# krm01/Snappy.jl

Hardware: AMD Instinct MI355X
Metric: GB/s compressed+decompressed (batched blocks) at 1/2/4/8 GPUs; % HBM peak (higher is better)
Workload: dtype u8; 1 GPU; configs 2+3: 10000 x 64 KiB text blocks per GPU, fast-mode compress + uncompress round trip per step; blocks_per_gpu=10000, block_bytes=65536, parallelism=dp1 (blocks sharded per rank, RCCL size all-gather)

## Files before the change

### include/snappy_mi355x.h

```cpp
#ifndef SNAPPY_MI355X_H_
#define SNAPPY_MI355X_H_

#include <stddef.h>
#include <stdint.h>

#ifdef __cplusplus
extern "C" {
#endif

typedef int32_t sm_status;
enum {
  SM_OK = 0,
  SM_INVALID_INPUT = 1,
  SM_BUFFER_TOO_SMALL = 2,
  SM_ERR_INPUT_TOO_LARGE = 16,
  SM_ERR_INVALID = 17,
  SM_ERR_VARINT = 18,
  SM_ERR_COPY_OFFSET = 19,
  SM_ERR_COPY_LENGTH = 20,
  SM_ERR_LITERAL = 21,
  SM_ERR_DEVICE = 32,
  SM_ERR_ARGUMENT = 33
};

enum { SM_MODE_REFERENCE = 0, SM_MODE_FAST = 1, SM_MODE_FAST_DENSE = 2 };

#define SM_BLOCK_SIZE 65536u
#define SM_OUT_LEN_ERROR 0xfff00000u

typedef struct sm_ctx sm_ctx;

const char* sm_status_message(sm_status st);

size_t sm_max_compressed_length(size_t source_length);
sm_status sm_uncompressed_length(const char* compressed, size_t compressed_length, size_t* result);
sm_status sm_parse32(const uint8_t* buf, size_t len, size_t off, uint32_t* value, size_t* next);
size_t sm_encode32(uint8_t* buf, uint32_t value);
sm_status sm_find_match_length(const uint8_t* buf, size_t len, size_t i1, size_t i2, size_t limit,
                               size_t* matched);

sm_ctx* sm_ctx_create(int device);
void sm_ctx_destroy(sm_ctx* ctx);
void* sm_ctx_stream(sm_ctx* ctx);
int sm_ctx_last_path(sm_ctx* ctx);
sm_status sm_ctx_set_small_decode(sm_ctx* ctx, int enable);
sm_status sm_ctx_set_split_compress(sm_ctx* ctx, int enable);
int sm_ctx_last_compress_split(sm_ctx* ctx);

sm_status sm_compress(sm_ctx* ctx, const char* input, size_t input_length, char* compressed,
                      size_t* compressed_length, int mode);
sm_status sm_uncompress(sm_ctx* ctx, const char* compressed, size_t compressed_length, char* uncompressed,
                        size_t* uncompressed_length);

sm_status sm_compress_batch_device(sm_ctx* ctx, const uint8_t* d_in, const uint64_t* d_in_off,
                                   const uint32_t* d_in_len, uint32_t nblk, uint8_t* d_out,
                                   const uint64_t* d_out_off, uint32_t* d_out_len, int mode, void* stream);
sm_status sm_compress_fragments_device(sm_ctx* ctx, const uint8_t* d_in, const uint64_t* d_in_off,
                                       const uint32_t* d_in_len, uint32_t nblk, uint8_t* d_out,
                                       const uint64_t* d_out_off, uint32_t* d_out_len, uint64_t total_len,
                                       int mode, void* stream);
sm_status sm_place_fragments_device(sm_ctx* ctx, const uint8_t* d_src, const uint64_t* d_src_off,
                                    const uint32_t* d_len, uint32_t nfrag, const uint64_t* d_dst_off,
                                    uint64_t total_len, int write_header, uint8_t* d_dst, uint64_t dst_capacity,
                                    uint64_t* d_local_off, int32_t* d_status, void* stream);
sm_status sm_uncompress_fragments_device(sm_ctx* ctx, const uint8_t* d_in, const uint64_t* d_in_off,
                                         const uint32_t* d_in_len, uint32_t nblk, uint8_t* d_out,
                                         const uint64_t* d_out_off, const uint32_t* d_frag_len, uint32_t* d_out_len,
                                         int32_t* d_status, void* stream);

sm_status sm_uncompress_batch_device(sm_ctx* ctx, const uint8_t* d_in, const uint64_t* d_in_off,
                                     const uint32_t* d_in_len, uint32_t nblk, uint8_t* d_out,
                                     const uint64_t* d_out_off, const uint32_t* d_out_cap,
                                     uint32_t* d_out_len, int32_t* d_status, void* stream);

sm_status sm_validate_batch_device(sm_ctx* ctx, const uint8_t* d_in, const uint64_t* d_in_off,
                                   const uint32_t* d_in_len, uint32_t nblk, int32_t* d_status, void* stream);
sm_status sm_uncompressed_length_batch_device(sm_ctx* ctx, const uint8_t* d_in, const uint64_t* d_in_off,
                                              const uint32_t* d_in_len, uint32_t nblk, uint32_t* d_len,
                                              int32_t* d_status, void* stream);

sm_status sm_compress_batch(sm_ctx* ctx, const uint8_t* in, const uint64_t* in_off, const uint32_t* in_len,
                            uint32_t nblk, uint8_t* out, const uint64_t* out_off, uint32_t* out_len, int mode);
sm_status sm_uncompress_batch(sm_ctx* ctx, const uint8_t* in, const uint64_t* in_off, const uint32_t* in_len,
                              uint32_t nblk, uint8_t* out, const uint64_t* out_off, const uint32_t* out_cap,
                              uint32_t* out_len, int32_t* status);

sm_status sm_compress_batch_sharded(sm_ctx* const* ctxs, int nctx, const uint8_t* in, const uint64_t* in_off,
                                    const uint32_t* in_len, uint32_t nblk, uint8_t* out, const uint64_t* out_off,
                                    uint32_t* out_len, int mode);
sm_status sm_uncompress_batch_sharded(sm_ctx* const* ctxs, int nctx, const uint8_t* in, const uint64_t* in_off,
                                      const uint32_t* in_len, uint32_t nblk, uint8_t* out, const uint64_t* out_off,
                                      const uint32_t* out_cap, uint32_t* out_len, int32_t* status);

sm_status sm_validate_compressed_buffer(sm_ctx* ctx, const char* compressed, size_t compressed_length);

sm_status sm_snappy_compress(const char* input, size_t input_length, char* compressed, size_t* compressed_length);
sm_status sm_snappy_uncompress(const char* compressed, size_t compressed_length, char* uncompressed,
                               size_t* uncompressed_length);
size_t sm_snappy_max_compressed_length(size_t source_length);
sm_status sm_snappy_uncompressed_length(const char* compressed, size_t compressed_length, size_t* result);
sm_status sm_snappy_validate_compressed_buffer(const char* compressed, size_t compressed_length);
sm_status sm_snappy_set_mode(int mode);

const char* sm_version(void);

#ifdef __cplusplus
}
#endif
#endif
```

### snappy.jl_amd/__init__.py

```python
import ctypes
import os
import threading

import numpy as np

HERE = os.path.dirname(os.path.abspath(__file__))
LIB_PATH = os.environ.get("SNAPPY_MI355X_LIB") or os.path.join(HERE, "libsnappy_mi355x.so")
BLOCK_SIZE = 65536

SM_OK = 0
SM_BUFFER_TOO_SMALL = 2
SM_ERR_DEVICE = 32
SM_OUT_LEN_ERROR = 0xFFF00000
MODES = {"reference": 0, "fast": 1, "dense": 2}

ABI_SYMBOLS = (
    "sm_status_message", "sm_max_compressed_length", "sm_uncompressed_length", "sm_parse32",
    "sm_encode32", "sm_ctx_create", "sm_ctx_destroy", "sm_ctx_stream", "sm_compress", "sm_uncompress",
    "sm_compress_batch_device", "sm_uncompress_batch_device", "sm_compress_batch",
    "sm_uncompress_batch", "sm_version", "sm_compress_fragments_device", "sm_ctx_last_path", "sm_ctx_set_small_decode",
    "sm_ctx_set_split_compress", "sm_ctx_last_compress_split",
    "sm_find_match_length", "sm_validate_batch_device", "sm_uncompressed_length_batch_device",
    "sm_validate_compressed_buffer", "sm_compress_batch_sharded", "sm_uncompress_batch_sharded",
    "sm_uncompress_fragments_device", "sm_place_fragments_device", "sm_snappy_compress", "sm_snappy_uncompress",
    "sm_snappy_max_compressed_length", "sm_snappy_uncompressed_length", "sm_snappy_validate_compressed_buffer",
    "sm_snappy_set_mode",
)


class SnappyError(Exception):

    def __init__(self, code, message=None):
        self.code = int(code)
        super().__init__(message if message is not None else status_message(code))


_lib = None
_ctx = {}
_ctx_lock = threading.Lock()


def library_path():
    return LIB_PATH


def lib():
    global _lib
    if _lib is None:
        if not os.path.exists(LIB_PATH):
            raise OSError("libsnappy_mi355x.so not built (run __graft_entry__.build())")
        _lib = load_library(LIB_PATH)
    return _lib


def load_library(path):
    L = ctypes.CDLL(path)
    vp, sz, i32, u32 = ctypes.c_void_p, ctypes.c_size_t, ctypes.c_int32, ctypes.c_uint32
    L.sm_status_message.restype = ctypes.c_char_p
    L.sm_status_message.argtypes = [i32]
    L.sm_max_compressed_length.restype = sz
    L.sm_max_compressed_length.argtypes = [sz]
    L.sm_uncompressed_length.restype = i32
    L.sm_uncompressed_length.argtypes = [vp, sz, ctypes.POINTER(sz)]
    L.sm_parse32.restype = i32
    L.sm_parse32.argtypes = [vp, sz, sz, ctypes.POINTER(u32), ctypes.POINTER(sz)]
    L.sm_encode32.restype = sz
    L.sm_encode32.argtypes = [vp, u32]
    L.sm_ctx_create.restype = vp
    L.sm_ctx_create.argtypes = [ctypes.c_int]
    L.sm_ctx_destroy.restype = None
    L.sm_ctx_destroy.argtypes = [vp]
    L.sm_ctx_stream.restype = vp
    L.sm_ctx_stream.argtypes = [vp]
    L.sm_compress.restype = i32
    L.sm_compress.argtypes = [vp, vp, sz, vp, ctypes.POINTER(sz), ctypes.c_int]
    L.sm_uncompress.restype = i32
    L.sm_uncompress.argtypes = [vp, vp, sz, vp, ctypes.POINTER(sz)]
    L.sm_compress_batch_device.restype = i32
    L.sm_compress_batch_device.argtypes = [vp, vp, vp, vp, u32, vp, vp, vp, ctypes.c_int, vp]
    L.sm_uncompress_batch_device.restype = i32
    L.sm_uncompress_batch_device.argtypes = [vp, vp, vp, vp, u32, vp, vp, vp, vp, vp, vp]
    L.sm_compress_batch.restype = i32
    L.sm_compress_batch.argtypes = [vp, vp, vp, vp, u32, vp, vp, vp, ctypes.c_int]
    L.sm_uncompress_batch.restype = i32
    L.sm_uncompress_batch.argtypes = [vp, vp, vp, vp, u32, vp, vp, vp, vp, vp]
    L.sm_compress_batch_sharded.restype = i32
    L.sm_compress_batch_sharded.argtypes = [vp, ctypes.c_int, vp, vp, vp, u32, vp, vp, vp, ctypes.c_int]
    L.sm_uncompress_batch_sharded.restype = i32
    L.sm_uncompress_batch_sharded.argtypes = [vp, ctypes.c_int, vp, vp, vp, u32, vp, vp, vp, vp, vp]
    L.sm_find_match_length.restype = i32
    L.sm_find_match_length.argtypes = [vp, sz, sz, sz, sz, ctypes.POINTER(sz)]
    L.sm_ctx_last_path.restype = ctypes.c_int
    L.sm_ctx_last_path.argtypes = [vp]
    L.sm_ctx_set_small_decode.restype = ctypes.c_int
    L.sm_ctx_set_small_decode.argtypes = [vp, ctypes.c_int]
    L.sm_ctx_set_split_compress.restype = ctypes.c_int
    L.sm_ctx_set_split_compress.argtypes = [vp, ctypes.c_int]
    L.sm_ctx_last_compress_split.restype = ctypes.c_int
    L.sm_ctx_last_compress_split.argtypes = [vp]
    L.sm_version.restype = ctypes.c_char_p
    L.sm_version.argtypes = []
    L.sm_compress_fragments_device.restype = i32
    L.sm_compress_fragments_device.argtypes = [vp, vp, vp, vp, u32, vp, vp, vp, ctypes.c_uint64, ctypes.c_int, vp]
    L.sm_validate_batch_device.restype = i32
    L.sm_validate_batch_device.argtypes = [vp, vp, vp, vp, u32, vp, vp]
    L.sm_uncompressed_length_batch_device.restype = i32
    L.sm_uncompressed_length_batch_device.argtypes = [vp, vp, vp, vp, u32, vp, vp, vp]
    L.sm_validate_compressed_buffer.restype = i32
    L.sm_validate_compressed_buffer.argtypes = [vp, vp, sz]
    L.sm_place_fragments_device.restype = i32
    L.sm_place_fragments_device.argtypes = [vp, vp, vp, vp, u32, vp, ctypes.c_uint64, ctypes.c_int, vp,
                                            ctypes.c_uint64, vp, vp, vp]
    L.sm_uncompress_fragments_device.restype = i32
    L.sm_uncompress_fragments_device.argtypes = [vp, vp, vp, vp, u32, vp, vp, vp, vp, vp, vp]
    L.sm_snappy_compress.restype = i32
    L.sm_snappy_compress.argtypes = [vp, sz, vp, ctypes.POINTER(sz)]
    L.sm_snappy_uncompress.restype = i32
    L.sm_snappy_uncompress.argtypes = [vp, sz, vp, ctypes.POINTER(sz)]
    L.sm_snappy_max_compressed_length.restype = sz
    L.sm_snappy_max_compressed_length.argtypes = [sz]
    L.sm_snappy_uncompressed_length.restype = i32
    L.sm_snappy_uncompressed_length.argtypes = [vp, sz, ctypes.POINTER(sz)]
    L.sm_snappy_validate_compressed_buffer.restype = i32
    L.sm_snappy_validate_compressed_buffer.argtypes = [vp, sz]
    L.sm_snappy_set_mode.restype = i32
    L.sm_snappy_set_mode.argtypes = [ctypes.c_int]
    return L


def status_message(code):
    return lib().sm_status_message(int(code)).decode()


def _bytes(x):
    if isinstance(x, str):
        x = x.encode("utf-8")
    if isinstance(x, np.ndarray):
        return np.ascontiguousarray(x, dtype=np.uint8)
    return np.frombuffer(bytes(x), dtype=np.uint8)


def context(device=0):
    with _ctx_lock:
        c = _ctx.get(device)
        if c is None:
            c = lib().sm_ctx_create(device)
            if not c:
                raise SnappyError(32, "no usable HIP device %d for snappy_mi355x" % device)
            _ctx[device] = c
    return c


def contexts(devices):
    seen, out = {}, []
    for d in devices:
        k = seen.get(d, 0)
        seen[d] = k + 1
        key = ("shard", d, k)
        c = _ctx.get(key)
        if c is None:
            c = lib().sm_ctx_create(d)
            if not c:
                raise SnappyError(32, "no usable HIP device %d for snappy_mi355x" % d)
            _ctx[key] = c
        out.append(c)
    return (ctypes.c_void_p * len(out))(*out)


def _mode(mode):
    if mode not in MODES:
        raise ValueError("mode must be 'reference', 'fast' or 'dense'")
    return MODES[mode]


def maxlength_compressed(n):
    return lib().sm_max_compressed_length(int(n))


def parse32(buf, offset=0):
    a = _bytes(buf)
    v = ctypes.c_uint32(0)
    nx = ctypes.c_size_t(0)
    st = lib().sm_parse32(a.ctypes.data if a.size else None, a.size, int(offset), ctypes.byref(v), ctypes.byref(nx))
    if st:
        raise SnappyError(st)
    return v.value, nx.value


def encode32(value):
    out = np.zeros(8, dtype=np.uint8)
    n = lib().sm_encode32(out.ctypes.data, int(value))
    return out[:n].tobytes()


def length_uncompressed(data):
    return parse32(data, 0)


_tls = threading.local()
_SCRATCH_MAX = 64 << 20


def _out_buffer(n):
    if n > _SCRATCH_MAX:
        a = np.empty(max(n, 1), dtype=np.uint8)
        return a.__array_interface__["data"][0], a
    buf = getattr(_tls, "buf", None)
    if buf is None or buf.size < n:
        buf = np.empty(max(n, 1 << 20), dtype=np.uint8)
        _tls.buf, _tls.ptr = buf, buf.__array_interface__["data"][0]
    return _tls.ptr, buf


def _in_arg(data):
    if isinstance(data, bytes):
        return (data if data else None), len(data), data
    a = _bytes(data)
    return (a.__array_interface__["data"][0] if a.size else None), a.size, a


def compress(data, mode="fast", device=0):
    src, n, keep = _in_arg(data)
    if n > 0xFFFFFFFF:
        raise SnappyError(16)
    cap = 32 + n + n // 6
    ptr, buf = _out_buffer(cap)
    ol = ctypes.c_size_t(cap)
    st = lib().sm_compress(context(device), src, n, ptr, ctypes.byref(ol), _mode(mode))
    if st:
        raise SnappyError(st)
    return ctypes.string_at(ptr, ol.value)


def find_match_length(buf, i1, i2, limit):
    src = _bytes(buf)
    res = ctypes.c_size_t(0)
    st = lib().sm_find_match_length(src.ctypes.data if src.size else None, src.size, i1, i2, limit,
                                    ctypes.byref(res))
    if st:
        raise SnappyError(st)
    return res.value


def last_uncompress_path(device=0):
    return int(lib().sm_ctx_last_path(context(device)))


def set_small_decode(enable, device=0):
    st = lib().sm_ctx_set_small_decode(context(device), 1 if enable else 0)
    if st:
        raise SnappyError(st)


def set_split_compress(enable, device=0):
    st = lib().sm_ctx_set_split_compress(context(device), 1 if enable else 0)
    if st:
        raise SnappyError(st)


def last_compress_split(device=0):
    return int(lib().sm_ctx_last_compress_split(context(device))) == 1


def _declared_length(b):
    v = 0
    for i in range(min(5, len(b))):
        c = b[i]
        v |= (c & 0x7F) << (7 * i)
        if c < 0x80:
            return v if v <= 0xFFFFFFFF else 0
    return 0


def uncompress(data, device=0):
    src, n, keep = _in_arg(data)
    size = _declared_length(keep if isinstance(keep, bytes) else memoryview(keep))
    ptr, buf = _out_buffer(size)
    ol = ctypes.c_size_t(size)
    st = lib().sm_uncompress(context(device), src, n, ptr, ctypes.byref(ol))
    if st:
        raise SnappyError(st)
    return ctypes.string_at(ptr, ol.value)



def pack_blocks(blocks):
    lens = np.array([len(b) for b in blocks], dtype=np.uint32)
    offs = np.zeros(len(blocks), dtype=np.uint64)
    if len(blocks) > 1:
        offs[1:] = np.cumsum(lens[:-1], dtype=np.uint64)
    buf = np.frombuffer(b"".join(bytes(b) for b in blocks), dtype=np.uint8) if blocks else np.zeros(0, np.uint8)
    return np.ascontiguousarray(buf), offs, lens


def slot_offsets(in_len):
    caps = (32 + in_len.astype(np.uint64) + in_len.astype(np.uint64) // 6 + 15) // 16 * 16
    offs = np.zeros(in_len.size, dtype=np.uint64)
    if in_len.size > 1:
        offs[1:] = np.cumsum(caps[:-1], dtype=np.uint64)
    return offs, caps


def compress_batch(blocks, mode="fast", device=0, devices=None):
    buf, in_off, in_len = pack_blocks(blocks)
    if np.any(in_len > BLOCK_SIZE):
        raise ValueError("batch blocks must be <= 65536 bytes")
    out_off, caps = slot_offsets(in_len)
    out = np.empty(int(out_off[-1] + caps[-1]) if len(blocks) else 1, dtype=np.uint8)
    out_len = np.zeros(len(blocks), dtype=np.uint32)
    if not blocks:
        return []
    args = (buf.ctypes.data, in_off.ctypes.data, in_len.ctypes.data, len(blocks), out.ctypes.data,
            out_off.ctypes.data, out_len.ctypes.data, _mode(mode))
    if devices is None:
        st = lib().sm_compress_batch(context(device), *args)
    else:
        st = lib().sm_compress_batch_sharded(contexts(devices), len(devices), *args)
    if st:
        raise SnappyError(st)
    return [out[int(o): int(o) + int(l)].tobytes() for o, l in zip(out_off, out_len)]


def uncompress_batch(streams, capacities=None, device=0, devices=None):
    if not streams:
        return [], np.zeros(0, np.int32)
    buf, in_off, in_len = pack_blocks(streams)
    if capacities is None:
        caps = []
        for s in streams:
            try:
                caps.append(parse32(s)[0])
            except SnappyError:
                caps.append(0)
        capacities = caps
    cap = np.array(capacities, dtype=np.uint32)
    out_off = np.zeros(len(streams), dtype=np.uint64)
    if len(streams) > 1:
        out_off[1:] = np.cumsum(cap[:-1].astype(np.uint64), dtype=np.uint64)
    out = np.empty(max(int(cap.astype(np.uint64).sum()), 1), dtype=np.uint8)
    out_len = np.zeros(len(streams), dtype=np.uint32)
    status = np.zeros(len(streams), dtype=np.int32)
    args = (buf.ctypes.data, in_off.ctypes.data, in_len.ctypes.data, len(streams), out.ctypes.data,
            out_off.ctypes.data, cap.ctypes.data, out_len.ctypes.data, status.ctypes.data)
    if devices is None:
        st = lib().sm_uncompress_batch(context(device), *args)
    else:
        st = lib().sm_uncompress_batch_sharded(contexts(devices), len(devices), *args)
    if st:
        raise SnappyError(st)
    res = [out[int(o): int(o) + int(l)].tobytes() if s == 0 else None for o, l, s in zip(out_off, out_len, status)]
    return res, status



def _ptr(t):
    return ctypes.c_void_p(t.data_ptr())


def _stream(stream, dev):
    import torch
    if stream is None:
        return torch.cuda.current_stream(dev).cuda_stream
    return stream.cuda_stream if hasattr(stream, "cuda_stream") else stream


def compress_batch_device(d_in, d_in_off, d_in_len, d_out, d_out_off, d_out_len, mode="fast", stream=None,
                          device=None):
    import torch
    dev = d_in.device.index if device is None else device
    if stream is None:
        stream = torch.cuda.current_stream(dev).cuda_stream
    elif hasattr(stream, "cuda_stream"):
        stream = stream.cuda_stream
    st = lib().sm_compress_batch_device(context(dev), _ptr(d_in), _ptr(d_in_off), _ptr(d_in_len), d_in_len.numel(),
                                        _ptr(d_out), _ptr(d_out_off), _ptr(d_out_len), _mode(mode),
                                        ctypes.c_void_p(stream))
    if st:
        raise SnappyError(st)


def compress_fragments_device(d_in, d_in_off, d_in_len, d_out, d_out_off, d_out_len, total_len, mode="fast",
                              stream=None, device=None):
    import torch
    dev = d_in.device.index if device is None else device
    if stream is None:
        stream = torch.cuda.current_stream(dev).cuda_stream
    elif hasattr(stream, "cuda_stream"):
        stream = stream.cuda_stream
    st = lib().sm_compress_fragments_device(context(dev), _ptr(d_in), _ptr(d_in_off), _ptr(d_in_len),
                                            d_in_len.numel(), _ptr(d_out), _ptr(d_out_off), _ptr(d_out_len),
                                            int(total_len), _mode(mode), ctypes.c_void_p(stream))
    if st:
        raise SnappyError(st)


def uncompress_batch_device(d_in, d_in_off, d_in_len, d_out, d_out_off, d_out_cap, d_out_len, d_status,
                            stream=None, device=None):
    import torch
    dev = d_in.device.index if device is None else device
    if stream is None:
        stream = torch.cuda.current_stream(dev).cuda_stream
    elif hasattr(stream, "cuda_stream"):
        stream = stream.cuda_stream
    st = lib().sm_uncompress_batch_device(context(dev), _ptr(d_in), _ptr(d_in_off), _ptr(d_in_len),
                                          d_in_len.numel(), _ptr(d_out), _ptr(d_out_off), _ptr(d_out_cap),
                                          _ptr(d_out_len), _ptr(d_status), ctypes.c_void_p(stream))
    if st:
        raise SnappyError(st)


def place_fragments_device(d_src, d_src_off, d_len, d_dst_off, d_dst, total_len, write_header, d_local_off=None,
                           d_status=None, stream=None, device=None):
    dev = d_dst.device.index if device is None else device
    nfrag = d_len.numel()
    nul = ctypes.c_void_p(0)
    st = lib().sm_place_fragments_device(context(dev), _ptr(d_src) if nfrag else nul, _ptr(d_src_off) if nfrag else nul,
                                         _ptr(d_len) if nfrag else nul, nfrag, _ptr(d_dst_off) if nfrag else nul,
                                         int(total_len), 1 if write_header else 0, _ptr(d_dst), d_dst.numel(),
                                         _ptr(d_local_off) if d_local_off is not None else nul,
                                         _ptr(d_status) if d_status is not None else nul,
                                         ctypes.c_void_p(_stream(stream, dev)))
    if st:
        raise SnappyError(st)


def uncompress_fragments_device(d_in, d_in_off, d_in_len, d_out, d_out_off, d_frag_len, d_out_len, d_status,
                                stream=None, device=None):
    dev = d_in.device.index if device is None else device
    st = lib().sm_uncompress_fragments_device(context(dev), _ptr(d_in), _ptr(d_in_off), _ptr(d_in_len),
                                              d_in_len.numel(), _ptr(d_out), _ptr(d_out_off), _ptr(d_frag_len),
                                              _ptr(d_out_len), _ptr(d_status), ctypes.c_void_p(_stream(stream, dev)))
    if st:
        raise SnappyError(st)


def validate_batch_device(d_in, d_in_off, d_in_len, d_status, stream=None, device=None):
    dev = d_in.device.index if device is None else device
    st = lib().sm_validate_batch_device(context(dev), _ptr(d_in), _ptr(d_in_off), _ptr(d_in_len), d_in_len.numel(),
                                        _ptr(d_status), ctypes.c_void_p(_stream(stream, dev)))
    if st:
        raise SnappyError(st)


def uncompressed_length_batch_device(d_in, d_in_off, d_in_len, d_len, d_status, stream=None, device=None):
    dev = d_in.device.index if device is None else device
    st = lib().sm_uncompressed_length_batch_device(context(dev), _ptr(d_in), _ptr(d_in_off), _ptr(d_in_len),
                                                   d_in_len.numel(), _ptr(d_len), _ptr(d_status),
                                                   ctypes.c_void_p(_stream(stream, dev)))
    if st:
        raise SnappyError(st)


def validate(data, device=0):
    src = _bytes(data)
    return int(lib().sm_validate_compressed_buffer(context(device), src.ctypes.data if src.size else None, src.size))


def version():
    return lib().sm_version().decode()
```

### snappy.jl_amd/csrc/sm_api.hip

```cpp
#include <hip/hip_runtime.h>
#include <stdint.h>
#include <string.h>

#include <algorithm>
#include <cstdlib>
#include <atomic>
#include <mutex>
#include <new>
#include <thread>
#include <vector>

#include "../../include/snappy_mi355x.h"
#include "sm_device.h"
#include "sm_internal.h"

#ifndef SM_VERSION_STR
#define SM_VERSION_STR "dev"
#endif

struct DevBuf {
  void* p = nullptr;
  size_t cap = 0;
  hipError_t ensure(size_t n) {
    if (n <= cap) return hipSuccess;
    if (p) (void)hipFree(p);
    p = nullptr;
    cap = 0;
    size_t want = n < 4096 ? 4096 : n;
    hipError_t e = hipMalloc(&p, want);
    if (e == hipSuccess) cap = want;
    return e;
  }
  void release() {
    if (p) (void)hipFree(p);
    p = nullptr;
    cap = 0;
  }
};

struct HostBuf {
  void* p = nullptr;
  void* dp = nullptr;
  size_t cap = 0;
  hipError_t ensure(size_t n) {
    if (n <= cap) return hipSuccess;
    release();
    const size_t want = ((n < (1u << 20) ? (1u << 20) : n) + 4095) & ~(size_t)4095;
    void* q = nullptr;
    if (posix_memalign(&q, 4096, want) != 0) return hipErrorOutOfMemory;
    const hipError_t e = hipHostRegister(q, want, hipHostRegisterMapped);
    if (e != hipSuccess) {
      free(q);
      return e;
    }
    p = q;
    cap = want;
    if (hipHostGetDevicePointer(&dp, q, 0) != hipSuccess) dp = nullptr;
    return hipSuccess;
  }
  void release() {
    if (p) {
      (void)hipHostUnregister(p);
      free(p);
    }
    p = nullptr;
    dp = nullptr;
    cap = 0;
  }
};

struct sm_ctx {
  int device = 0;
  hipStream_t stream = nullptr;
  hipStream_t copy = nullptr;
  std::vector<hipEvent_t> ev;
  DevBuf in, out, out2, meta, idx, gat, org;
  HostBuf stage;
  HostBuf stage_in;
  hipEvent_t in_ev = nullptr;
  int last_path = -1;
  bool small = true;
  bool split = true;
  bool last_split = false;
  std::mutex mu;
};

#ifndef SM_SMALL_BODY8
#define SM_SMALL_BODY8 8
#endif

namespace {

bool valid_mode(int m) { return m == SM_MODE_REFERENCE || m == SM_MODE_FAST || m == SM_MODE_FAST_DENSE; }

struct DeviceGuard {
  int prev = -1;
  explicit DeviceGuard(int dev) {
    if (hipGetDevice(&prev) != hipSuccess) prev = -1;
    (void)hipSetDevice(dev);
  }
  ~DeviceGuard() {
    if (prev >= 0) (void)hipSetDevice(prev);
  }
};


inline size_t align_up(size_t v, size_t a) { return (v + a - 1) / a * a; }

#ifdef SM_HOST_TRACE
#include <chrono>
#include <cstdio>
struct HostTrace {
  std::chrono::steady_clock::time_point t = std::chrono::steady_clock::now();
  void mark(const char* what, hipStream_t s) {
    (void)hipStreamSynchronize(s);
    const auto now = std::chrono::steady_clock::now();
    fprintf(stderr, "  %-28s %8.3f ms\n", what, std::chrono::duration<double, std::milli>(now - t).count());
    t = now;
  }
};
#define HT_DECL HostTrace ht_;
#define HT(what) ht_.mark(what, s);
#else
#define HT_DECL
#define HT(what)
#endif

constexpr uint32_t kParallelMinOutput = 4 * 65536;
constexpr size_t kOrgKeep = 256u << 20;
constexpr size_t kPipeMinInput = 32u << 20;
constexpr size_t kSmallCompressMax = 4u << 20;
constexpr uint32_t kPieceFrags = 256;
#ifndef SM_OUT_PIECE
#define SM_OUT_PIECE 2048
#endif
constexpr uint32_t kOutPieceFrags = SM_OUT_PIECE;

constexpr size_t kPinnedInMin = 32u << 10;
constexpr size_t kPinnedInMax = 16u << 20;

bool stage_in_acquire(sm_ctx* ctx, size_t n) {
  if (ctx->stage_in.ensure(n + 16) != hipSuccess || !ctx->stage_in.dp) return false;
  return !ctx->in_ev || hipEventSynchronize(ctx->in_ev) == hipSuccess;
}
hipError_t stage_in_release(sm_ctx* ctx, hipStream_t s) {
  if (!ctx->in_ev) {
    const hipError_t e = hipEventCreateWithFlags(&ctx->in_ev, hipEventDisableTiming);
    if (e != hipSuccess) {
      ctx->in_ev = nullptr;
      return e;
    }
  }
  return hipEventRecord(ctx->in_ev, s);
}

hipError_t upload_input(sm_ctx* ctx, const void* src, size_t n, hipStream_t s) {
  if (n == 0) return hipSuccess;
  if (n >= kPinnedInMin && n <= kPinnedInMax && stage_in_acquire(ctx, n)) {
    memcpy(ctx->stage_in.p, src, n);
    const hipError_t e = sm::launch_to_host((const uint8_t*)ctx->stage_in.dp, (uint32_t)n, (uint8_t*)ctx->in.p,
                                            nullptr, 0, nullptr, s);
    if (e != hipSuccess) return e;
    return stage_in_release(ctx, s);
  }
  return hipMemcpyAsync(ctx->in.p, src, n, hipMemcpyHostToDevice, s);
}

bool literal_only(const uint8_t* c, size_t n, size_t hdr, uint32_t size, sm::LitSpans& sp) {
  size_t p = hdr;
  uint64_t o = 0;
  sp.n = 0;
  while (p < n) {
    if (sp.n == sm::kLitSpans) return false;
    const uint32_t t = c[p];
    if (t & 3) return false;
    uint64_t len = (t >> 2) + 1;
    size_t q = p + 1;
    if ((t >> 2) >= 60) {
      const uint32_t nb = (t >> 2) - 59;
      if (nb > 3 || q + nb > n) return false;
      uint32_t v = 0;
      for (uint32_t k = 0; k < nb; ++k) v |= (uint32_t)c[q + k] << (8 * k);
      len = (uint64_t)v + 1;
      q += nb;
    }
    if (q + len > n || o + len > size) return false;
    sp.src[sp.n] = (uint32_t)q;
    sp.dst[sp.n] = (uint32_t)o;
    ++sp.n;
    o += len;
    p = q + len;
  }
  sp.dst[sp.n] = (uint32_t)o;
  return sp.n > 0 && o == size;
}

int literal_uncompress(sm_ctx* ctx, const uint8_t* comp, size_t n, uint32_t size, const sm::LitSpans& ls,
                       uint8_t* host_out) {
  hipStream_t s = ctx->stream;
  const size_t w_off = align_up(size, 256);
  if (ctx->stage.ensure(w_off + 64) != hipSuccess || !ctx->stage.dp) return 0;
  if (!stage_in_acquire(ctx, n)) return 0;
  memcpy(ctx->stage_in.p, comp, n);
  uint8_t* const sdp = (uint8_t*)ctx->stage.dp;
  volatile uint32_t* const w = (volatile uint32_t*)((uint8_t*)ctx->stage.p + w_off);
  w[1] = 0xffffffffu;
  if (sm::launch_literal_spans((const uint8_t*)ctx->stage_in.dp, ls, sdp, (uint32_t*)(sdp + w_off), s) != hipSuccess)
    return -1;
  if (hipStreamSynchronize(s) != hipSuccess) return -1;
  if (w[1] != 0 || w[0] != size) return -1;
  memcpy(host_out, ctx->stage.p, size);
  return 1;
}

hipError_t ensure_copy_stream(sm_ctx* ctx, size_t n) {
  if (!ctx->copy) {
    const hipError_t e = hipStreamCreateWithFlags(&ctx->copy, hipStreamNonBlocking);
    if (e != hipSuccess) {
      ctx->copy = nullptr;
      return e;
    }
  }
  while (ctx->ev.size() < n) {
    hipEvent_t e;
    const hipError_t r = hipEventCreateWithFlags(&e, hipEventDisableTiming);
    if (r != hipSuccess) return r;
    ctx->ev.push_back(e);
  }
  return hipSuccess;
}

void host_walk(const uint8_t* comp, uint32_t n, uint64_t p, uint64_t lim, uint64_t* exit_pos, uint64_t* produced) {
  uint64_t o = 0;
  while (p < lim) {
    const uint32_t c = comp[p];
    const uint32_t entry = sm::char_entry(c);
    const uint32_t taglen = entry >> 11;
    uint32_t tr = 0;
    for (uint32_t k = 0; k < 4; ++k) tr |= (p + 1 + k < n ? (uint32_t)comp[p + 1 + k] : 0u) << (8 * k);
    const uint32_t trailer = taglen >= 4 ? tr : (tr & ((1u << (8 * taglen)) - 1u));
    if (c & 3) {
      p += 1 + taglen;
      o += entry & 0xff;
    } else {
      const uint32_t lit = (entry & 0xff) + trailer;
      p += 1ull + taglen + lit;
      o += lit;
    }
  }
  *exit_pos = p;
  *produced = o;
}

struct PathChunk {
  uint64_t y, O, out, ex;
};
int path_first_error(sm_ctx* ctx, uint32_t n, uint32_t size, const std::vector<PathChunk>& path, int32_t* err) {
  if (n >= 0x80000000u || path.empty()) return 0;
  hipStream_t s = ctx->stream;
  const size_t npath = path.size();
  std::vector<sm::OriginPath> op(npath);
  for (size_t e = 0; e < npath; ++e) {
    const uint64_t O = std::min<uint64_t>(path[e].O, 0xffffffffull), out = std::min<uint64_t>(path[e].out, 0xffffffffull - O);
    op[e] = {(uint32_t)path[e].y, (uint32_t)std::min<uint64_t>(path[e].ex, 0xffffffffull), (uint32_t)O, (uint32_t)out};
  }
  const size_t st_off = align_up(npath * sizeof(sm::OriginPath), 256);
  if (ctx->org.ensure(st_off + npath * 4) != hipSuccess) return 0;
  sm::OriginPath* d_path = (sm::OriginPath*)ctx->org.p;
  int32_t* d_st = (int32_t*)((uint8_t*)ctx->org.p + st_off);
  if (hipMemcpyAsync(d_path, op.data(), npath * sizeof(sm::OriginPath), hipMemcpyHostToDevice, s) != hipSuccess)
    return -1;
  if (sm::launch_path_check((const uint8_t*)ctx->in.p, n, size, d_path, (uint32_t)npath, d_st, s) != hipSuccess)
    return -1;
  std::vector<int32_t> st(npath);
  if (hipMemcpyAsync(st.data(), d_st, npath * 4, hipMemcpyDeviceToHost, s) != hipSuccess) return -1;
  if (hipStreamSynchronize(s) != hipSuccess) return -1;
  for (int32_t v : st) {
    if (v == sm::kOk) continue;
    if (v == sm::kErrCross) return 0;
    *err = v;
    return 3;
  }
  const PathChunk& last = path.back();
  if (last.O + last.out == size) return 0;
  *err = sm::kErrInvalid;
  return 3;
}

int parallel_uncompress(sm_ctx* ctx, const uint8_t* comp, uint32_t n, uint32_t ip0, uint32_t size,
                        uint8_t* host_out, bool* copied, int32_t* err) {
  *copied = false;
  using sm::kIdxChunk;
  using sm::kIdxEntries;
  const uint32_t nchunks = (n - ip0 + kIdxChunk - 1) / kIdxChunk;
  const uint32_t nfrag = (uint32_t)(((uint64_t)size + 65535) / 65536);
  const size_t rec_n = (size_t)nchunks * kIdxEntries;
  const size_t frag_off = align_up(2 * rec_n * 4, 16);
  const size_t st_off = frag_off + (size_t)nfrag * sizeof(sm::StreamFrag);
  if (ctx->idx.ensure(st_off + (size_t)nfrag * 4) != hipSuccess) return 0;
  hipStream_t s = ctx->stream;
  HT_DECL
  uint32_t* d_rec = (uint32_t*)ctx->idx.p;
  const uint8_t* d_in = (const uint8_t*)ctx->in.p;
  if (sm::launch_stream_index(d_in, n, ip0, nchunks, d_rec, s) != hipSuccess) return -1;
  HT("index kernel")
  if (ctx->stage.ensure(2 * rec_n * 4) != hipSuccess) return 0;
  const uint32_t* rec = (const uint32_t*)ctx->stage.p;
  if (hipMemcpyAsync(ctx->stage.p, d_rec, 2 * rec_n * 4, hipMemcpyDeviceToHost, s) != hipSuccess) return -1;
  if (hipStreamSynchronize(s) != hipSuccess) return -1;
  HT("index records D2H")
  std::vector<PathChunk> path;
  path.reserve(nchunks + 16);
  uint64_t y = ip0, O = 0;
  while (y < (uint64_t)n - 1) {
    const uint64_t c = (y - ip0) / kIdxChunk, base = ip0 + c * kIdxChunk, l = y - base;
    if (c + 8 < nchunks) __builtin_prefetch(&rec[2 * (c + 8) * kIdxEntries]);
    uint64_t ex, ot;
    if (l < kIdxEntries) {
      ex = rec[2 * (c * kIdxEntries + l)];
      ot = rec[2 * (c * kIdxEntries + l) + 1];
    } else {
      host_walk(comp, n, y, std::min<uint64_t>(base + kIdxChunk, (uint64_t)n - 1), &ex, &ot);
    }
    path.push_back({y, O, ot, ex});
    O += ot;
    if (ex <= y) return 0;
    y = ex;
    if (O > size) break;
  }
  if (O != size) return path_first_error(ctx, n, size, path, err);
  std::vector<sm::StreamFrag> frags(nfrag);
  size_t k = 0;
  for (uint32_t f = 0; f < nfrag; ++f) {
    const uint64_t F = (uint64_t)f * 65536;
    while (k + 1 < path.size() && path[k].O + path[k].out <= F) ++k;
    frags[f] = {(uint32_t)path[k].y, (uint32_t)path[k].O, (uint32_t)F,
                f + 1 == nfrag ? 0xffffffffu : (uint32_t)(F + 65536)};
  }
  HT("host path + fragments")
  sm::StreamFrag* d_frags = (sm::StreamFrag*)((uint8_t*)ctx->idx.p + frag_off);
  int32_t* d_st = (int32_t*)((uint8_t*)ctx->idx.p + st_off);
  if (hipMemcpyAsync(d_frags, frags.data(), frags.size() * sizeof(sm::StreamFrag), hipMemcpyHostToDevice, s) !=
      hipSuccess)
    return -1;
  const uint32_t nfp = (nfrag + kOutPieceFrags - 1) / kOutPieceFrags;
  const uint32_t npiece = (host_out && nfp > 1 && ensure_copy_stream(ctx, nfp) == hipSuccess) ? nfp : 1;
  uint8_t* out = (uint8_t*)ctx->out.p;
  for (uint32_t pc = 0; pc < npiece; ++pc) {
    const uint32_t f0 = pc * kOutPieceFrags, f1 = npiece == 1 ? nfrag : std::min(nfrag, f0 + kOutPieceFrags);
    if (sm::launch_decompress_frags(d_in, n, size, out, d_frags + f0, f1 - f0, d_st + f0, s) != hipSuccess) return -1;
    if (npiece > 1 && hipEventRecord(ctx->ev[pc], s) != hipSuccess) return -1;
  }
  if (npiece > 1) {
    for (uint32_t pc = 0; pc < npiece; ++pc) {
      const size_t b0 = (size_t)pc * kOutPieceFrags * 65536;
      const size_t b1 = std::min((size_t)size, b0 + (size_t)kOutPieceFrags * 65536);
      if (hipStreamWaitEvent(ctx->copy, ctx->ev[pc], 0) != hipSuccess) return -1;
      if (hipMemcpyAsync(host_out + b0, out + b0, b1 - b0, hipMemcpyDeviceToHost, ctx->copy) != hipSuccess) return -1;
    }
    if (hipStreamSynchronize(ctx->copy) != hipSuccess) return -1;
  }
  std::vector<int32_t> st(nfrag);
  if (hipMemcpyAsync(st.data(), d_st, nfrag * 4, hipMemcpyDeviceToHost, s) != hipSuccess) return -1;
  if (hipStreamSynchronize(s) != hipSuccess) return -1;
  HT("fragment decode")
  bool cross = false;
  for (int32_t v : st) {
    if (v == sm::kErrCross) cross = true;
    else if (v != sm::kOk) return path_first_error(ctx, n, size, path, err);
  }
  if (!cross) {
    *copied = npiece > 1;
    return 1;
  }
  if (n >= 0x80000000u || size >= 0x80000000u) return 0;
  const size_t npath = path.size();
  std::vector<sm::OriginPath> op(npath);
  for (size_t e = 0; e < npath; ++e)
    op[e] = {(uint32_t)path[e].y, (uint32_t)path[e].ex, (uint32_t)path[e].O, (uint32_t)path[e].out};
  const size_t p_off = 0, path_off = align_up((size_t)size * 4, 256), st2_off = align_up(path_off + npath * 16, 256);
  const size_t pend_off = align_up(st2_off + npath * 4, 256);
  if (ctx->org.ensure(pend_off + 16) != hipSuccess) return 0;
  uint8_t* ob = (uint8_t*)ctx->org.p;
  uint32_t* d_P = (uint32_t*)(ob + p_off);
  sm::OriginPath* d_path = (sm::OriginPath*)(ob + path_off);
  int32_t* d_st2 = (int32_t*)(ob + st2_off);
  uint32_t* d_pend = (uint32_t*)(ob + pend_off);
  if (hipMemcpyAsync(d_path, op.data(), npath * sizeof(sm::OriginPath), hipMemcpyHostToDevice, s) != hipSuccess)
    return -1;
  if (sm::launch_origin_fill(d_in, n, size, d_path, (uint32_t)npath, d_P, d_st2, s) != hipSuccess) return -1;
  std::vector<int32_t> st2(npath);
  if (hipMemcpyAsync(st2.data(), d_st2, npath * 4, hipMemcpyDeviceToHost, s) != hipSuccess) return -1;
  if (hipStreamSynchronize(s) != hipSuccess) return -1;
  for (int32_t v : st2)
    if (v != sm::kOk) return path_first_error(ctx, n, size, path, err);
  bool done = false;
  for (int round = 0; round < 32 && !done; ++round) {
    uint32_t pend = 0;
    if (hipMemsetAsync(d_pend, 0, 4, s) != hipSuccess) return -1;
    if (sm::launch_origin_resolve(d_P, size, d_pend, s) != hipSuccess) return -1;
    if (hipMemcpyAsync(&pend, d_pend, 4, hipMemcpyDeviceToHost, s) != hipSuccess) return -1;
    if (hipStreamSynchronize(s) != hipSuccess) return -1;
    done = pend == 0;
  }
  if (!done) return 0;
  if (sm::launch_origin_gather(d_in, d_P, size, (uint8_t*)ctx->out.p, s) != hipSuccess) return -1;
  if (ctx->org.cap > kOrgKeep) {
    if (hipStreamSynchronize(s) != hipSuccess) return -1;
    ctx->org.release();
  }
  return 2;
}

#ifndef SM_SMALL_MIN
#define SM_SMALL_MIN 4096
#endif
constexpr uint32_t kSmallMinOutput = SM_SMALL_MIN;
constexpr uint32_t kSmallMaxChunks = (1u << 20) / sm::kSmallChunk;
#ifndef SM_SMALL_FINE_BODY10
#define SM_SMALL_FINE_BODY10 6
#endif
#ifndef SM_SMALL_TINY_BODY
#define SM_SMALL_TINY_BODY 16384
#endif
#ifndef SM_SMALL_TINY_BODY10
#define SM_SMALL_TINY_BODY10 9
#endif
uint32_t small_chunk(uint32_t body, uint32_t size) {
  if (body <= SM_SMALL_TINY_BODY && (uint64_t)body * 10 <= (uint64_t)size * SM_SMALL_TINY_BODY10)
    return sm::kSmallChunkTiny;
  if ((uint64_t)body * 10 > (uint64_t)size * SM_SMALL_FINE_BODY10 || body > (256u << 10)) return sm::kSmallChunk;
  return sm::kSmallChunkFine;
}
constexpr uint32_t kSmallMaxOutput = 64u << 20;
constexpr uint32_t kPinnedOutMax = 16u << 20;

int small_uncompress(sm_ctx* ctx, const uint8_t* comp, uint32_t n, uint32_t ip0, uint32_t size, uint8_t* host_out) {
  using sm::kIdxEntries;
  const uint32_t chunk = small_chunk(n - ip0, size);
  const uint32_t nchunks = (n - ip0 + chunk - 1) / chunk;
  uint32_t rounds = 1;
  uint32_t hops = sm::kSmallHops;
  if (size <= sm::kOneLaunchHops)
    hops = std::max(hops, size);
  else
    for (uint64_t reach = sm::kSmallHops; reach < size; reach *= sm::kSmallHops) ++rounds;
  const size_t path_off = align_up((size_t)nchunks * kIdxEntries * 8 + (size_t)nchunks * sm::kDeepChains * sm::kDeepLevels * 16, 256);
  const size_t ctl_off = align_up(path_off + (size_t)nchunks * sizeof(sm::OriginPath), 256);
  const size_t ctl_n = 4 + rounds;
  if (ctx->idx.ensure(ctl_off + ctl_n * 4) != hipSuccess) return 0;
  if (ctx->org.ensure((size_t)size * 4) != hipSuccess) return 0;
  const bool pin_out = size <= kPinnedOutMax;
  const size_t w_off = pin_out ? align_up(size, 256) : 0;
  if (ctx->stage.ensure(w_off + 64) != hipSuccess || !ctx->stage.dp) return 0;
  hipStream_t s = ctx->stream;
  uint8_t* ib = (uint8_t*)ctx->idx.p;
  uint32_t* d_ctl = (uint32_t*)(ib + ctl_off);
  uint8_t* const sdp = (uint8_t*)ctx->stage.dp;
  if (!stage_in_acquire(ctx, n)) return 0;
  memcpy(ctx->stage_in.p, comp, n);
  ((volatile uint32_t*)((uint8_t*)ctx->stage.p + w_off))[2] = 0;
  const hipError_t le = sm::launch_small_decode((const uint8_t*)ctx->in.p, (const uint8_t*)ctx->stage_in.dp, n, ip0,
                                                size, chunk, nchunks, (uint32_t*)ib, (sm::OriginPath*)(ib + path_off),
                                                d_ctl, (uint32_t*)ctx->org.p, rounds, hops,
                                                pin_out ? sdp : (uint8_t*)ctx->out.p, (uint32_t*)(sdp + w_off), s);
  if (le != hipSuccess || stage_in_release(ctx, s) != hipSuccess) {
    (void)hipStreamSynchronize(s);
    return -1;
  }
  if (!pin_out && hipMemcpyAsync(host_out, ctx->out.p, size, hipMemcpyDeviceToHost, s) != hipSuccess) return -1;
  if (hipStreamSynchronize(s) != hipSuccess) return -1;
  const volatile uint32_t* w = (const volatile uint32_t*)((uint8_t*)ctx->stage.p + w_off);
  if (w[0] || w[1] || w[2]) return 0;
  if (pin_out) memcpy(host_out, ctx->stage.p, size);
  return 4;
}

}

#define SM_CHECK(x)                 \
  do {                              \
    if ((x) != hipSuccess) return SM_ERR_DEVICE; \
  } while (0)

namespace {
struct Shard {
  uint32_t b0 = 0, n = 0;
  uint64_t in_base = 0, out_base = 0;
  std::vector<uint64_t> in_off, out_off;
};

std::vector<Shard> make_shards(int nctx, uint32_t nblk, const uint64_t* in_off, const uint64_t* out_off) {
  std::vector<Shard> sh((size_t)nctx);
  for (int i = 0; i < nctx; ++i) {
    Shard& s = sh[(size_t)i];
    s.b0 = (uint32_t)((uint64_t)nblk * (uint64_t)i / (uint64_t)nctx);
    s.n = (uint32_t)((uint64_t)nblk * (uint64_t)(i + 1) / (uint64_t)nctx) - s.b0;
    if (s.n == 0) continue;
    s.in_base = *std::min_element(in_off + s.b0, in_off + s.b0 + s.n);
    s.out_base = *std::min_element(out_off + s.b0, out_off + s.b0 + s.n);
    s.in_off.resize(s.n);
    s.out_off.resize(s.n);
    for (uint32_t k = 0; k < s.n; ++k) {
      s.in_off[k] = in_off[s.b0 + k] - s.in_base;
      s.out_off[k] = out_off[s.b0 + k] - s.out_base;
    }
  }
  return sh;
}

template <typename F>
sm_status run_shards(int nctx, F&& shard_fn) {
  std::vector<sm_status> st((size_t)nctx, SM_OK);
  std::vector<std::thread> th;
  th.reserve((size_t)nctx);
  for (int i = 0; i < nctx; ++i) th.emplace_back([&, i] { st[(size_t)i] = shard_fn(i); });
  for (auto& t : th) t.join();
  for (sm_status x : st)
    if (x != SM_OK) return x;
  return SM_OK;
}

sm_status gather_to_host(sm_ctx* ctx, const uint8_t* d_src, const uint64_t* d_src_off, const uint32_t* d_len,
                         const uint32_t* len, uint32_t nblk, const uint64_t* out_off, uint8_t* host) {
  hipStream_t s = ctx->stream;
  std::vector<uint64_t> dst(nblk);
  uint64_t total = 0;
  for (uint32_t b = 0; b < nblk; ++b) {
    dst[b] = total;
    total += len[b];
  }
  if (total == 0) return SM_OK;
  if (ctx->gat.ensure(8 * (size_t)nblk) != hipSuccess || ctx->out2.ensure(total + 16) != hipSuccess ||
      ctx->stage.ensure(total) != hipSuccess)
    return SM_ERR_DEVICE;
  uint64_t* d_dst = (uint64_t*)ctx->gat.p;
  if (hipMemcpyAsync(d_dst, dst.data(), 8 * (size_t)nblk, hipMemcpyHostToDevice, s) != hipSuccess) return SM_ERR_DEVICE;
  if (sm::launch_gather(d_src, d_src_off, d_len, d_dst, (uint8_t*)ctx->out2.p, nblk, s) != hipSuccess)
    return SM_ERR_DEVICE;
  if (hipMemcpyAsync(ctx->stage.p, ctx->out2.p, total, hipMemcpyDeviceToHost, s) != hipSuccess) return SM_ERR_DEVICE;
  if (hipStreamSynchronize(s) != hipSuccess) return SM_ERR_DEVICE;
  const uint8_t* st = (const uint8_t*)ctx->stage.p;
  for (uint32_t b = 0; b < nblk; ++b)
    if (len[b]) memcpy(host + out_off[b], st + dst[b], len[b]);
  return SM_OK;
}

sm_status check_compressed_lengths(const uint32_t* out_len, const uint32_t* in_len, uint32_t nblk) {
  for (uint32_t b = 0; b < nblk; ++b)
    if (out_len[b] > sm::max_compressed_length(in_len[b])) return out_len[b] >= SM_OUT_LEN_ERROR ? SM_ERR_DEVICE : SM_ERR_ARGUMENT;
  return SM_OK;
}

bool valid_ctxs(sm_ctx* const* ctxs, int nctx) {
  if (!ctxs || nctx <= 0) return false;
  for (int i = 0; i < nctx; ++i) {
    if (!ctxs[i]) return false;
    for (int j = 0; j < i; ++j)
      if (ctxs[j] == ctxs[i]) return false;
  }
  return true;
}
}

extern "C" {

int sm_ctx_last_path(sm_ctx* ctx) { return ctx ? ctx->last_path : -1; }

sm_status sm_ctx_set_small_decode(sm_ctx* ctx, int enable) {
  if (!ctx) return SM_ERR_ARGUMENT;
  std::lock_guard<std::mutex> lk(ctx->mu);
  ctx->small = enable != 0;
  return SM_OK;
}

sm_status sm_ctx_set_split_compress(sm_ctx* ctx, int enable) {
  if (!ctx) return SM_ERR_ARGUMENT;
  std::lock_guard<std::mutex> lk(ctx->mu);
  ctx->split = enable != 0;
  return SM_OK;
}

int sm_ctx_last_compress_split(sm_ctx* ctx) { return ctx ? (ctx->last_split ? 1 : 0) : -1; }

const char* sm_status_message(sm_status st) {
  switch (st) {
    case SM_OK: return "OK";
    case SM_INVALID_INPUT: return "Invalid input.";
    case SM_BUFFER_TOO_SMALL: return "Buffer too small.";
    case SM_ERR_INPUT_TOO_LARGE: return "Input too large.";
    case SM_ERR_INVALID: return "Invalid input.";
    case SM_ERR_VARINT: return "Could not decode varint32.";
    case SM_ERR_COPY_OFFSET: return "Invalid input: corrupt copy offset";
    case SM_ERR_COPY_LENGTH: return "Invalid input: corrupt copy length";
    case SM_ERR_LITERAL: return "Invalid input: corrupt literal";
    case SM_ERR_DEVICE: return "HIP device error.";
    case SM_ERR_ARGUMENT: return "Invalid argument.";
    default: return "Unknown status.";
  }
}

const char* sm_version(void) { return "snappy_mi355x gfx950 " SM_VERSION_STR; }

size_t sm_max_compressed_length(size_t n) { return 32 + n + n / 6; }

sm_status sm_parse32(const uint8_t* buf, size_t len, size_t off, uint32_t* value, size_t* next) {
  uint32_t result = 0;
  for (int i = 0; i < 5; ++i) {
    if (off + i >= len) return SM_ERR_VARINT;
    uint32_t b = buf[off + i];
    if (i < 4) {
      result |= (b & 0x7f) << (7 * i);
      if (b < 0x80) {
        if (value) *value = result;
        if (next) *next = off + i + 1;
        return SM_OK;
      }
    } else {
      result |= (b & 0x7f) << 28;
      if (b < 0x10) {
        if (value) *value = result;
        if (next) *next = off + 5;
        return SM_OK;
      }
    }
  }
  return SM_ERR_VARINT;
}

size_t sm_encode32(uint8_t* buf, uint32_t v) {
  size_t i = 0;
  while (v >= 0x80) {
    buf[i++] = (uint8_t)(v | 0x80);
    v >>= 7;
  }
  buf[i++] = (uint8_t)v;
  return i;
}

sm_status sm_find_match_length(const uint8_t* buf, size_t len, size_t i1, size_t i2, size_t limit,
                               size_t* matched) {
  if (!matched || (len && !buf)) return SM_ERR_ARGUMENT;
  auto ld64 = [&](size_t i, uint64_t* v) {
    if (i + 8 > len) return false;
    memcpy(v, buf + i, 8);
    return true;
  };
  size_t m = 0;
  while (i2 + 7 <= limit) {
    uint64_t a, b;
    if (!ld64(i1 + m, &a) || !ld64(i2, &b)) return SM_ERR_ARGUMENT;
    if (a != b) {
      *matched = m + (__builtin_ctzll(a ^ b) >> 3);
      return SM_OK;
    }
    i2 += 8;
    m += 8;
  }
  while (i2 <= limit) {
    if (i2 >= len || i1 + m >= len) return SM_ERR_ARGUMENT;
    if (buf[i1 + m] != buf[i2]) break;
    ++i2;
    ++m;
  }
  *matched = m;
  return SM_OK;
}

sm_status sm_uncompressed_length(const char* compressed, size_t n, size_t* result) {
  uint32_t v = 0;
  sm_status st = sm_parse32((const uint8_t*)compressed, n, 0, &v, nullptr);
  if (st == SM_OK && result) *result = v;
  return st;
}

sm_ctx* sm_ctx_create(int device) {
  int count = 0;
  if (hipGetDeviceCount(&count) != hipSuccess || count <= 0 || device < 0 || device >= count) return nullptr;
  sm_ctx* ctx = new (std::nothrow) sm_ctx();
  if (!ctx) return nullptr;
  ctx->device = device;
  DeviceGuard g(device);
  if (hipStreamCreateWithFlags(&ctx->stream, hipStreamNonBlocking) != hipSuccess) {
    delete ctx;
    return nullptr;
  }
  return ctx;
}

void sm_ctx_destroy(sm_ctx* ctx) {
  if (!ctx) return;
  {
    DeviceGuard g(ctx->device);
    (void)hipStreamSynchronize(ctx->stream);
    ctx->in.release();
    ctx->out.release();
    ctx->out2.release();
    ctx->meta.release();
    ctx->idx.release();
    ctx->gat.release();
    ctx->org.release();
    ctx->stage.release();
    ctx->stage_in.release();
    if (ctx->in_ev) (void)hipEventDestroy(ctx->in_ev);
    if (ctx->copy) {
      (void)hipStreamSynchronize(ctx->copy);
      (void)hipStreamDestroy(ctx->copy);
    }
    for (hipEvent_t e : ctx->ev) (void)hipEventDestroy(e);
    (void)hipStreamDestroy(ctx->stream);
  }
  delete ctx;
}

void* sm_ctx_stream(sm_ctx* ctx) { return ctx ? (void*)ctx->stream : nullptr; }

sm_status sm_compress_batch_device(sm_ctx* ctx, const uint8_t* d_in, const uint64_t* d_in_off,
                                   const uint32_t* d_in_len, uint32_t nblk, uint8_t* d_out,
                                   const uint64_t* d_out_off, uint32_t* d_out_len, int mode, void* stream) {
  if (!ctx || !valid_mode(mode)) return SM_ERR_ARGUMENT;
  if (nblk == 0) return SM_OK;
  if (!d_in || !d_in_off || !d_in_len || !d_out || !d_out_off || !d_out_len) return SM_ERR_ARGUMENT;
  DeviceGuard g(ctx->device);
  sm::CompressArgs a{d_in, d_in_off, d_in_len, d_out, d_out_off, d_out_len, nblk, 0, 1};
  SM_CHECK(sm::launch_compress(a, mode, (hipStream_t)stream));
  return SM_OK;
}

sm_status sm_compress_fragments_device(sm_ctx* ctx, const uint8_t* d_in, const uint64_t* d_in_off,
                                       const uint32_t* d_in_len, uint32_t nblk, uint8_t* d_out,
                                       const uint64_t* d_out_off, uint32_t* d_out_len, uint64_t total_len,
                                       int mode, void* stream) {
  if (!ctx || !valid_mode(mode)) return SM_ERR_ARGUMENT;
  if (total_len > 0xffffffffull) return SM_ERR_INPUT_TOO_LARGE;
  if (nblk == 0) return SM_OK;
  if (!d_in || !d_in_off || !d_in_len || !d_out || !d_out_off || !d_out_len) return SM_ERR_ARGUMENT;
  DeviceGuard g(ctx->device);
  sm::CompressArgs a{d_in, d_in_off, d_in_len, d_out, d_out_off, d_out_len, nblk, sm::hashtable_size(total_len), 0};
  SM_CHECK(sm::launch_compress(a, mode, (hipStream_t)stream));
  return SM_OK;
}

sm_status sm_place_fragments_device(sm_ctx* ctx, const uint8_t* d_src, const uint64_t* d_src_off,
                                    const uint32_t* d_len, uint32_t nfrag, const uint64_t* d_dst_off,
                                    uint64_t total_len, int write_header, uint8_t* d_dst, uint64_t dst_capacity,
                                    uint64_t* d_local_off, int32_t* d_status, void* stream) {
  if (!ctx) return SM_ERR_ARGUMENT;
  if (total_len > 0xffffffffull) return SM_ERR_INPUT_TOO_LARGE;
  if (nfrag == 0 && !write_header) return SM_OK;
  if (!d_dst || (nfrag && (!d_src || !d_src_off || !d_len || !d_dst_off))) return SM_ERR_ARGUMENT;
  if (write_header && dst_capacity < sm::varint_len((uint32_t)total_len)) return SM_BUFFER_TOO_SMALL;
  DeviceGuard g(ctx->device);
  SM_CHECK(sm::launch_place(d_src, d_src_off, d_len, d_dst_off, nfrag, total_len, write_header ? 1 : 0, dst_capacity,
                            d_dst, d_local_off, d_status, (hipStream_t)stream));
  return SM_OK;
}

sm_status sm_uncompress_batch_device(sm_ctx* ctx, const uint8_t* d_in, const uint64_t* d_in_off,
                                     const uint32_t* d_in_len, uint32_t nblk, uint8_t* d_out,
                                     const uint64_t* d_out_off, const uint32_t* d_out_cap,
                                     uint32_t* d_out_len, int32_t* d_status, void* stream) {
  if (!ctx) return SM_ERR_ARGUMENT;
  if (nblk == 0) return SM_OK;
  if (!d_in || !d_in_off || !d_in_len || !d_out || !d_out_off || !d_out_cap || !d_out_len || !d_status)
    return SM_ERR_ARGUMENT;
  DeviceGuard g(ctx->device);
  sm::DecompressArgs a{d_in, d_in_off, d_in_len, d_out, d_out_off, d_out_cap, d_out_len, d_status, nblk};
  SM_CHECK(sm::launch_decompress(a, 0, (hipStream_t)stream));
  return SM_OK;
}

sm_status sm_compress_batch(sm_ctx* ctx, const uint8_t* in, const uint64_t* in_off, const uint32_t* in_len,
                            uint32_t nblk, uint8_t* out, const uint64_t* out_off, uint32_t* out_len, int mode) {
  if (!ctx || !valid_mode(mode)) return SM_ERR_ARGUMENT;
  if (nblk == 0) return SM_OK;
  if (!in || !in_off || !in_len || !out || !out_off || !out_len) return SM_ERR_ARGUMENT;
  size_t in_total = 0, out_total = 0;
  for (uint32_t b = 0; b < nblk; ++b) {
    if (in_len[b] > SM_BLOCK_SIZE) return SM_ERR_ARGUMENT;
    size_t ie = in_off[b] + in_len[b];
    size_t oe = out_off[b] + sm_max_compressed_length(in_len[b]);
    if (ie > in_total) in_total = ie;
    if (oe > out_total) out_total = oe;
  }
  std::lock_guard<std::mutex> lk(ctx->mu);
  DeviceGuard g(ctx->device);
  hipStream_t s = ctx->stream;
  size_t meta_bytes = (size_t)nblk * (8 + 4 + 8 + 4);
  SM_CHECK(ctx->in.ensure(in_total + 16));
  SM_CHECK(ctx->out.ensure(out_total + 16));
  SM_CHECK(ctx->meta.ensure(meta_bytes + 64));
  uint8_t* m = (uint8_t*)ctx->meta.p;
  uint64_t* d_in_off = (uint64_t*)m;
  uint64_t* d_out_off = (uint64_t*)(m + 8 * (size_t)nblk);
  uint32_t* d_in_len = (uint32_t*)(m + 16 * (size_t)nblk);
  uint32_t* d_out_len = (uint32_t*)(m + 20 * (size_t)nblk);
  SM_CHECK(hipMemcpyAsync(ctx->in.p, in, in_total, hipMemcpyHostToDevice, s));
  SM_CHECK(hipMemcpyAsync(d_in_off, in_off, 8 * (size_t)nblk, hipMemcpyHostToDevice, s));
  SM_CHECK(hipMemcpyAsync(d_out_off, out_off, 8 * (size_t)nblk, hipMemcpyHostToDevice, s));
  SM_CHECK(hipMemcpyAsync(d_in_len, in_len, 4 * (size_t)nblk, hipMemcpyHostToDevice, s));
  sm::CompressArgs a{(const uint8_t*)ctx->in.p, d_in_off, d_in_len, (uint8_t*)ctx->out.p, d_out_off, d_out_len,
                     nblk, 0, 1};
  SM_CHECK(sm::launch_compress(a, mode, s));
  SM_CHECK(hipMemcpyAsync(out_len, d_out_len, 4 * (size_t)nblk, hipMemcpyDeviceToHost, s));
  SM_CHECK(hipStreamSynchronize(s));
  const sm_status lst = check_compressed_lengths(out_len, in_len, nblk);
  if (lst != SM_OK) return lst;
  return gather_to_host(ctx, (const uint8_t*)ctx->out.p, d_out_off, d_out_len, out_len, nblk, out_off, out);
}

sm_status sm_uncompress_batch(sm_ctx* ctx, const uint8_t* in, const uint64_t* in_off, const uint32_t* in_len,
                              uint32_t nblk, uint8_t* out, const uint64_t* out_off, const uint32_t* out_cap,
                              uint32_t* out_len, int32_t* status) {
  if (!ctx) return SM_ERR_ARGUMENT;
  if (nblk == 0) return SM_OK;
  if (!in || !in_off || !in_len || !out || !out_off || !out_cap || !out_len || !status) return SM_ERR_ARGUMENT;
  size_t in_total = 0, out_total = 0;
  for (uint32_t b = 0; b < nblk; ++b) {
    size_t ie = in_off[b] + in_len[b];
    size_t oe = out_off[b] + out_cap[b];
    if (ie > in_total) in_total = ie;
    if (oe > out_total) out_total = oe;
  }
  std::lock_guard<std::mutex> lk(ctx->mu);
  DeviceGuard g(ctx->device);
  hipStream_t s = ctx->stream;
  size_t meta_bytes = (size_t)nblk * (8 + 8 + 4 + 4 + 4 + 4);
  SM_CHECK(ctx->in.ensure(in_total + 16));
  SM_CHECK(ctx->out.ensure(out_total + 16));
  SM_CHECK(ctx->meta.ensure(meta_bytes + 64));
  uint8_t* m = (uint8_t*)ctx->meta.p;
  uint64_t* d_in_off = (uint64_t*)m;
  uint64_t* d_out_off = (uint64_t*)(m + 8 * (size_t)nblk);
  uint32_t* d_in_len = (uint32_t*)(m + 16 * (size_t)nblk);
  uint32_t* d_out_cap = (uint32_t*)(m + 20 * (size_t)nblk);
  uint32_t* d_out_len = (uint32_t*)(m + 24 * (size_t)nblk);
  int32_t* d_status = (int32_t*)(m + 28 * (size_t)nblk);
  SM_CHECK(hipMemcpyAsync(ctx->in.p, in, in_total, hipMemcpyHostToDevice, s));
  SM_CHECK(hipMemcpyAsync(d_in_off, in_off, 8 * (size_t)nblk, hipMemcpyHostToDevice, s));
  SM_CHECK(hipMemcpyAsync(d_out_off, out_off, 8 * (size_t)nblk, hipMemcpyHostToDevice, s));
  SM_CHECK(hipMemcpyAsync(d_in_len, in_len, 4 * (size_t)nblk, hipMemcpyHostToDevice, s));
  SM_CHECK(hipMemcpyAsync(d_out_cap, out_cap, 4 * (size_t)nblk, hipMemcpyHostToDevice, s));
  sm::DecompressArgs a{(const uint8_t*)ctx->in.p, d_in_off, d_in_len, (uint8_t*)ctx->out.p, d_out_off,
                       d_out_cap, d_out_len, d_status, nblk};
  SM_CHECK(sm::launch_decompress(a, 0, s));
  SM_CHECK(hipMemcpyAsync(out_len, d_out_len, 4 * (size_t)nblk, hipMemcpyDeviceToHost, s));
  SM_CHECK(hipMemcpyAsync(status, d_status, 4 * (size_t)nblk, hipMemcpyDeviceToHost, s));
  SM_CHECK(hipStreamSynchronize(s));
  for (uint32_t b = 0; b < nblk; ++b)
    if (status[b] != SM_OK) out_len[b] = 0;
  return gather_to_host(ctx, (const uint8_t*)ctx->out.p, d_out_off, d_out_len, out_len, nblk, out_off, out);
}

sm_status sm_validate_batch_device(sm_ctx* ctx, const uint8_t* d_in, const uint64_t* d_in_off,
                                   const uint32_t* d_in_len, uint32_t nblk, int32_t* d_status, void* stream) {
  if (!ctx) return SM_ERR_ARGUMENT;
  if (nblk == 0) return SM_OK;
  if (!d_in || !d_in_off || !d_in_len || !d_status) return SM_ERR_ARGUMENT;
  DeviceGuard g(ctx->device);
  SM_CHECK(sm::launch_validate(d_in, d_in_off, d_in_len, nblk, d_status, (hipStream_t)stream));
  return SM_OK;
}

sm_status sm_uncompressed_length_batch_device(sm_ctx* ctx, const uint8_t* d_in, const uint64_t* d_in_off,
                                              const uint32_t* d_in_len, uint32_t nblk, uint32_t* d_len,
                                              int32_t* d_status, void* stream) {
  if (!ctx) return SM_ERR_ARGUMENT;
  if (nblk == 0) return SM_OK;
  if (!d_in || !d_in_off || !d_in_len || !d_len || !d_status) return SM_ERR_ARGUMENT;
  DeviceGuard g(ctx->device);
  SM_CHECK(sm::launch_uncompressed_length(d_in, d_in_off, d_in_len, nblk, d_len, d_status, (hipStream_t)stream));
  return SM_OK;
}

sm_status sm_compress_batch_sharded(sm_ctx* const* ctxs, int nctx, const uint8_t* in, const uint64_t* in_off,
                                    const uint32_t* in_len, uint32_t nblk, uint8_t* out, const uint64_t* out_off,
                                    uint32_t* out_len, int mode) {
  if (!valid_ctxs(ctxs, nctx) || !valid_mode(mode)) return SM_ERR_ARGUMENT;
  if (nblk == 0) return SM_OK;
  if (!in || !in_off || !in_len || !out || !out_off || !out_len) return SM_ERR_ARGUMENT;
  for (uint32_t b = 0; b < nblk; ++b)
    if (in_len[b] > SM_BLOCK_SIZE) return SM_ERR_ARGUMENT;
  const std::vector<Shard> sh = make_shards(nctx, nblk, in_off, out_off);
  return run_shards(nctx, [&](int i) -> sm_status {
    const Shard& s = sh[(size_t)i];
    if (s.n == 0) return SM_OK;
    return sm_compress_batch(ctxs[i], in + s.in_base, s.in_off.data(), in_len + s.b0, s.n, out + s.out_base,
                             s.out_off.data(), out_len + s.b0, mode);
  });
}

sm_status sm_uncompress_batch_sharded(sm_ctx* const* ctxs, int nctx, const uint8_t* in, const uint64_t* in_off,
                                      const uint32_t* in_len, uint32_t nblk, uint8_t* out, const uint64_t* out_off,
                                      const uint32_t* out_cap, uint32_t* out_len, int32_t* status) {
  if (!valid_ctxs(ctxs, nctx)) return SM_ERR_ARGUMENT;
  if (nblk == 0) return SM_OK;
  if (!in || !in_off || !in_len || !out || !out_off || !out_cap || !out_len || !status) return SM_ERR_ARGUMENT;
  const std::vector<Shard> sh = make_shards(nctx, nblk, in_off, out_off);
  return run_shards(nctx, [&](int i) -> sm_status {
    const Shard& s = sh[(size_t)i];
    if (s.n == 0) return SM_OK;
    return sm_uncompress_batch(ctxs[i], in + s.in_base, s.in_off.data(), in_len + s.b0, s.n, out + s.out_base,
                               s.out_off.data(), out_cap + s.b0, out_len + s.b0, status + s.b0);
  });
}

sm_status sm_validate_compressed_buffer(sm_ctx* ctx, const char* compressed, size_t n) {
  if (!ctx || (n && !compressed)) return SM_ERR_ARGUMENT;
  if (n > 0xffffffffull) return SM_ERR_ARGUMENT;
  std::lock_guard<std::mutex> lk(ctx->mu);
  DeviceGuard g(ctx->device);
  hipStream_t s = ctx->stream;
  SM_CHECK(ctx->in.ensure(n + 16));
  SM_CHECK(ctx->meta.ensure(64));
  uint8_t* m = (uint8_t*)ctx->meta.p;
  uint64_t* d_off = (uint64_t*)m;
  uint32_t* d_len = (uint32_t*)(m + 8);
  int32_t* d_status = (int32_t*)(m + 12);
  const uint64_t zero = 0;
  const uint32_t len32 = (uint32_t)n;
  int32_t st = SM_ERR_DEVICE;
  SM_CHECK(upload_input(ctx, compressed, n, s));
  SM_CHECK(hipMemcpyAsync(d_off, &zero, 8, hipMemcpyHostToDevice, s));
  SM_CHECK(hipMemcpyAsync(d_len, &len32, 4, hipMemcpyHostToDevice, s));
  SM_CHECK(sm::launch_validate((const uint8_t*)ctx->in.p, d_off, d_len, 1, d_status, s));
  SM_CHECK(hipMemcpyAsync(&st, d_status, 4, hipMemcpyDeviceToHost, s));
  SM_CHECK(hipStreamSynchronize(s));
  return st;
}

sm_status sm_compress(sm_ctx* ctx, const char* input, size_t n, char* compressed, size_t* compressed_length,
                      int mode) {
  if (!ctx || !compressed_length || (n && !input) || !compressed) return SM_ERR_ARGUMENT;
  if (!valid_mode(mode)) return SM_ERR_ARGUMENT;
  if (n > 0xffffffffull) return SM_ERR_INPUT_TOO_LARGE;
  if (*compressed_length < sm_max_compressed_length(n)) return SM_BUFFER_TOO_SMALL;
  uint8_t hdr[5];
  size_t hl = sm_encode32(hdr, (uint32_t)n);
  memcpy(compressed, hdr, hl);
  if (n == 0) {
    *compressed_length = hl;
    return SM_OK;
  }
  const uint32_t nfrag = (uint32_t)((n + SM_BLOCK_SIZE - 1) / SM_BLOCK_SIZE);
  const size_t slot = align_up(sm_max_compressed_length(SM_BLOCK_SIZE) + 8, 256);
  std::vector<uint64_t> in_off(nfrag), out_off(nfrag), dst_off(nfrag);
  std::vector<uint32_t> in_len(nfrag), out_len(nfrag);
  for (uint32_t i = 0; i < nfrag; ++i) {
    in_off[i] = (uint64_t)i * SM_BLOCK_SIZE;
    size_t e = in_off[i] + SM_BLOCK_SIZE;
    in_len[i] = (uint32_t)((e < n ? e : n) - in_off[i]);
    out_off[i] = (uint64_t)i * slot;
  }
  std::lock_guard<std::mutex> lk(ctx->mu);
  DeviceGuard g(ctx->device);
  hipStream_t s = ctx->stream;
  ctx->last_split = false;
  SM_CHECK(ctx->in.ensure(n + 16));
  SM_CHECK(ctx->out.ensure((size_t)nfrag * slot));
  SM_CHECK(ctx->out2.ensure(sm_max_compressed_length(n) + 16));
  SM_CHECK(ctx->meta.ensure((size_t)nfrag * 32 + 64 + 4 * 256));
  uint8_t* m = (uint8_t*)ctx->meta.p;
  uint64_t* d_in_off = (uint64_t*)m;
  uint64_t* d_out_off = (uint64_t*)(m + 8 * (size_t)nfrag);
  uint64_t* d_dst_off = (uint64_t*)(m + 16 * (size_t)nfrag);
  uint32_t* d_in_len = (uint32_t*)(m + 24 * (size_t)nfrag);
  uint32_t* d_out_len = (uint32_t*)(m + 28 * (size_t)nfrag);
  uint32_t* d_part_len = (uint32_t*)(m + 32 * (size_t)nfrag + 64);
  HT_DECL
  const size_t t_off = align_up(sm_max_compressed_length(n) + 16, 256);
  if (n <= kSmallCompressMax && ctx->stage.ensure(t_off + 16) == hipSuccess && ctx->stage.dp) {
    uint32_t parts = 1;
    if (mode != SM_MODE_REFERENCE && ctx->split) {
      uint32_t p2 = 1;
      while (p2 < nfrag) p2 <<= 1;
      parts = std::min<uint32_t>(sm::kWave, 256 / p2);
    }
    const uint32_t span = (uint32_t)((SM_BLOCK_SIZE / 1024 + parts - 1) / parts);
    const size_t sl = parts > 1 ? std::max<size_t>(slot, (size_t)parts * span * sm::kSpanSlot) : slot;
    SM_CHECK(ctx->out.ensure((size_t)nfrag * sl));
    sm::CompressArgs a{(const uint8_t*)ctx->in.p, d_in_off, d_in_len, (uint8_t*)ctx->out.p, d_out_off, d_out_len,
                       nfrag, sm::hashtable_size(n), 0};
    const bool staged = mode != SM_MODE_REFERENCE && stage_in_acquire(ctx, n);
    if (staged) {
      memcpy(ctx->stage_in.p, input, n);
      a.in_host = (const uint8_t*)ctx->stage_in.dp;
    } else {
      SM_CHECK(upload_input(ctx, input, n, s));
    }
    if (mode == SM_MODE_REFERENCE) {
      SM_CHECK(sm::launch_frag_plan(n, nfrag, sl, d_in_off, d_in_len, d_out_off, s));
    } else {
      a.plan_n = n;
      a.plan_slot = sl;
    }
    uint8_t* const sdp = (uint8_t*)ctx->stage.dp;
    const sm::ScSpan sp{parts, span, (uint64_t)span * sm::kSpanSlot, d_part_len};
    hipError_t le = parts > 1 ? sm::launch_compress_span(a, mode, sp, s) : sm::launch_compress(a, mode, s);
    if (le == hipSuccess)
      le = parts > 1 ? sm::launch_parts_gather((const uint8_t*)ctx->out.p, d_out_off, sp, (const uint8_t*)ctx->in.p,
                                               d_in_off, d_in_len, nfrag, (uint64_t*)(sdp + t_off), sdp, s)
                     : sm::launch_frag_gather((const uint8_t*)ctx->out.p, d_out_off, d_out_len, d_in_len, nfrag,
                                              (uint64_t*)(sdp + t_off), sdp, s);
    if (staged) {
      const hipError_t re = stage_in_release(ctx, s);
      if (le == hipSuccess) le = re;
    }
    if (le != hipSuccess) {
      (void)hipStreamSynchronize(s);
      return SM_ERR_DEVICE;
    }
    SM_CHECK(hipStreamSynchronize(s));
    HT("compress (small): all")
    const volatile uint64_t* tot = (const volatile uint64_t*)((uint8_t*)ctx->stage.p + t_off);
    const uint64_t len = tot[0];
    if (tot[1]) return SM_ERR_DEVICE;
    if (hl + len > *compressed_length) return SM_BUFFER_TOO_SMALL;
    memcpy(compressed + hl, ctx->stage.p, len);
    *compressed_length = hl + len;
    ctx->last_split = parts > 1;
    return SM_OK;
  }
  SM_CHECK(hipMemcpyAsync(d_in_off, in_off.data(), 8 * (size_t)nfrag, hipMemcpyHostToDevice, s));
  SM_CHECK(hipMemcpyAsync(d_out_off, out_off.data(), 8 * (size_t)nfrag, hipMemcpyHostToDevice, s));
  SM_CHECK(hipMemcpyAsync(d_in_len, in_len.data(), 4 * (size_t)nfrag, hipMemcpyHostToDevice, s));
  uint32_t npiece = n >= kPipeMinInput ? (nfrag + kPieceFrags - 1) / kPieceFrags : 1;
  if (npiece > 1 && ensure_copy_stream(ctx, npiece) != hipSuccess) npiece = 1;
  for (uint32_t pc = 0; pc < npiece; ++pc) {
    const uint32_t f0 = pc * kPieceFrags, f1 = npiece == 1 ? nfrag : std::min(nfrag, f0 + kPieceFrags);
    const size_t b0 = (size_t)f0 * SM_BLOCK_SIZE, b1 = std::min(n, (size_t)f1 * SM_BLOCK_SIZE);
    if (npiece == 1) {
      SM_CHECK(hipMemcpyAsync(ctx->in.p, input, n, hipMemcpyHostToDevice, s));
    } else {
      SM_CHECK(hipMemcpyAsync((uint8_t*)ctx->in.p + b0, input + b0, b1 - b0, hipMemcpyHostToDevice, ctx->copy));
      SM_CHECK(hipEventRecord(ctx->ev[pc], ctx->copy));
      SM_CHECK(hipStreamWaitEvent(s, ctx->ev[pc], 0));
    }
    sm::CompressArgs a{(const uint8_t*)ctx->in.p, d_in_off + f0, d_in_len + f0, (uint8_t*)ctx->out.p,
                       d_out_off + f0, d_out_len + f0, f1 - f0, sm::hashtable_size(n), 0};
    SM_CHECK(sm::launch_compress(a, mode, s));
  }
  HT("compress: H2D input + kernels")
  SM_CHECK(hipMemcpyAsync(out_len.data(), d_out_len, 4 * (size_t)nfrag, hipMemcpyDeviceToHost, s));
  SM_CHECK(hipStreamSynchronize(s));
  HT("compress: kernels + lengths")
  {
    const sm_status lst = check_compressed_lengths(out_len.data(), in_len.data(), nfrag);
    if (lst != SM_OK) return lst;
  }
  size_t total = 0;
  for (uint32_t i = 0; i < nfrag; ++i) {
    dst_off[i] = total;
    total += out_len[i];
  }
  if (hl + total > *compressed_length) return SM_BUFFER_TOO_SMALL;
  SM_CHECK(hipMemcpyAsync(d_dst_off, dst_off.data(), 8 * (size_t)nfrag, hipMemcpyHostToDevice, s));
  SM_CHECK(sm::launch_gather((const uint8_t*)ctx->out.p, d_out_off, d_out_len, d_dst_off, (uint8_t*)ctx->out2.p,
                             nfrag, s));
  HT("compress: gather")
  SM_CHECK(hipMemcpyAsync(compressed + hl, ctx->out2.p, total, hipMemcpyDeviceToHost, s));
  SM_CHECK(hipStreamSynchronize(s));
  HT("compress: D2H output")
  *compressed_length = hl + total;
  return SM_OK;
}

sm_status sm_uncompress(sm_ctx* ctx, const char* compressed, size_t n, char* uncompressed,
                        size_t* uncompressed_length) {
  if (!ctx || !uncompressed_length || (n && !compressed)) return SM_ERR_ARGUMENT;
  uint32_t size = 0;
  sm_status st = sm_parse32((const uint8_t*)compressed, n, 0, &size, nullptr);
  if (st != SM_OK) return st;
  if (n > 0xffffffffull) return SM_ERR_ARGUMENT;
  if (*uncompressed_length < size) return SM_BUFFER_TOO_SMALL;
  if (size && !uncompressed) return SM_ERR_ARGUMENT;
  std::lock_guard<std::mutex> lk(ctx->mu);
  DeviceGuard g(ctx->device);
  hipStream_t s = ctx->stream;
  SM_CHECK(ctx->in.ensure(n + 16));
  SM_CHECK(ctx->out.ensure((size_t)size + 16));
  SM_CHECK(ctx->meta.ensure(64));
  uint8_t* m = (uint8_t*)ctx->meta.p;
  uint64_t* d_off = (uint64_t*)m;
  uint32_t* d_in_len = (uint32_t*)(m + 8);
  uint32_t* d_cap = (uint32_t*)(m + 12);
  uint32_t* d_out_len = (uint32_t*)(m + 16);
  int32_t* d_status = (int32_t*)(m + 20);
  uint32_t hv[2] = {(uint32_t)n, size};
  HT_DECL
  size_t hdr = 0;
  (void)sm_parse32((const uint8_t*)compressed, n, 0, &size, &hdr);
  {
    sm::LitSpans ls;
    if (ctx->small && size <= kPinnedOutMax && n <= kPinnedInMax && literal_only((const uint8_t*)compressed, n, hdr, size, ls)) {
      const int r = literal_uncompress(ctx, (const uint8_t*)compressed, n, size, ls, (uint8_t*)uncompressed);
      if (r < 0) return SM_ERR_DEVICE;
      if (r == 1) {
        ctx->last_path = 5;
        *uncompressed_length = size;
        return SM_OK;
      }
    }
  }
  if (ctx->small && size >= kSmallMinOutput && size <= kSmallMaxOutput && n > hdr &&
      (uint64_t)(n - hdr) * 8 <= (uint64_t)size * SM_SMALL_BODY8 &&
      (n - hdr + sm::kSmallChunk - 1) / sm::kSmallChunk <= kSmallMaxChunks) {
    const int r = small_uncompress(ctx, (const uint8_t*)compressed, (uint32_t)n, (uint32_t)hdr, size,
                                   (uint8_t*)uncompressed);
    if (r < 0) return SM_ERR_DEVICE;
    if (r == 4) {
      ctx->last_path = 4;
      *uncompressed_length = size;
      return SM_OK;
    }
  }
  SM_CHECK(upload_input(ctx, compressed, n, s));
  HT("uncompress: H2D input")
  if (size >= kParallelMinOutput && n - hdr >= 2 * sm::kIdxChunk) {
    bool copied = false;
    int32_t err = SM_OK;
    const int r = parallel_uncompress(ctx, (const uint8_t*)compressed, (uint32_t)n, (uint32_t)hdr, size,
                                      (uint8_t*)uncompressed, &copied, &err);
    if (r < 0) return SM_ERR_DEVICE;
    if (r == 3) {
      ctx->last_path = 3;
      return err;
    }
    if (r >= 1) {
      ctx->last_path = r;
      if (!copied) {
        SM_CHECK(hipMemcpyAsync(uncompressed, ctx->out.p, size, hipMemcpyDeviceToHost, s));
        SM_CHECK(hipStreamSynchronize(s));
      }
      HT("uncompress: D2H output")
      *uncompressed_length = size;
      return SM_OK;
    }
  }
  ctx->last_path = 0;
  sm::DecompressArgs a{(const uint8_t*)ctx->in.p, d_off, d_in_len, (uint8_t*)ctx->out.p, d_off, d_cap, d_out_len,
                       d_status, 1};
  a.one_n = hv[0];
  a.one_cap = hv[1];
  SM_CHECK(sm::launch_decompress(a, size > SM_BLOCK_SIZE, s));
  const size_t w_off = align_up(size, 256);
  if (size <= kPinnedOutMax && ctx->stage.ensure(w_off + 64) == hipSuccess && ctx->stage.dp) {
    uint8_t* const sdp = (uint8_t*)ctx->stage.dp;
    SM_CHECK(sm::launch_to_host((const uint8_t*)ctx->out.p, size, sdp, d_out_len, 2, (uint32_t*)(sdp + w_off), s));
    SM_CHECK(hipStreamSynchronize(s));
    const volatile uint32_t* w = (const volatile uint32_t*)((uint8_t*)ctx->stage.p + w_off);
    const uint32_t dlen = w[0];
    const int32_t dst = (int32_t)w[1];
    if (dst != SM_OK) return dst;
    if (dlen > size) return SM_ERR_DEVICE;
    if (dlen) memcpy(uncompressed, ctx->stage.p, dlen);
    *uncompressed_length = dlen;
    return SM_OK;
  }
  int32_t dst = 0;
  uint32_t dlen = 0;
  SM_CHECK(hipMemcpyAsync(&dst, d_status, 4, hipMemcpyDeviceToHost, s));
  SM_CHECK(hipMemcpyAsync(&dlen, d_out_len, 4, hipMemcpyDeviceToHost, s));
  SM_CHECK(hipStreamSynchronize(s));
  if (dst != SM_OK) return dst;
  if (dlen) {
    SM_CHECK(hipMemcpyAsync(uncompressed, ctx->out.p, dlen, hipMemcpyDeviceToHost, s));
    SM_CHECK(hipStreamSynchronize(s));
  }
  *uncompressed_length = dlen;
  return SM_OK;
}

sm_status sm_uncompress_fragments_device(sm_ctx* ctx, const uint8_t* d_in, const uint64_t* d_in_off,
                                         const uint32_t* d_in_len, uint32_t nblk, uint8_t* d_out,
                                         const uint64_t* d_out_off, const uint32_t* d_frag_len, uint32_t* d_out_len,
                                         int32_t* d_status, void* stream) {
  if (!ctx) return SM_ERR_ARGUMENT;
  if (nblk == 0) return SM_OK;
  if (!d_in || !d_in_off || !d_in_len || !d_out || !d_out_off || !d_frag_len || !d_out_len || !d_status)
    return SM_ERR_ARGUMENT;
  DeviceGuard g(ctx->device);
  sm::DecompressArgs a{d_in, d_in_off, d_in_len, d_out, d_out_off, d_frag_len, d_out_len, d_status, nblk, 1};
  SM_CHECK(sm::launch_decompress(a, 0, (hipStream_t)stream));
  return SM_OK;
}


namespace {
std::mutex g_default_mu;
sm_ctx* g_default_ctx = nullptr;
std::atomic<int> g_default_mode{SM_MODE_FAST_DENSE};

sm_ctx* default_ctx() {
  std::lock_guard<std::mutex> lk(g_default_mu);
  if (!g_default_ctx) {
    const char* e = getenv("SNAPPY_MI355X_DEVICE");
    g_default_ctx = sm_ctx_create(e ? atoi(e) : 0);
  }
  return g_default_ctx;
}
}

namespace {
sm_status snappy_c_status(sm_status st) {
  return st == SM_OK ? SM_OK : (st == SM_BUFFER_TOO_SMALL ? SM_BUFFER_TOO_SMALL : SM_INVALID_INPUT);
}
}

sm_status sm_snappy_set_mode(int mode) {
  if (!valid_mode(mode)) return SM_ERR_ARGUMENT;
  g_default_mode.store(mode, std::memory_order_relaxed);
  return SM_OK;
}

sm_status sm_snappy_compress(const char* input, size_t input_length, char* compressed, size_t* compressed_length) {
  sm_ctx* ctx = default_ctx();
  if (!ctx) return SM_INVALID_INPUT;
  return snappy_c_status(sm_compress(ctx, input, input_length, compressed, compressed_length,
                                     g_default_mode.load(std::memory_order_relaxed)));
}

sm_status sm_snappy_uncompress(const char* compressed, size_t compressed_length, char* uncompressed,
                               size_t* uncompressed_length) {
  sm_ctx* ctx = default_ctx();
  if (!ctx) return SM_INVALID_INPUT;
  return snappy_c_status(sm_uncompress(ctx, compressed, compressed_length, uncompressed, uncompressed_length));
}

size_t sm_snappy_max_compressed_length(size_t source_length) { return sm_max_compressed_length(source_length); }

sm_status sm_snappy_uncompressed_length(const char* compressed, size_t compressed_length, size_t* result) {
  return snappy_c_status(sm_uncompressed_length(compressed, compressed_length, result));
}

sm_status sm_snappy_validate_compressed_buffer(const char* compressed, size_t compressed_length) {
  sm_ctx* ctx = default_ctx();
  if (!ctx) return SM_INVALID_INPUT;
  return snappy_c_status(sm_validate_compressed_buffer(ctx, compressed, compressed_length));
}

}
```

### snappy.jl_amd/csrc/sm_compress.hip

```cpp
#include <type_traits>

#include "sm_device.h"
#include "sm_internal.h"

namespace sm {



__device__ inline uint32_t emit_varint(uint8_t* dst, uint32_t op, uint32_t v, uint32_t lane) {
  uint32_t nb = varint_len(v);
  if (lane < nb) dst[op + lane] = (uint8_t)(((v >> (7 * lane)) & 0x7f) | (lane + 1 < nb ? 0x80 : 0));
  return op + nb;
}

__device__ inline uint32_t put_copy_upto_64(uint8_t* dst, uint32_t op, uint32_t offset, uint32_t len) {
  if (len < 12 && offset < 2048) {
    dst[op] = (uint8_t)(1 + ((len - 4) << 2) + ((offset >> 3) & 0xe0));
    dst[op + 1] = (uint8_t)offset;
    return op + 2;
  }
  dst[op] = (uint8_t)(2 + ((len - 1) << 2));
  dst[op + 1] = (uint8_t)offset;
  dst[op + 2] = (uint8_t)(offset >> 8);
  return op + 3;
}

__device__ inline uint32_t put_copy(uint8_t* dst, uint32_t op, uint32_t offset, uint32_t len) {
  if (len < 12) return put_copy_upto_64(dst, op, offset, len);
  while (len >= 68) { op = put_copy_upto_64(dst, op, offset, 64); len -= 64; }
  if (len > 64) { op = put_copy_upto_64(dst, op, offset, 60); len -= 60; }
  return put_copy_upto_64(dst, op, offset, len);
}


constexpr uint32_t kMaxProbes = 320;
constexpr uint32_t kProbeSteps = kMaxProbes / kWave;
constexpr uint32_t kTabBytes = 2 * kMaxHashTableSize;

struct BlockBytes {
  __amdgpu_buffer_rsrc_t r;
  uint32_t nm4;
  __device__ uint32_t word(uint32_t pos) const {
    const uint32_t pc = min(pos, nm4), sh = pos - pc;
    const uint32_t w = __builtin_amdgcn_raw_buffer_load_b32(r, (int)pc, 0, 0);
    return sh < 4 ? w >> (sh << 3) : 0u;
  }
  __device__ uint32_t byte(uint32_t pos) const { return __builtin_amdgcn_raw_buffer_load_b8(r, (int)pos, 0, 0); }
};

struct LdsBytes {
  const uint8_t* blk;
  uint32_t n;
  __device__ uint32_t word(uint32_t pos) const { return lds_ld32(blk, min(pos, n)); }
  __device__ uint32_t byte(uint32_t pos) const { return blk[min(pos, n)]; }
};
constexpr uint32_t kLdsBlockPad = 32;

__device__ inline uint32_t tab_probe(uint32_t* t, uint32_t h, uint32_t p) {
  const uint32_t sh = (h & 1u) << 4;
  const uint32_t addr = (uint32_t)(uintptr_t)((__attribute__((address_space(3))) uint32_t*)(&t[h >> 1]));
  const uint32_t mk = 0xffffu << sh, v = p << sh;
  uint32_t old;
  asm volatile("ds_mskor_rtn_b32 %0, %1, %2, %3\n\ts_waitcnt lgkmcnt(0)"
               : "=&v"(old)
               : "v"(addr), "v"(mk), "v"(v)
               : "memory");
  return (old >> sh) & 0xffffu;
}

template <class B>
__device__ inline void copy_to_global(const B& S, uint8_t* __restrict__ g, uint32_t s, uint32_t len,
                                      uint32_t lane) {
  uint32_t head = (uint32_t)((16 - ((uintptr_t)g & 15)) & 15);
  if (head > len) head = len;
  if (lane < head) g[lane] = (uint8_t)S.byte(s + lane);
  g += head; s += head; len -= head;
  const uint32_t n16 = len >> 4;
  uint4* g16 = reinterpret_cast<uint4*>(g);
  constexpr uint32_t kU = 4;
  for (uint32_t k0 = lane; k0 < n16; k0 += kU * kWave) {
    uint4 v[kU];
#pragma unroll
    for (uint32_t i = 0; i < kU; ++i) {
      const uint32_t p = s + 16 * (k0 + i * kWave);
      if (k0 + i * kWave < n16) v[i] = make_uint4(S.word(p), S.word(p + 4), S.word(p + 8), S.word(p + 12));
    }
#pragma unroll
    for (uint32_t i = 0; i < kU; ++i)
      if (k0 + i * kWave < n16) g16[k0 + i * kWave] = v[i];
  }
  const uint32_t done = n16 << 4;
  if (lane < len - done) g[done + lane] = (uint8_t)S.byte(s + done + lane);
}

template <class B>
__device__ inline uint32_t emit_literal_w(const B& S, uint8_t* dst, uint32_t op, uint32_t start,
                                          uint32_t len, uint32_t lane) {
  const uint32_t n = len - 1;
  if (len < 60) {
    if (lane == 0) dst[op] = (uint8_t)(n << 2);
    op += 1;
  } else {
    const uint32_t count = n < 256 ? 1 : n < 65536 ? 2 : n < (1u << 24) ? 3 : 4;
    if (lane == 0) dst[op] = (uint8_t)((59 + count) << 2);
    if (lane >= 1 && lane <= count) dst[op + lane] = (uint8_t)(n >> (8 * (lane - 1)));
    op += 1 + count;
  }
  copy_to_global(S, dst + op, start, len, lane);
  return op + len;
}

template <class B>
__device__ uint32_t flush_copies(const B& S, uint8_t* __restrict__ dst, uint32_t op, uint32_t& base,
                                 uint32_t ntok, uint32_t tk, uint32_t tl, uint32_t lane) {
  const bool act = lane < ntok;
  const uint32_t pos = tk & 0xffffu, off = tk >> 16;
  const uint32_t end = pos + tl;
  const uint32_t pend = __shfl_up(end, 1, kWave);
  const uint32_t ls = lane == 0 ? base : pend;
  const uint32_t ll = act ? pos - ls : 0u;
  const uint32_t lt = ll == 0 ? 0u : ll < 60 ? 1u : ll <= 256 ? 2u : 3u;
  const uint32_t ct = act ? copy_tag_bytes(off, tl) : 0u;
  const uint32_t sz = lt + ll + ct;
  const uint32_t inc = scan_dpp(sz);
  const uint32_t o = op + inc - sz;
  const uint32_t lo = o + lt;
  if (lt == 1) dst[o] = (uint8_t)((ll - 1) << 2);
  if (lt > 1) {
    const uint32_t n1 = ll - 1;
    dst[o] = (uint8_t)((58 + lt) << 2);
    dst[o + 1] = (uint8_t)n1;
    if (lt > 2) dst[o + 2] = (uint8_t)(n1 >> 8);
  }
  for (uint32_t i = 0;; i += 4) {
    const bool go = ll <= 64 && i < ll;
    if (!ballot(go)) break;
    if (go) {
      const uint32_t w = S.word(ls + i), r = ll - i;
      uint8_t* q = dst + lo + i;
      q[0] = (uint8_t)w;
      if (r > 1) q[1] = (uint8_t)(w >> 8);
      if (r > 2) q[2] = (uint8_t)(w >> 16);
      if (r > 3) q[3] = (uint8_t)(w >> 24);
    }
  }
  for (uint64_t lm = ballot(ll > 64); lm; lm &= lm - 1) {
    const uint32_t t = ctz64(lm);
    copy_to_global(S, dst + readlane(lo, t), readlane(ls, t), readlane(ll, t), lane);
  }
  if (act) put_copy(dst, lo + ll, off, tl);
  base = readlane(end, ntok - 1);
  return op + readlane(inc, kWave - 1);
}

__device__ inline uint32_t writelane(uint32_t v, uint32_t l, uint32_t old) {
  asm volatile("v_writelane_b32 %0, %1, %2" : "+v"(old) : "s"(v), "{m0}"(l));
  return old;
}

template <bool kLds>
__global__ __launch_bounds__(64) void k_compress_exact(CompressArgs a) {
  __shared__ __attribute__((aligned(16))) uint32_t stab[kTabBytes / 4];
  __shared__ __attribute__((aligned(16))) uint8_t sblk[kLds ? kBlockSize + kLdsBlockPad : 16];

  const uint32_t b = blockIdx.x;
  const uint32_t lane = lane_id();
  const uint32_t n = a.in_len[b];
  uint8_t* dst = a.out + a.out_off[b];
  if (n > kBlockSize) {
    if (lane == 0) a.out_len[b] = 0xffffffffu;
    return;
  }
  std::conditional_t<kLds, LdsBytes, BlockBytes> S;
  if constexpr (kLds) {
    const uint8_t* src = a.in + a.in_off[b];
    wave_load_global_to_lds(sblk, src, n, lane);
    for (uint32_t k = n + lane; k < n + kLdsBlockPad; k += kWave) sblk[k] = 0;
    S.blk = sblk;
    S.n = n;
  } else {
    S.r = __builtin_amdgcn_make_buffer_rsrc(const_cast<uint8_t*>(a.in + a.in_off[b]), (short)0, (int)n, 0x00020000);
    S.nm4 = n - 4;
  }
  const uint32_t tsize = a.table_size ? a.table_size : hashtable_size(n);
  const uint32_t shift = 32 - (31 - __builtin_clz(tsize));
  for (uint32_t k = lane; k < tsize / 2; k += kWave) stab[k] = 0;
  uint32_t Dk[kProbeSteps] = {}, Dn[kProbeSteps] = {};
  {
    uint32_t d = 0, skip = 32;
#pragma unroll
    for (uint32_t i = 0; i < kProbeSteps; ++i) {
      for (uint32_t l = 0; l < kWave; ++l) {
        Dk[i] = writelane(d, l, Dk[i]);
        if (l) Dn[i] = writelane(d, l - 1, Dn[i]);
        else if (i) Dn[i - 1] = writelane(d, kWave - 1, Dn[i - 1]);
        const uint32_t step = skip >> 5;
        skip += step;
        d = min(d + step, 0x20000u);
      }
    }
    Dn[kProbeSteps - 1] = writelane(d, kWave - 1, Dn[kProbeSteps - 1]);
  }
  __syncthreads();

  uint32_t op = a.header ? emit_varint(dst, 0, n, lane) : 0;
  if (n == 0) {
    if (lane == 0) a.out_len[b] = op;
    return;
  }
  const uint32_t e = n - 1;
  const int32_t ip_limit = (int32_t)n - 16;
  uint32_t ip = 0, next_emit = 0, base = 0, ntok = 0, tk = 0, tl = 0;

  if (n >= kInputMarginBytes) {
    for (;;) {
      ip += 1;
      const uint32_t p0 = ip;
      uint32_t p = 0, h = 0, raw = 0;
      bool valid = false;
      uint64_t hm = 0;
#pragma unroll
      for (uint32_t i = 0; i < kProbeSteps; ++i) {
        p = p0 + Dk[i];
        valid = (int32_t)(p0 + Dn[i]) <= ip_limit;
        const uint32_t cur = S.word(p);
        h = hash32(cur, shift);
        raw = 0;
        if (__builtin_expect(valid, 1)) raw = tab_probe(stab, h, p);
        hm = ballot(valid && raw < p && S.word(raw) == cur);
        if (hm || ballot(valid) != ~0ull) break;
      }
      const bool found = hm != 0;
      uint32_t cand = 0;
      if (__builtin_expect(found, 1)) {
        const uint32_t j = ctz64(hm);
        const uint32_t pj = readlane(p, j);
        if (valid && lane > j && raw <= pj)
          reinterpret_cast<uint16_t*>(stab)[h] = (uint16_t)raw;
        ip = pj;
        cand = readlane(raw, j);
      }
      if (__builtin_expect(!found, 0)) break;
      for (;;) {
        const uint32_t avail = n - ip;
        auto fbyte = [](uint32_t x) {
          uint32_t r;
          asm("v_ffbl_b32 %0, %1" : "=v"(r) : "v"(x));
          return min(r >> 3, 4u);
        };
        uint32_t A = S.word(ip + 4 * lane);
        uint32_t fb = fbyte(A ^ S.word(cand + 4 * lane));
        const uint64_t lim0 = avail > 4 * kWave ? 0ull : ~0ull << ((avail - 1) >> 2);
        uint64_t m = ballot(fb < 4) | lim0;
        uint32_t f, rb = 0;
        if (__builtin_expect(m != 0, 1)) {
          f = min(readlane(4 * lane + fb, ctz64(m)), avail);
        } else {
          for (;;) {
            rb += 4 * kWave;
            const uint32_t off = rb + 4 * lane;
            fb = fbyte(S.word(ip + off) ^ S.word(cand + off));
            m = ballot(fb < 4 || off + 4 >= avail);
            if (__builtin_expect(m != 0, 1)) {
              f = min(readlane(off + fb, ctz64(m)), avail);
              break;
            }
          }
        }
        if (__builtin_expect(f < 4 || cand >= ip, 0)) break;
        const uint32_t ipn = ip + f;
        uint32_t wp, wc;
        if (__builtin_expect(rb == 0 && f <= 4 * kWave - 4, 1)) {
          const uint32_t k = (f - 1) >> 2, r8 = ((f - 1) & 3u) << 3;
          const uint64_t w = ((uint64_t)readlane(A, k + 1) << 32) | readlane(A, k);
          wp = (uint32_t)(w >> r8);
          wc = (uint32_t)(w >> (r8 + 8));
        } else {
          wp = uniform(S.word(ipn - 1));
          wc = uniform(S.word(ipn));
        }
        uint16_t* u = reinterpret_cast<uint16_t*>(stab);
        u[hash32(wp, shift)] = (uint16_t)(ipn - 1);
        const uint32_t h2 = hash32(wc, shift);
        const uint32_t raw = u[h2];
        u[h2] = (uint16_t)ipn;
        tk = writelane(ip | ((ip - cand) << 16), ntok, tk);
        tl = writelane(f, ntok, tl);
        ++ntok;
        ip = ipn;
        next_emit = ip;
        if (__builtin_expect(ntok == kWave, 0)) {
          op = flush_copies(S, dst, op, base, ntok, tk, tl, lane);
          ntok = 0;
        }
        if (__builtin_expect((int32_t)ip >= ip_limit, 0)) break;
        cand = readlane(raw, 0);
      }
      if (__builtin_expect((int32_t)ip >= ip_limit, 0)) break;
    }
  }
  if (ntok) op = flush_copies(S, dst, op, base, ntok, tk, tl, lane);
  if (next_emit <= e) op = emit_literal_w(S, dst, op, next_emit, e - next_emit + 1, lane);
  if (lane == 0) a.out_len[b] = op;
}


__global__ __launch_bounds__(256) void k_gather(const uint8_t* __restrict__ src, const uint64_t* src_off,
                                                 const uint32_t* len, const uint64_t* dst_off,
                                                 uint8_t* __restrict__ dst) {
  const uint32_t b = blockIdx.x;
  const uint8_t* s = src + src_off[b];
  uint8_t* d = dst + dst_off[b];
  const uint32_t n = len[b];
  for (uint32_t k = threadIdx.x; k < n; k += blockDim.x) d[k] = s[k];
}

__global__ __launch_bounds__(256) void k_frag_plan(uint64_t n, uint32_t nfrag, uint64_t slot, uint64_t* in_off,
                                                   uint32_t* in_len, uint64_t* out_off) {
  const uint32_t f = blockIdx.x * blockDim.x + threadIdx.x;
  if (f >= nfrag) return;
  const uint64_t b = (uint64_t)f * kBlockSize;
  in_off[f] = b;
  in_len[f] = (uint32_t)min((uint64_t)kBlockSize, n - b);
  out_off[f] = (uint64_t)f * slot;
}

__device__ __attribute__((always_inline)) inline void gather_unit(const uint8_t* __restrict__ s8, uint32_t n,
                                                                 uint8_t* __restrict__ g, uint32_t y, uint32_t ny) {
  const uint4* s16 = reinterpret_cast<const uint4*>(s8);
  const uint32_t ad = (uint32_t)((uintptr_t)g & 15);
  const uint32_t u0 = ad ? 1u : 0u, u1 = (n + ad) >> 4;
  uint4* const g16 = reinterpret_cast<uint4*>(g - ad);
  const uint32_t sb = (16 - ad) & 15, dw = sb >> 2, bs = sb & 3;
  const uint32_t stride = blockDim.x * ny;
  for (uint32_t u = u0 + y * blockDim.x + threadIdx.x; u < u1; u += stride) {
    const uint32_t j = 16 * u - ad;
    const uint4 A = s16[j >> 4], B = sb ? s16[(j >> 4) + 1] : make_uint4(0, 0, 0, 0);
    const uint32_t x[8] = {A.x, A.y, A.z, A.w, B.x, B.y, B.z, B.w};
    uint32_t r5[5];
#pragma unroll
    for (int q = 0; q < 5; ++q) {
      uint32_t vv = x[q];
#pragma unroll
      for (int dd = 1; dd < 4; ++dd) vv = dw == (uint32_t)dd ? x[q + dd] : vv;
      r5[q] = vv;
    }
    g16[u] = make_uint4(__builtin_amdgcn_alignbyte(r5[1], r5[0], bs), __builtin_amdgcn_alignbyte(r5[2], r5[1], bs),
                        __builtin_amdgcn_alignbyte(r5[3], r5[2], bs), __builtin_amdgcn_alignbyte(r5[4], r5[3], bs));
  }
  if (y == 0) {
    const uint32_t nh = min(u0 ? 16 - ad : 0u, n);
    const uint32_t tb = max(16 * u1 > ad ? 16 * u1 - ad : 0u, nh);
    if (threadIdx.x < nh + (n - tb)) {
      const uint32_t jj = threadIdx.x < nh ? threadIdx.x : tb + (threadIdx.x - nh);
      g[jj] = s8[jj];
    }
  }
}

__global__ __launch_bounds__(256) void k_gather16(const uint8_t* __restrict__ src, const uint64_t* src_off,
                                                  const uint32_t* len, const uint32_t* in_len, uint32_t nfrag,
                                                  uint64_t* tot, uint8_t* __restrict__ dst) {
  __shared__ uint32_t sh[2];
  const uint32_t b = blockIdx.x;
  if (threadIdx.x < kWave) {
    const uint32_t l = threadIdx.x;
    const uint32_t L = l < nfrag ? len[l] : 0u;
    const bool bad = l < nfrag && (uint64_t)L > 32 + (uint64_t)in_len[l] + in_len[l] / 6;
    const uint32_t before = scan_dpp(l < b ? L : 0u);
    const uint32_t all = scan_dpp(bad ? 0u : L);
    const bool anybad = ballot(bad) != 0;
    if (l == 63) {
      sh[0] = before;
      sh[1] = anybad;
      if (b == 0 && blockIdx.y == 0) {
        tot[0] = all;
        tot[1] = anybad;
      }
    }
  }
  __syncthreads();
  if (sh[1]) return;
  gather_unit(src + src_off[b], len[b], dst + sh[0], blockIdx.y, gridDim.y);
}

__global__ __launch_bounds__(256) void k_gather_parts(const uint8_t* __restrict__ src, const uint64_t* out_off,
                                                      ScSpan sp, const uint8_t* __restrict__ in,
                                                      const uint64_t* in_off, const uint32_t* in_len, uint32_t nunit,
                                                      uint64_t* tot, uint8_t* __restrict__ dst) {
  __shared__ uint32_t wsum[4], ex[256], eff[256], code;
  const uint32_t t = threadIdx.x, lane = t & 63, w = t >> 6;
  const uint32_t L = t < nunit ? sp.part_len[t] : 0u;
  const uint32_t nb = t < nunit ? in_len[t / sp.parts] : 0u;
  const uint32_t lit = nb ? literal_tag_bytes(nb) + nb : 0u;
  const uint32_t bound = (t % sp.parts == 0) ? max((uint32_t)sp.pitch, lit + 5u) : (uint32_t)sp.pitch;
  const bool big = t < nunit && L > bound;
  const uint32_t Lv = big ? 0u : L;
  uint32_t sum = Lv;
  for (uint32_t d = 1; d < sp.parts; d <<= 1) sum += (uint32_t)__shfl_xor((int)sum, (int)d, 64);
  const bool over = t < nunit && nb && sum > lit;
  const uint32_t E = over ? (t % sp.parts == 0 ? lit : 0u) : Lv;
  const uint32_t inc = scan_dpp(E);
  const uint64_t anybig = ballot(big);
  if (t == 0) code = 0;
  if (lane == 63) wsum[w] = inc;
  __syncthreads();
  if (lane == 0 && anybig) code = 1;
  uint32_t pre = 0;
  for (uint32_t k = 0; k < w; ++k) pre += wsum[k];
  ex[t] = pre + inc - E;
  eff[t] = over ? 1u : 0u;
  __syncthreads();
  const uint32_t u = blockIdx.x;
  if (u == 0 && blockIdx.y == 0 && t == 0) {
    tot[0] = (uint64_t)wsum[0] + wsum[1] + wsum[2] + wsum[3];
    tot[1] = code;
  }
  if (code) return;
  const uint32_t b = u / sp.parts, j = u % sp.parts;
  uint8_t* const g = dst + ex[u];
  if (!eff[u]) {
    gather_unit(src + out_off[b] + (uint64_t)j * sp.pitch, sp.part_len[u], g, blockIdx.y, gridDim.y);
  } else if (j == 0) {
    const uint32_t n = in_len[b], tb = literal_tag_bytes(n);
    if (blockIdx.y == 0 && t < tb) {
      const uint32_t n1 = n - 1;
      g[t] = tb == 1 ? (uint8_t)(n1 << 2) : (t == 0 ? (uint8_t)((58 + tb) << 2) : (uint8_t)(n1 >> (8 * (t - 1))));
    }
    gather_unit(in + in_off[b], n, g + tb, blockIdx.y, gridDim.y);
  }
}

__global__ __launch_bounds__(256) void k_place(const uint8_t* __restrict__ src, const uint64_t* src_off,
                                               const uint32_t* len, const uint64_t* dst_off, uint32_t nfrag,
                                               uint64_t total, int header, uint64_t cap, uint8_t* __restrict__ dst,
                                               uint64_t* loc_off, int32_t* status) {
  const uint32_t b = blockIdx.x;
  if (header && b == 0 && blockIdx.y == 0) {
    const uint32_t hv = varint_len((uint32_t)total);
    if (threadIdx.x < hv && threadIdx.x < cap)
      dst[threadIdx.x] = (uint8_t)((((uint32_t)total >> (7 * threadIdx.x)) & 0x7f) | (threadIdx.x + 1 < hv ? 0x80 : 0));
  }
  if (b >= nfrag) return;
  const uint64_t base = header ? 0ull : dst_off[0];
  const uint32_t n = len[b];
  const uint64_t at = dst_off[b] - base;
  const bool bad = n >= kOutLenError || at > cap || cap - at < n || (header && at < varint_len((uint32_t)total));
  if (blockIdx.y == 0 && threadIdx.x == 0) {
    if (loc_off) loc_off[b] = at;
    if (bad && status) *status = kErrDevice;
  }
  if (bad) return;
  const uint8_t* const s = src + src_off[b];
  if (((uintptr_t)s & 15) == 0) {
    gather_unit(s, n, dst + at, blockIdx.y, gridDim.y);
  } else {
    for (uint32_t k = blockIdx.y * blockDim.x + threadIdx.x; k < n; k += blockDim.x * gridDim.y) dst[at + k] = s[k];
  }
}

hipError_t launch_place(const uint8_t* src, const uint64_t* src_off, const uint32_t* len, const uint64_t* dst_off,
                        uint32_t nfrag, uint64_t total, int header, uint64_t cap, uint8_t* dst, uint64_t* loc_off,
                        int32_t* status, hipStream_t s) {
  if (nfrag == 0 && !header) return hipSuccess;
  hipLaunchKernelGGL(k_place, dim3(max(nfrag, 1u), 4), dim3(256), 0, s, src, src_off, len, dst_off, nfrag, total, header,
                     cap, dst, loc_off, status);
  return hipGetLastError();
}

hipError_t launch_frag_plan(uint64_t n, uint32_t nfrag, uint64_t slot, uint64_t* in_off, uint32_t* in_len,
                            uint64_t* out_off, hipStream_t s) {
  hipLaunchKernelGGL(k_frag_plan, dim3((nfrag + 255) / 256), dim3(256), 0, s, n, nfrag, slot, in_off, in_len, out_off);
  return hipGetLastError();
}

hipError_t launch_parts_gather(const uint8_t* src, const uint64_t* out_off, const ScSpan& sp, const uint8_t* in,
                               const uint64_t* in_off, const uint32_t* in_len, uint32_t nblk, uint64_t* tot,
                               uint8_t* dst, hipStream_t s) {
  const uint32_t nunit = nblk * sp.parts;
  if (nblk == 0 || sp.parts == 0 || sp.parts > kWave || (sp.parts & (sp.parts - 1)) || nunit > 256)
    return hipErrorInvalidValue;
  hipLaunchKernelGGL(k_gather_parts, dim3(nunit, 4), dim3(256), 0, s, src, out_off, sp, in, in_off, in_len, nunit,
                     tot, dst);
  return hipGetLastError();
}

hipError_t launch_frag_gather(const uint8_t* src, const uint64_t* src_off, const uint32_t* out_len,
                              const uint32_t* in_len, uint32_t nfrag, uint64_t* tot, uint8_t* dst, hipStream_t s) {
  if (nfrag == 0 || nfrag > kWave) return hipErrorInvalidValue;
  hipLaunchKernelGGL(k_gather16, dim3(nfrag, 4), dim3(256), 0, s, src, src_off, out_len, in_len, nfrag, tot, dst);
  return hipGetLastError();
}


static uint32_t cu_count() {
  static uint32_t cache[64] = {};
  int dev = 0;
  if (hipGetDevice(&dev) != hipSuccess || dev < 0 || dev >= 64) dev = 0;
  uint32_t ncu = __atomic_load_n(&cache[dev], __ATOMIC_RELAXED);
  if (!ncu) {
    int v = 0;
    if (hipDeviceGetAttribute(&v, hipDeviceAttributeMultiprocessorCount, dev) != hipSuccess || v <= 0) v = 256;
    ncu = (uint32_t)v;
    __atomic_store_n(&cache[dev], ncu, __ATOMIC_RELAXED);
  }
  return ncu;
}

hipError_t launch_compress(const CompressArgs& a, int mode, hipStream_t s) {
  if (a.nblk == 0) return hipSuccess;
  if (mode != 0) return launch_compress_fast(a, mode, s);
  if (a.nblk <= cu_count())
    hipLaunchKernelGGL(k_compress_exact<true>, dim3(a.nblk), dim3(64), 0, s, a);
  else
    hipLaunchKernelGGL(k_compress_exact<false>, dim3(a.nblk), dim3(64), 0, s, a);
  return hipGetLastError();
}

hipError_t launch_gather(const uint8_t* src, const uint64_t* src_off, const uint32_t* len,
                         const uint64_t* dst_off, uint8_t* dst, uint32_t nblk, hipStream_t s) {
  if (nblk == 0) return hipSuccess;
  hipLaunchKernelGGL(k_gather, dim3(nblk), dim3(256), 0, s, src, src_off, len, dst_off, dst);
  return hipGetLastError();
}

}
```

### snappy.jl_amd/csrc/sm_compress_fast.hip

```cpp
#include "sm_device.h"
#include "sm_internal.h"

namespace sm {

constexpr uint32_t kScreenTodo = 0xfffffffeu;

constexpr uint32_t kScrMin = 8;
constexpr uint32_t kScrMinLen = 8192;
constexpr uint32_t kScrAnchorDiv = 256;
#ifndef SM_SCR_THREADS
#define SM_SCR_THREADS 512
#endif
#ifndef SM_SCR_FIRST
#define SM_SCR_FIRST 1
#endif
constexpr uint32_t kScrThreads = SM_SCR_THREADS;
constexpr uint32_t kScrPieces = kBlockSize / 16 / kScrThreads;
constexpr uint32_t kScrFirst = SM_SCR_FIRST;
constexpr uint32_t kScrTabBits = 12;
constexpr uint32_t kScrEmpty = 0xffffffffu;
static_assert(((kScrEmpty * kHashMul) >> 26) != 0, "the empty mark must not be an anchor word");

__device__ inline uint4 scr_load16(const uint8_t* src, uint32_t o, uint32_t n, bool aligned) {
  if (aligned && o + 16 <= n) return *reinterpret_cast<const uint4*>(src + o);
  uint32_t w[4] = {0, 0, 0, 0};
#pragma unroll
  for (uint32_t k = 0; k < 16; ++k)
    if (o + k < n) w[k >> 2] |= (uint32_t)src[o + k] << (8 * (k & 3));
  return make_uint4(w[0], w[1], w[2], w[3]);
}

__device__ inline uint32_t scr_anchors(uint32_t* tab, uint4 v, uint4 nv, uint32_t o, uint32_t n, bool nvalid,
                                       uint32_t& anc) {
  const uint32_t x[5] = {v.x, v.y, v.z, v.w, nv.x};
  uint32_t rep = 0;
#pragma unroll
  for (uint32_t j = 0; j < 16; ++j) {
    const uint32_t w = (j & 3) ? __builtin_amdgcn_alignbyte(x[(j >> 2) + 1], x[j >> 2], j & 3) : x[j >> 2];
    const uint32_t h = w * kHashMul;
    const bool ok = o + j + 4 <= n && (j < 13 || nvalid);
    if (ok && (h >> 26) == 0) {
      const uint32_t old = atomicExch(&tab[(h >> 14) & ((1u << kScrTabBits) - 1)], w);
      rep += old == w ? 1u : 0u;
      ++anc;
    }
  }
  return rep;
}

__global__ __launch_bounds__(kScrThreads) void k_literal_screen(CompressArgs a) {
  __shared__ uint32_t tab[1u << kScrTabBits];
  __shared__ uint32_t cnt[4];
  const uint32_t tid = threadIdx.x, lane = tid & 63u;
  const uint32_t b = blockIdx.x;
  uint32_t n;
  uint64_t ioff, ooff;
  if (a.plan_n) {
    ioff = (uint64_t)b * kBlockSize;
    n = (uint32_t)min((uint64_t)kBlockSize, a.plan_n - ioff);
    ooff = (uint64_t)b * a.plan_slot;
    if (tid == 0) {
      const_cast<uint64_t*>(a.in_off)[b] = ioff;
      const_cast<uint32_t*>(a.in_len)[b] = n;
      const_cast<uint64_t*>(a.out_off)[b] = ooff;
    }
  } else {
    n = a.in_len[b];
    ioff = a.in_off[b];
    ooff = a.out_off[b];
  }
  const uint8_t* src = a.in + ioff;
  uint8_t* dst = a.out + ooff;
  if (a.in_host && n <= kBlockSize) {
    src = a.in_host + ioff;
    uint8_t* const d = const_cast<uint8_t*>(a.in) + ioff;
    const bool al = (((uintptr_t)src | (uintptr_t)d) & 15) == 0;
    const uint32_t n16 = al ? n >> 4 : 0u;
    for (uint32_t k = tid; k < n16; k += kScrThreads)
      reinterpret_cast<uint4*>(d)[k] = reinterpret_cast<const uint4*>(src)[k];
    for (uint32_t k = 16 * n16 + tid; k < n; k += kScrThreads) d[k] = src[k];
  }
  if (n < kScrMinLen || n > kBlockSize) {
    if (tid == 0) a.out_len[b] = kScreenTodo;
    return;
  }
  const bool aligned = ((uintptr_t)src & 15) == 0;
  for (uint32_t k = tid; k < (1u << kScrTabBits); k += kScrThreads) tab[k] = kScrEmpty;
  if (tid < 4) cnt[tid] = 0;
  uint4 v[kScrPieces];
#pragma unroll
  for (uint32_t i = 0; i < kScrPieces; ++i) v[i] = make_uint4(0, 0, 0, 0);
  auto pass = [&](uint32_t i0, uint32_t i1, uint32_t slot) {
#pragma unroll
    for (uint32_t i = i0; i < i1; ++i) v[i] = scr_load16(src, 16 * (tid + kScrThreads * i), n, aligned);
    __syncthreads();
    uint32_t rep = 0, anc = 0;
#pragma unroll
    for (uint32_t i = i0; i < i1; ++i) {
      uint4 nv;
      nv.x = __builtin_amdgcn_update_dpp(0u, v[i].x, 0x130, 0xf, 0xf, false);
      rep += scr_anchors(tab, v[i], nv, 16 * (tid + kScrThreads * i), n, lane < 63, anc);
    }
    rep = __builtin_amdgcn_readlane(scan_dpp(rep), 63);
    anc = __builtin_amdgcn_readlane(scan_dpp(anc), 63);
    if (lane == 0 && rep) atomicAdd(&cnt[slot], rep);
    if (lane == 0 && anc) atomicAdd(&cnt[2 + slot], anc);
    __syncthreads();
  };
  pass(0, kScrFirst, 0);
  if (cnt[0] >= kScrMin) {
    if (tid == 0) a.out_len[b] = kScreenTodo;
    return;
  }
  if (n > 16 * kScrThreads * kScrFirst) pass(kScrFirst, kScrPieces, 1);
  const uint32_t scanned = min(n, n > 16 * kScrThreads * kScrFirst ? kBlockSize : 16 * kScrThreads * kScrFirst);
  if (cnt[0] + cnt[1] >= kScrMin || (cnt[2] + cnt[3]) * kScrAnchorDiv < scanned) {
    if (tid == 0) a.out_len[b] = kScreenTodo;
    return;
  }
  const uint32_t hv0 = a.header ? varint_len(n) : 0u;
  const uint32_t h = hv0 + literal_tag_bytes(n);
  const uint32_t ad = (uint32_t)((uintptr_t)dst & 15);
  const uint32_t m = (16u - ((ad + h) & 15u)) & 15u;
  uint4* d16 = reinterpret_cast<uint4*>(dst - ad);
  const uint32_t u_of_p0 = (m + ad + h) >> 4;
  const uint32_t dw = m >> 2, bs = m & 3u;
#pragma unroll
  for (uint32_t i = 0; i < kScrPieces; ++i) {
    const uint32_t p = tid + kScrThreads * i;
    const bool full = 16 * p + m + 16 <= n;
    uint4 nv;
    nv.x = __builtin_amdgcn_update_dpp(0u, v[i].x, 0x130, 0xf, 0xf, false);
    nv.y = __builtin_amdgcn_update_dpp(0u, v[i].y, 0x130, 0xf, 0xf, false);
    nv.z = __builtin_amdgcn_update_dpp(0u, v[i].z, 0x130, 0xf, 0xf, false);
    nv.w = __builtin_amdgcn_update_dpp(0u, v[i].w, 0x130, 0xf, 0xf, false);
    if (lane == 63 && full && m != 0) nv = scr_load16(src, 16 * (p + 1), n, aligned);
    if (full) {
      const uint32_t x[8] = {v[i].x, v[i].y, v[i].z, v[i].w, nv.x, nv.y, nv.z, nv.w};
      uint32_t r[5];
#pragma unroll
      for (int k = 0; k < 5; ++k) {
        uint32_t t = x[k];
#pragma unroll
        for (int d = 1; d < 4; ++d) t = dw == (uint32_t)d ? x[k + d] : t;
        r[k] = t;
      }
      d16[u_of_p0 + p] = make_uint4(__builtin_amdgcn_alignbyte(r[1], r[0], bs), __builtin_amdgcn_alignbyte(r[2], r[1], bs),
                                    __builtin_amdgcn_alignbyte(r[3], r[2], bs), __builtin_amdgcn_alignbyte(r[4], r[3], bs));
    }
  }
  const uint32_t nfull = n >= m + 16 ? (n - m) / 16 : 0u;
  const uint32_t headEnd = h + min(m, n);
  const uint32_t tailBeg = nfull ? h + m + 16 * nfull : headEnd;
  const uint32_t nh = headEnd, nt = h + n - tailBeg;
  for (uint32_t j = tid; j < nh + nt; j += kScrThreads) {
    const uint32_t jj = j < nh ? j : tailBeg + (j - nh);
    uint8_t c;
    if (jj < hv0) {
      c = (uint8_t)(((n >> (7 * jj)) & 0x7f) | (jj + 1 < hv0 ? 0x80 : 0));
    } else if (jj < h) {
      const uint32_t tb = h - hv0, k = jj - hv0;
      c = tb == 1 ? (uint8_t)((n - 1) << 2) : (k == 0 ? (uint8_t)((58 + tb) << 2) : (uint8_t)((n - 1) >> (8 * (k - 1))));
    } else {
      c = src[jj - h];
    }
    dst[jj] = c;
  }
  if (tid == 0) a.out_len[b] = h + n;
}


hipError_t launch_compress_fast(const CompressArgs& a0, int mode, hipStream_t s) {
  CompressArgs a = a0;
  a.screened = 1;
  hipLaunchKernelGGL(k_literal_screen, dim3(a.nblk), dim3(kScrThreads), 0, s, a);
  const hipError_t e = hipGetLastError();
  if (e != hipSuccess) return e;
  return launch_compress_sc(a, mode, s);
}

hipError_t launch_compress_span(const CompressArgs& a0, int mode, const ScSpan& sp, hipStream_t s) {
  if (mode != 1 && mode != 2) return hipErrorInvalidValue;
  CompressArgs a = a0;
  a.screened = 1;
  hipLaunchKernelGGL(k_literal_screen, dim3(a.nblk), dim3(kScrThreads), 0, s, a);
  const hipError_t e = hipGetLastError();
  if (e != hipSuccess) return e;
  return launch_compress_sc_span(a, mode, sp, s);
}

}
```

### snappy.jl_amd/csrc/sm_compress_sc.hip

```cpp
#include "sm_device.h"
#include "sm_internal.h"

namespace sm {

constexpr uint32_t kScreenTodoSc = 0xfffffffeu;

constexpr uint32_t kScS = 1024;
constexpr uint32_t kScC = kScS / 64;
constexpr uint32_t kScG = kScS / 64;
constexpr uint32_t kScW = 16;
constexpr uint32_t kScWorkers = kScW - 1;
#ifndef SC_RING
#define SC_RING 16
#endif
constexpr uint32_t kScRing = SC_RING;
static_assert((kScRing & (kScRing - 1)) == 0, "the span kernel's slot sequence needs a power of 2");
constexpr uint32_t kScSlot = 1088;
constexpr uint32_t kScThreads = 64 * kScW;
constexpr uint32_t kScTabBits = 13;
constexpr uint32_t kScTabWords = 1u << kScTabBits;
constexpr uint32_t kScExt = 17;
constexpr uint32_t kScMaxL = 255;
#ifndef SC_SPIN_BITS
#define SC_SPIN_BITS 22
#endif
constexpr uint32_t kScSpinMax = 1u << SC_SPIN_BITS;
static_assert(kScC == 16 && kScG == 16, "a lane's 16 positions: one u16 mask, one 16-byte row");

#ifndef SC_CB
#define SC_CB 2
#endif
#ifndef SC_FAR
#define SC_FAR 256
#endif
constexpr uint32_t kMaskPasses = 16;
#ifndef SC_WPRIO
#define SC_WPRIO 3
#endif
#ifndef SC_TPRIO
#define SC_TPRIO 3
#endif
#ifndef SC_TSLEEP
#define SC_TSLEEP 1
#endif
#ifndef SC_WSLEEP
#define SC_WSLEEP 1
#endif


struct ScWaveLds {
  uint8_t L[kScS];
  uint16_t O[kScS];
};
struct ScLds {
  uint8_t pre[16];
  uint8_t blk[kBlockSize + 64];
  uint32_t T[kScTabWords + 4];
  ScWaveLds w[kScWorkers];
  uint8_t ring[kScRing][kScSlot];
  uint32_t rsize[kScRing];
  uint32_t rseq[kScRing];
  uint32_t ins;
  uint32_t next;
  uint32_t err;
};
static_assert(sizeof(ScLds) <= 160 * 1024, "LDS");
static_assert(sizeof(ScWaveLds) % 32 == 0 && offsetof(ScLds, w) % 32 == 0 && offsetof(ScWaveLds, O) % 32 == 0,
              "rows are 32-byte aligned (section C's O addresses XOR the swizzle into bits 2..4)");
static_assert(kScSlot % 16 == 0 && offsetof(ScLds, ring) % 16 == 0, "slots are 16-byte aligned");
static_assert(kScSlot == kSpanSlot, "the host sizes part pitches by the staging slot");

template <typename Pred>
__device__ __attribute__((always_inline)) inline uint32_t sc_wait(uint32_t* p, Pred pred, uint32_t& err, uint32_t code) {
  uint32_t v;
  for (uint32_t it = 0; !pred(v = uniform(__hip_atomic_load(p, __ATOMIC_ACQUIRE, __HIP_MEMORY_SCOPE_WORKGROUP))); ++it) {
    if (it > kScSpinMax) {
      err |= code;
      break;
    }
    if (SC_WSLEEP) __builtin_amdgcn_s_sleep(SC_WSLEEP);
  }
  return v;
}


__device__ inline uint32_t sc_ld32(const uint8_t* blk, uint32_t a) { return *reinterpret_cast<const uint32_t*>(blk + a); }


__device__ inline uint32_t sc_abyte(uint32_t hi, uint32_t lo, uint32_t s) { return __builtin_amdgcn_alignbyte(hi, lo, s); }

__device__ inline uint32_t sc_ld32u(const uint8_t* blk, uint32_t p) {
  const uint32_t* w = reinterpret_cast<const uint32_t*>(blk + (p & ~3u));
  return sc_abyte(w[1], w[0], p);
}

__device__ inline uint4 sc_ld128(const uint8_t* blk, uint32_t p) {
  const uint32_t* w = reinterpret_cast<const uint32_t*>(blk + (p & ~3u));
  const uint32_t s = p;
  const uint32_t w0 = w[0], w1 = w[1], w2 = w[2], w3 = w[3], w4 = w[4];
  return make_uint4(__builtin_amdgcn_alignbyte(w1, w0, s), __builtin_amdgcn_alignbyte(w2, w1, s),
                    __builtin_amdgcn_alignbyte(w3, w2, s), __builtin_amdgcn_alignbyte(w4, w3, s));
}

__device__ inline uint32_t sc_diff8(uint32_t a0, uint32_t a1, uint32_t b0, uint32_t b1) {
  const uint64_t d = ((uint64_t)(a1 ^ b1) << 32) | (a0 ^ b0);
  return d ? (uint32_t)__builtin_ctzll(d) >> 3 : 8u;
}

__device__ inline uint4 sc_trim(uint4 v, uint32_t len) {
  const uint64_t mlo = len >= 8 ? ~0ull : (1ull << (8 * (len & 7))) - 1;
  const uint64_t mhi = len >= 16 ? ~0ull : (len <= 8 ? 0ull : (1ull << (8 * (len & 7))) - 1);
  return make_uint4(v.x & (uint32_t)mlo, v.y & (uint32_t)(mlo >> 32), v.z & (uint32_t)mhi, v.w & (uint32_t)(mhi >> 32));
}

__device__ inline uint4 sc_trim1(uint4 v, uint32_t len) {
  uint32_t l8 = len << 3;
  asm("" : "+v"(l8));
  uint64_t mlo, mhi;
  asm("v_lshrrev_b64 %0, %1, -1" : "=v"(mlo) : "v"(64 - min(l8, 64u)));
  asm("v_lshrrev_b64 %0, %1, -1" : "=v"(mhi) : "v"(128 - l8));
  const bool hi = len > 8;
  return make_uint4(v.x & (uint32_t)mlo, v.y & (uint32_t)(mlo >> 32), hi ? v.z & (uint32_t)mhi : 0u,
                    hi ? v.w & (uint32_t)(mhi >> 32) : 0u);
}

__device__ inline void sc_lds_or(uint32_t a, uint4 v) {
  const uint32_t wa = (a - 1u) & ~3u, t = 0u - a;
  const uint32_t u0 = __builtin_amdgcn_alignbyte(v.x, 0u, t);
  const uint32_t u1 = __builtin_amdgcn_alignbyte(v.y, v.x, t);
  const uint32_t u2 = __builtin_amdgcn_alignbyte(v.z, v.y, t);
  const uint32_t u3 = __builtin_amdgcn_alignbyte(v.w, v.z, t);
  const uint32_t u4 = __builtin_amdgcn_alignbyte(0u, v.w, t);
  asm volatile("ds_or_b32 %0, %1\nds_or_b32 %0, %2 offset:4\nds_or_b32 %0, %3 offset:8\nds_or_b32 %0, %4 offset:12\n"
               "ds_or_b32 %0, %5 offset:16"
               : : "v"(wa), "v"(u0), "v"(u1), "v"(u2), "v"(u3), "v"(u4) : "memory");
}

__device__ inline void sc_lds_orn(uint32_t a, uint4 v, uint32_t nb) {
  const uint32_t wa = (a - 1u) & ~3u, t = 0u - a, d = a - wa;
  const uint32_t u0 = __builtin_amdgcn_alignbyte(v.x, 0u, t);
  const uint32_t u1 = __builtin_amdgcn_alignbyte(v.y, v.x, t);
  asm volatile("ds_or_b32 %0, %1" : : "v"(wa), "v"(u0) : "memory");
  asm volatile("ds_or_b32 %0, %1 offset:4" : : "v"(wa), "v"(u1) : "memory");
  if (d + nb > 8) {
    const uint32_t u2 = __builtin_amdgcn_alignbyte(v.z, v.y, t);
    const uint32_t u3 = __builtin_amdgcn_alignbyte(v.w, v.z, t);
    const uint32_t u4 = __builtin_amdgcn_alignbyte(0u, v.w, t);
    asm volatile("ds_or_b32 %0, %1 offset:8\nds_or_b32 %0, %2 offset:12\nds_or_b32 %0, %3 offset:16"
                 : : "v"(wa), "v"(u2), "v"(u3), "v"(u4) : "memory");
  }
}

__device__ inline void sc_lds_or3(uint32_t a, uint32_t cv, uint32_t cs = 3) {
  const uint32_t wa = (a - 1u) & ~3u, t = 0u - a;
  const uint32_t lo = __builtin_amdgcn_alignbyte(cv, 0u, t), hi = __builtin_amdgcn_alignbyte(0u, cv, t);
  asm volatile("ds_or_b32 %0, %1\nds_or_b32 %0, %2 offset:4" : : "v"(wa), "v"(lo), "v"(hi) : "memory");
}

__device__ inline uint4 sc_prepend(uint4 v, uint32_t tag, uint32_t t) {
  if (t == 0) return v;
  const uint32_t s = 4 - t;
  return make_uint4(__builtin_amdgcn_alignbyte(v.x, tag << (8 * s), s), __builtin_amdgcn_alignbyte(v.y, v.x, s),
                    __builtin_amdgcn_alignbyte(v.z, v.y, s), __builtin_amdgcn_alignbyte(v.w, v.z, s));
}

__device__ inline uint32_t sc_lit_tag(uint32_t len, uint32_t& sz) {
  const uint32_t l1 = len - 1;
  sz = len <= 60 ? 1u : (len <= 256 ? 2u : 3u);
  return sz == 1 ? (l1 << 2) : (sz == 2 ? (60u << 2) | (l1 << 8) : (61u << 2) | (l1 << 8));
}

__device__ inline uint32_t sc_hash_bucket(uint32_t w) {
  uint32_t h;
  asm("v_bfe_u32 %0, %1, %2, %3" : "=v"(h) : "v"(w * kHashMul), "n"(32 - kScTabBits), "n"(kScTabBits));
  return h;
}

__device__ inline uint32_t sc_select(uint64_t m, uint32_t a, uint32_t b) {
  uint32_t r;
  asm("v_cndmask_b32_e64 %0, %1, %2, %3" : "=v"(r) : "v"(b), "v"(a), "s"(m));
  return r;
}

__device__ inline uint32_t sc_sel(uint32_t c, uint32_t a, uint32_t b) { return c ? a : b; }

__device__ inline uint32_t sc_copy_piece(uint32_t off, uint32_t L, uint32_t& sz) {
  const bool c1 = L < 12 && off < 2048;
  sz = c1 ? 2u : 3u;
  const uint32_t e1 = (1u + ((L - 4) << 2) + ((off >> 3) & 0xe0u)) | ((off & 0xffu) << 8);
  const uint32_t e2 = (2u + ((L - 1) << 2)) | (off << 8);
  return sc_sel(c1, e1, e2);
}

__device__ inline uint32_t sc_extend(const uint8_t* blk, uint32_t q, uint32_t off, uint32_t L, uint32_t cap) {
  for (;;) {
    const uint4 x = sc_ld128(blk, q + L), y = sc_ld128(blk, q + L - off);
    const uint32_t f0 = sc_diff8(x.x, x.y, y.x, y.y);
    const uint32_t fb = f0 < 8 ? f0 : 8u + sc_diff8(x.z, x.w, y.z, y.w);
    L = min(L + fb, cap);
    if (fb < 16 || L >= cap) return L;
  }
}

__device__ inline uint32_t sc_copy_bytes(uint32_t off, uint32_t L) {
  const uint32_t t = L - 1, n = t >> 6;
  return n + 2 * n + (((t & 63) < 11 && off < 2048) ? 2u : 3u);
}

__device__ inline uint32_t sc_ffbl(uint32_t x) {
  uint32_t r;
  asm("v_ffbl_b32 %0, %1" : "=v"(r) : "v"(x));
  return r;
}

__device__ __attribute__((always_inline)) inline uint32_t sc_eq16(uint32_t X0, uint32_t X1, uint32_t X2, uint32_t X3,
                                                                  const uint32_t* w, uint32_t s) {
  const uint32_t a0 = w[0], a1 = w[1], a2 = w[2], a3 = w[3], a4 = w[4];
  const uint32_t b0 = sc_ffbl(X0 ^ __builtin_amdgcn_alignbyte(a1, a0, s));
  const uint32_t b1 = sc_ffbl(X1 ^ __builtin_amdgcn_alignbyte(a2, a1, s)) | 32u;
  const uint32_t b2 = sc_ffbl(X2 ^ __builtin_amdgcn_alignbyte(a3, a2, s)) | 64u;
  const uint32_t b3 = sc_ffbl(X3 ^ __builtin_amdgcn_alignbyte(a4, a3, s)) | 96u;
  return min(min(b0, b1), min(min(b2, b3), 128u)) >> 3;
}


__device__ __attribute__((always_inline)) inline uint32_t sc_eq12x(const uint8_t* blk, uint32_t x, uint32_t y) {
  const uint32_t* a = reinterpret_cast<const uint32_t*>(blk + (x & ~3u));
  const uint32_t* b = reinterpret_cast<const uint32_t*>(blk + (y & ~3u));
  const uint32_t a0 = a[0], a1 = a[1], a2 = a[2], a3 = a[3];
  const uint32_t b0 = b[0], b1 = b[1], b2 = b[2], b3 = b[3];
  const uint32_t f0 = sc_ffbl(sc_abyte(a1, a0, x) ^ sc_abyte(b1, b0, y));
  const uint32_t f1 = sc_ffbl(sc_abyte(a2, a1, x) ^ sc_abyte(b2, b1, y)) | 32u;
  const uint32_t f2 = sc_ffbl(sc_abyte(a3, a2, x) ^ sc_abyte(b3, b2, y)) | 64u;
  return min(min(f0, f1), min(f2, 104u)) >> 3;
}

__device__ inline uint32_t scan_max_dpp(uint32_t v) {
  v = max(v, (uint32_t)__builtin_amdgcn_update_dpp(0u, v, 0x111, 0xf, 0xf, true));
  v = max(v, (uint32_t)__builtin_amdgcn_update_dpp(0u, v, 0x112, 0xf, 0xf, true));
  v = max(v, (uint32_t)__builtin_amdgcn_update_dpp(0u, v, 0x114, 0xf, 0xf, true));
  v = max(v, (uint32_t)__builtin_amdgcn_update_dpp(0u, v, 0x118, 0xf, 0xf, true));
  v = max(v, (uint32_t)__builtin_amdgcn_update_dpp(0u, v, 0x142, 0xa, 0xf, false));
  v = max(v, (uint32_t)__builtin_amdgcn_update_dpp(0u, v, 0x143, 0xc, 0xf, false));
  return v;
}

__device__ inline uint32_t sc_bits(uint32_t a, uint32_t b) { return ((1u << b) - 1u) & ~((1u << a) - 1u); }

struct ScToks {
  uint32_t t[4];
  uint32_t n;
};

__device__ __attribute__((always_inline)) inline uint32_t sc_next_block(const CompressArgs& a, uint32_t from, uint32_t lane) {
  for (uint32_t b0 = from; b0 < a.nblk; b0 += 64 * gridDim.x) {
    const uint32_t bb = b0 + lane * gridDim.x;
    const bool todo = bb < a.nblk && (!a.screened || a.out_len[bb] == kScreenTodoSc);
    const uint64_t m = ballot(todo);
    if (m) return b0 + ctz64(m) * gridDim.x;
  }
  return a.nblk;
}

template <int kDense>
__device__ __attribute__((always_inline)) inline void sc_superchunk(ScLds& S, const uint32_t k, const uint32_t n,
                                                                   const uint32_t wave, const uint32_t lane_in) {
  uint32_t lane = lane_in;
  asm volatile("" : "+v"(lane));
  ScWaveLds& Wl = S.w[wave];
  const uint32_t sc0 = k * kScS, sce = min(sc0 + kScS, n);
  const uint32_t Tbase = lds_addr(S.T);
  uint32_t ha[kScG], hvv[kScG], wq[kScG];
  const uint32_t ql = sc0 + lane, qa = ql & ~3u, qb = ql;
  const uint32_t hv0 = ql, hv1 = ql << 16;
#pragma unroll
  for (int g = 0; g < (int)kScG; ++g) {
    const uint32_t w = sc_abyte(sc_ld32(S.blk, qa + 64 * g + 4), sc_ld32(S.blk, qa + 64 * g), qb);
    wq[g] = w;
    ha[g] = Tbase + 4 * sc_hash_bucket(w);
    hvv[g] = (g & 1) ? hv1 + ((64u * g) << 16) : hv0 + 64u * g;
  }
  if (sc0 + kScS + 3 > n) {
    asm volatile("");
#pragma unroll
    for (int g = 0; g < (int)kScG; ++g) ha[g] = ql + 64 * g + 4 <= n ? ha[g] : Tbase + 4 * kScTabWords;
  }
  const uint32_t mk0 = 0xffffu, mk1 = 0xffff0000u;
  __builtin_amdgcn_s_setprio(SC_TPRIO);
  for (uint32_t it = 0; uniform(__hip_atomic_load(&S.ins, __ATOMIC_RELAXED, __HIP_MEMORY_SCOPE_WORKGROUP)) != k; ++it) {
    if (it > kScSpinMax) {
      S.err |= 1;
      break;
    }
    if (SC_TSLEEP) __builtin_amdgcn_s_sleep(SC_TSLEEP);
  }
  __builtin_amdgcn_s_setprio(3);
  const uint32_t tok_a = lds_addr(&S.ins), tok_v = k + 1;
  uint32_t r[kScG];
  asm volatile(
      "ds_mskor_rtn_b32 %0, %16, %32, %34\n"
      "ds_mskor_rtn_b32 %1, %17, %33, %35\n"
      "ds_mskor_rtn_b32 %2, %18, %32, %36\n"
      "ds_mskor_rtn_b32 %3, %19, %33, %37\n"
      "ds_mskor_rtn_b32 %4, %20, %32, %38\n"
      "ds_mskor_rtn_b32 %5, %21, %33, %39\n"
      "ds_mskor_rtn_b32 %6, %22, %32, %40\n"
      "ds_mskor_rtn_b32 %7, %23, %33, %41\n"
      "ds_mskor_rtn_b32 %8, %24, %32, %42\n"
      "ds_mskor_rtn_b32 %9, %25, %33, %43\n"
      "ds_mskor_rtn_b32 %10, %26, %32, %44\n"
      "ds_mskor_rtn_b32 %11, %27, %33, %45\n"
      "ds_mskor_rtn_b32 %12, %28, %32, %46\n"
      "ds_mskor_rtn_b32 %13, %29, %33, %47\n"
      "ds_mskor_rtn_b32 %14, %30, %32, %48\n"
      "ds_mskor_rtn_b32 %15, %31, %33, %49\n"
      "ds_write_b32 %50, %51\n"
      "s_waitcnt lgkmcnt(0)"
      : "=&v"(r[0]), "=&v"(r[1]), "=&v"(r[2]), "=&v"(r[3]), "=&v"(r[4]), "=&v"(r[5]), "=&v"(r[6]), "=&v"(r[7]),
        "=&v"(r[8]), "=&v"(r[9]), "=&v"(r[10]), "=&v"(r[11]), "=&v"(r[12]), "=&v"(r[13]), "=&v"(r[14]), "=&v"(r[15])
      : "v"(ha[0]), "v"(ha[1]), "v"(ha[2]), "v"(ha[3]), "v"(ha[4]), "v"(ha[5]), "v"(ha[6]), "v"(ha[7]), "v"(ha[8]),
        "v"(ha[9]), "v"(ha[10]), "v"(ha[11]), "v"(ha[12]), "v"(ha[13]), "v"(ha[14]), "v"(ha[15]), "v"(mk0), "v"(mk1),
        "v"(hvv[0]), "v"(hvv[1]), "v"(hvv[2]), "v"(hvv[3]), "v"(hvv[4]), "v"(hvv[5]), "v"(hvv[6]), "v"(hvv[7]),
        "v"(hvv[8]), "v"(hvv[9]), "v"(hvv[10]), "v"(hvv[11]), "v"(hvv[12]), "v"(hvv[13]), "v"(hvv[14]), "v"(hvv[15]),
        "v"(tok_a), "v"(tok_v)
      : "memory");
  __builtin_amdgcn_s_setprio(0);

  uint64_t mbs[kScG];
  uint8_t* const Ob8 = reinterpret_cast<uint8_t*>(Wl.O);
  const uint32_t Orel = 32 * (lane >> 4) + 2 * (lane & 15);
  if constexpr (kDense) {
#pragma unroll
    for (int g = 0; g < (int)kScG; ++g) {
      const uint32_t q = sc0 + 64 * g + lane;
      const uint32_t sh = 16 * (g & 1);
      const uint32_t ca = (r[g] >> sh) & 0xffffu, cb = (r[g] >> (16 - sh)) & 0xffffu;
      const uint32_t c1 = max(ca, cb), c2 = min(ca, cb);
      const bool ok1 = c1 < q;
      const uint32_t d1 = q - c1, d2 = q - c2;
      uint16_t* const Og = reinterpret_cast<uint16_t*>(Ob8 + (Orel ^ (4u * (g & 7))) + 128u * g);
      const uint32_t r4 = 4 * g + (lane >> 4), i = lane & 15;
      const uint4 X = sc_ld128(S.blk, q);
      uint32_t lw1 = sc_eq16(X.x, X.y, X.z, X.w, reinterpret_cast<const uint32_t*>(S.blk + (c1 & ~3u)), c1);
      uint32_t lw2 = sc_eq16(X.x, X.y, X.z, X.w, reinterpret_cast<const uint32_t*>(S.blk + (c2 & ~3u)), c2);
      asm("" : "+v"(lw1), "+v"(lw2));
      const uint32_t l1 = ok1 ? lw1 : 0u, l2 = ok1 ? lw2 : 0u;
      const bool take2 = l2 == l1 ? (l2 >= 4 && d1 < (uint32_t)SC_FAR) : l2 > l1;
      const uint32_t l = take2 ? l2 : l1;
      const uint32_t avail = sce - q;
      const uint32_t enc = l < 4 ? 0u : ((l == 16 && avail > 16) ? kScExt : min(l, avail));
      *Og = (uint16_t)(take2 ? d2 : d1);
      Wl.L[16 * r4 + 4 * ((i >> 2) ^ ((g >> 1) & 3)) + (i & 3)] = (uint8_t)enc;
      mbs[g] = ballot(l >= 4);
    }
  } else {
#pragma unroll
    for (int g0 = 0; g0 < (int)kScG; g0 += SC_CB) {
      uint32_t c1s[SC_CB], c2s[SC_CB], v1s[SC_CB], v2s[SC_CB];
#pragma unroll
      for (int j = 0; j < SC_CB; ++j) {
        const int g = g0 + j;
        const uint32_t sh = 16 * (g & 1);
        const uint32_t ca = (r[g] >> sh) & 0xffffu, cb = (r[g] >> (16 - sh)) & 0xffffu;
        c1s[j] = max(ca, cb);
        c2s[j] = min(ca, cb);
        v1s[j] = sc_ld32u(S.blk, c1s[j]);
        v2s[j] = sc_ld32u(S.blk, c2s[j]);
      }
#pragma unroll
      for (int j = 0; j < SC_CB; ++j) asm("" : "+v"(v1s[j]), "+v"(v2s[j]));
#pragma unroll
      for (int j = 0; j < SC_CB; ++j) {
        const int g = g0 + j;
        const uint32_t q = sc0 + 64 * g + lane;
        const uint32_t c1 = c1s[j], c2 = c2s[j], w = wq[g];
        const bool ok1 = c1 < q;
        const uint32_t d1 = q - c1, d2 = q - c2;
        uint16_t* const Og = reinterpret_cast<uint16_t*>(Ob8 + (Orel ^ (4u * (g & 7))) + 128u * g);
        const uint64_t OK = ballot(ok1);
        const uint64_t M1 = ballot(v1s[j] == w) & OK, M2 = ballot(v2s[j] == w) & OK;
        const uint64_t U = M2 & (~M1 | ballot(d1 < (uint32_t)SC_FAR));
        *Og = (uint16_t)sc_select(U, d2, d1);
        mbs[g] = M1 | M2;
      }
    }
  }
  uint32_t mdw = 0;
#define SC_WL(g)                                                                                  \
  asm volatile("v_writelane_b32 %0, %1, %2" : "+v"(mdw) : "s"((uint32_t)mbs[g]), "n"(2 * (g)));   \
  asm volatile("v_writelane_b32 %0, %1, %2" : "+v"(mdw) : "s"((uint32_t)(mbs[g] >> 32)), "n"(2 * (g) + 1));
  SC_WL(0) SC_WL(1) SC_WL(2) SC_WL(3) SC_WL(4) SC_WL(5) SC_WL(6) SC_WL(7)
  SC_WL(8) SC_WL(9) SC_WL(10) SC_WL(11) SC_WL(12) SC_WL(13) SC_WL(14) SC_WL(15)
#undef SC_WL
  __atomic_signal_fence(__ATOMIC_SEQ_CST);

  const uint32_t c0 = sc0 + kScC * lane;
  const uint32_t ce = c0 < sce ? min(c0 + kScC, sce) : c0;
  const uint32_t nroom = c0 + 3 < sce ? min(sce - c0 - 3, 16u) : 0u;
  const uint32_t mask16 = (__shfl(mdw, (int)(lane >> 1), 64) >> (16 * (lane & 1))) & ((1u << nroom) - 1u);
  const uint32_t osw2 = ((lane >> 2) & 7) << 1, lsw4 = ((lane >> 3) & 3) << 2;
  const uint16_t* const Orow = Wl.O + 16 * lane;
  auto offAt = [&](uint32_t i) -> uint32_t { return Orow[i ^ osw2]; };
  uint8_t* const Lrow = Wl.L + 16 * lane;
  uint32_t xpos = 16, xlen = 0;
  auto walk = [&](auto kStop, uint32_t sr, uint32_t stop, uint32_t& path, uint32_t& mpos, uint32_t& pend)
      __attribute__((always_inline)) {
    const uint32_t m0 = sr < 16 ? mask16 >> sr : 0u;
    uint32_t i = sr + sc_ffbl(m0);
    path = 0;
    mpos = 16;
    uint32_t last = 16, lastL = 0;
    bool act = m0 != 0;
    while (act) {
      if constexpr (decltype(kStop)::value) {
        if ((stop >> i) & 1u) {
          mpos = i;
          break;
        }
      }
      path |= 1u << i;
      last = i;
      uint32_t enc;
      if constexpr (kDense) {
        enc = Lrow[i ^ lsw4];
      } else {
        const uint32_t q = c0 + i, off = offAt(i);
        const uint32_t p = q - off;
        enc = min(4u + sc_eq12x(S.blk + 4, q, p), sce - q);
        Lrow[i ^ lsw4] = (uint8_t)enc;
      }
      lastL = enc;
      const uint32_t t = i + min(enc, 16u);
      const uint32_t m = mask16 >> t;
      i = t + sc_ffbl(m);
      act = m != 0;
    }
    pend = ce;
    if (last < 16) {
      uint32_t L = lastL;
      const bool ext = L == kScExt;
      if (last + min(L, 16u) >= 16) {
        if (ballot(ext)) {
          if (ext) {
            if (xpos != last) {
              xlen = sc_extend(S.blk, c0 + last, offAt(last), 16u, min(kScMaxL, sce - (c0 + last)));
              xpos = last;
            }
            L = xlen;
          }
        }
        pend = c0 + last + L;
      }
    }
  };
  const bool row = c0 < sce;
  uint32_t s = c0, e, P;
  {
    uint32_t mp;
    walk(std::false_type{}, row ? 0u : 16u, 0u, P, mp, e);
    if (!row) e = c0;
  }
  for (uint32_t pass = 0;; ++pass) {
    const uint32_t pe = __builtin_amdgcn_update_dpp(0u, scan_max_dpp(e), 0x138, 0xf, 0xf, false);
    const uint32_t st = lane == 0 ? sc0 : pe;
    uint32_t sn = st;
    bool chg = st != s;
    if (!ballot(chg)) break;
    if (pass < kMaskPasses) {
      uint64_t cov = ballot(st >= ce);
      for (int it = 0; cov && it < 3; ++it) {
        const uint32_t x = sn >= ce ? 0u : e;
        const uint32_t pm = __builtin_amdgcn_update_dpp(0u, scan_max_dpp(x), 0x138, 0xf, 0xf, false);
        sn = lane == 0 ? sc0 : pm;
        const uint64_t c = ballot(sn >= ce);
        if (c == cov) break;
        cov = c;
      }
      chg = sn != s;
      if (!ballot(chg)) {
        sn = st;
        chg = st != s;
      }
    }

    const bool inrow = chg && sn < ce;
    uint32_t nP, mp, ne;
    walk(std::true_type{}, inrow ? sn - c0 : 16u, P, nP, mp, ne);
    if (chg) {
      s = sn;
      if (!inrow) {
        P = 0;
        e = sn;
      } else if (mp == 16) {
        P = nP;
        e = ne;
      } else {
        P = nP | (P & ~sc_bits(0, mp));
      }
    }
  }
  auto getL = [&](uint32_t i) -> uint32_t { return Lrow[i ^ lsw4]; };
  ScToks tk;
  {
    uint32_t pm = P;
    tk.n = (uint32_t)__builtin_popcount(P);
#pragma unroll
    for (int j = 0; j < 4; ++j) {
      const uint32_t i = pm ? (uint32_t)__builtin_ctz(pm) : 0u;
      pm &= pm - 1;
      uint32_t L = getL(i);
      L = L == kScExt ? xlen : L;
      const uint32_t off = offAt(i);
      tk.t[j] = off | (L << 16) | (i << 24);
    }
  }

  const bool live = s >= c0 && s < ce;
  uint32_t lead = 0, body = 0, trail = 0;
  {
    uint32_t p = s;
#pragma unroll
    for (int j = 0; j < 4; ++j) {
      const bool has = (uint32_t)j < tk.n;
      const uint32_t tv = tk.t[j];
      const uint32_t q = c0 + (tv >> 24), L = (tv >> 16) & 0xffu, run = q - p;
      if (j == 0)
        lead = sc_sel(has, run, 0u);
      else
        body += sc_sel(has && run, run + 1, 0u);
      body += sc_sel(has, sc_copy_bytes(tv & 0xffffu, L), 0u);
      p = sc_sel(has, q + L, p);
    }
    trail = (live && p < ce) ? ce - p : 0u;
    lead = tk.n == 0 ? trail : lead;
  }
  const uint32_t ptrail = __builtin_amdgcn_update_dpp(0u, trail, 0x138, 0xf, 0xf, false);
  const bool cont = ptrail > 0 && lead > 0;
  const bool mid = cont && tk.n == 0;
  const uint32_t Cs = scan_dpp(cont ? lead : 0u);
  const uint64_t above = ballot(!mid) & (~1ull << lane);
  const uint32_t fn = above ? ctz64(above) : 63u;
  const uint32_t Cf = __shfl(Cs, fn, 64);
  const bool starts = trail > 0 && !mid;
  const uint32_t merged = starts ? trail + Cf - Cs : 0u;
  uint32_t mts;
  (void)sc_lit_tag(merged ? merged : 1u, mts);
  uint32_t size;
  if (tk.n == 0)
    size = lead == 0 ? 0u : (cont ? lead : mts + trail);
  else
    size = (lead ? (cont ? lead : 1u + lead) : 0u) + body + (trail ? mts + trail : 0u);
  const uint32_t incl = scan_dpp(size);
  const uint32_t total = readlane(incl, 63);

  const uint32_t slot = k % kScRing;
  (void)sc_wait(&S.rseq[slot], [&](uint32_t v) { return v == k; }, S.err, 2u);

  uint8_t* const stg = S.ring[slot];
  {
    for (uint32_t u = lane; 16 * u < total; u += 64) reinterpret_cast<uint4*>(stg)[u] = make_uint4(0, 0, 0, 0);
    const uint32_t stga = lds_addr(stg);
    uint32_t at = incl - size, p = s;
#pragma unroll
    for (int j = 0; j < 4; ++j) {
      if ((uint32_t)j < tk.n) {
        const uint32_t tv = tk.t[j];
        const uint32_t q = c0 + (tv >> 24), L = (tv >> 16) & 0xffu, off = tv & 0xffffu;
        const uint32_t run = q - p;
        const uint32_t ts = (j == 0 && cont) ? 0u : 1u;
        const uint32_t len = run ? ts + run : 0u;
        if (ballot(len != 0)) {
          uint4 v = sc_ld128(S.blk - 4, p + 3);
          v.x = ts ? ((v.x & ~0xffu) | ((run - 1) << 2)) : v.x;
          if (run) sc_lds_orn(stga + at + ts - 1u, sc_trim1(v, run + 1), run + 1);
        }
        at += len;
        if (L <= 64) {
          uint32_t cs;
          const uint32_t cv = sc_copy_piece(off, L, cs);
          sc_lds_or3(stga + at, cv, cs);
          at += cs;
        } else {
          uint32_t R = L;
          while (R >= 68) {
            sc_lds_or3(stga + at, (2u + (63u << 2)) | (off << 8));
            at += 3;
            R -= 64;
          }
          if (R > 64) {
            sc_lds_or3(stga + at, (2u + (59u << 2)) | (off << 8));
            at += 3;
            R -= 60;
          }
          uint32_t cs;
          const uint32_t cv = sc_copy_piece(off, R, cs);
          sc_lds_or3(stga + at, cv, cs);
          at += cs;
        }
        p = q + L;
      }
    }
    if (live && p < ce) {
      const uint32_t run = ce - p;
      uint32_t tag = 0, ts = 0;
      if (!(tk.n == 0 && cont)) tag = sc_lit_tag(merged, ts);
      sc_lds_orn(stga + at, sc_trim(sc_prepend(sc_ld128(S.blk, p), tag, ts), min(ts + run, 16u)), min(ts + run, 16u));
      if (ts + run > 16) sc_lds_or(stga + at + 16, sc_trim(sc_ld128(S.blk, p + 16 - ts), ts + run - 16));
    }
  }
  __hip_atomic_store(&S.rsize[slot], total + 1, __ATOMIC_RELEASE, __HIP_MEMORY_SCOPE_WORKGROUP);
}

__device__ __attribute__((always_inline)) inline void sc_copy_out(uint8_t* const g, const uint8_t* stg, uint32_t len,
                                                                 uint32_t lane) {
  const uint32_t ad = (uint32_t)((uintptr_t)g & 15);
  const uint32_t u0 = ad ? 1u : 0u, u1 = (len + ad) >> 4;
  uint4* const g16 = reinterpret_cast<uint4*>(g - ad);
  const uint32_t* const s32 = reinterpret_cast<const uint32_t*>(stg);
  for (uint32_t u = u0 + lane; u < u1; u += 64) {
    const uint32_t j = 16 * u - ad;
    const uint32_t* w = s32 + (j >> 2);
    const uint32_t r0 = w[0], r1 = w[1], r2 = w[2], r3 = w[3], r4 = w[4];
    g16[u] = make_uint4(__builtin_amdgcn_alignbyte(r1, r0, j), __builtin_amdgcn_alignbyte(r2, r1, j),
                        __builtin_amdgcn_alignbyte(r3, r2, j), __builtin_amdgcn_alignbyte(r4, r3, j));
  }
  const uint32_t nh = min(u0 ? 16 - ad : 0u, len);
  const uint32_t tb = max(16 * u1 > ad ? 16 * u1 - ad : 0u, nh);
  const uint32_t nt = len - tb;
  if (lane < nh + nt) {
    const uint32_t jj = lane < nh ? lane : tb + (lane - nh);
    g[jj] = stg[jj];
  }
}

__device__ __attribute__((always_inline)) inline void sc_writer(ScLds& S, uint32_t n, uint8_t* const dst, uint32_t hv,
                                                               uint32_t k0, uint32_t k1, bool whole,
                                                               uint32_t* len_out, uint32_t lane) {
  uint32_t o = hv, err = 0;
  uint32_t vpre = 0;
  for (uint32_t k = k0; k < k1; ++k) {
    const uint32_t slot = k % kScRing;
    const uint32_t sz =
        (vpre ? vpre : sc_wait(&S.rsize[slot], [](uint32_t v) { return v != 0; }, err, 4u)) - 1;
    if (err) break;
    vpre = k + 1 < k1 ? uniform(__hip_atomic_load(&S.rsize[(k + 1) % kScRing], __ATOMIC_ACQUIRE,
                                                    __HIP_MEMORY_SCOPE_WORKGROUP))
                        : 0u;
    sc_copy_out(dst + o, S.ring[slot], sz, lane);
    o += sz;
    __hip_atomic_store(&S.rsize[slot], 0u, __ATOMIC_RELAXED, __HIP_MEMORY_SCOPE_WORKGROUP);
    __hip_atomic_store(&S.rseq[slot], k + kScRing, __ATOMIC_RELEASE, __HIP_MEMORY_SCOPE_WORKGROUP);
  }
  const uint32_t h = hv + (n ? literal_tag_bytes(n) : 0u);
  if (whole && !err && n && o > h + n) {
    uint8_t* const g = dst + hv;
    const uint32_t tb = h - hv, len = tb + n;
    const uint32_t ad = (uint32_t)((uintptr_t)g & 15);
    uint4* const g16 = reinterpret_cast<uint4*>(g - ad);
    const uint32_t u1 = (len + ad) >> 4;
    const uint32_t ua = (tb + ad + 15) >> 4;
    for (uint32_t u = ua + lane; u < u1; u += 64) g16[u] = sc_ld128(S.blk, 16 * u - ad - tb);
    const uint32_t he = ua < u1 ? 16 * ua - ad : len;
    const uint32_t te = ua < u1 ? 16 * u1 - ad : len;
    for (uint32_t j = lane; j < he + (len - te); j += 64) {
      const uint32_t jj = j < he ? j : te + (j - he);
      uint8_t c;
      if (jj < tb) {
        c = tb == 1 ? (uint8_t)((n - 1) << 2) : (jj == 0 ? (uint8_t)((58 + tb) << 2) : (uint8_t)((n - 1) >> (8 * (jj - 1))));
      } else {
        c = S.blk[jj - tb];
      }
      g[jj] = c;
    }
    o = h + n;
  }
  err |= uniform(__hip_atomic_load(&S.err, __ATOMIC_RELAXED, __HIP_MEMORY_SCOPE_WORKGROUP));
  if (lane == 0) *len_out = err ? 0xfff00000u | err : o;
}

template <int kDense>
__global__ __launch_bounds__(kScThreads) void k_compress_sc(CompressArgs a) {
  __shared__ __attribute__((aligned(16))) ScLds S;
  const uint32_t tid = threadIdx.x;
  const uint32_t wave = uniform(tid >> 6);
  const uint32_t lane = tid & 63;
  static_assert(kBlockSize / 16 / kScThreads == 4, "four 16-byte pieces per thread of a full block");
  uint4 pf0, pf1, pf2, pf3;
  uint32_t b = sc_next_block(a, blockIdx.x, lane);
  uint32_t n = 0;
  const uint8_t* src = nullptr;
  bool inpf = false;
#define SC_FETCH(bb)                                                              \
  {                                                                               \
    n = (bb) < a.nblk ? a.in_len[bb] : 0u;                                        \
    src = (bb) < a.nblk ? a.in + a.in_off[bb] : nullptr;                          \
    inpf = (bb) < a.nblk && n == kBlockSize && ((uintptr_t)src & 15) == 0;        \
    if (inpf) {                                                                   \
      const uint4* s16 = reinterpret_cast<const uint4*>(src);                     \
      pf0 = s16[tid];                                                             \
      pf1 = s16[tid + kScThreads];                                                \
      pf2 = s16[tid + 2 * kScThreads];                                            \
      pf3 = s16[tid + 3 * kScThreads];                                            \
    }                                                                             \
  }
  SC_FETCH(b)
  while (b < a.nblk) {
    uint8_t* const dst = a.out + a.out_off[b];
    if (n > kBlockSize) {
      if (tid == 0) a.out_len[b] = 0xffffffffu;
      b = sc_next_block(a, b + gridDim.x, lane);
      SC_FETCH(b)
      continue;
    }
    if (inpf) {
      uint4* d16 = reinterpret_cast<uint4*>(S.blk);
      d16[tid] = pf0;
      d16[tid + kScThreads] = pf1;
      d16[tid + 2 * kScThreads] = pf2;
      d16[tid + 3 * kScThreads] = pf3;
    } else if (((uintptr_t)src & 15) == 0) {
      const uint4* s16 = reinterpret_cast<const uint4*>(src);
      uint4* d16 = reinterpret_cast<uint4*>(S.blk);
      const uint32_t n16 = n >> 4;
      for (uint32_t k = tid; k < n16; k += kScThreads) d16[k] = s16[k];
      for (uint32_t k = (n & ~15u) + tid; k < n; k += kScThreads) S.blk[k] = src[k];
    } else {
      for (uint32_t k = tid; k < n; k += kScThreads) S.blk[k] = src[k];
    }
    if (tid < 64) S.blk[n + tid] = 0;
    {
      uint4* t16 = reinterpret_cast<uint4*>(S.T);
      for (uint32_t k = tid; k < 4 * kScTabWords / 16; k += kScThreads) t16[k] = make_uint4(0, 0, 0, 0);
    }
    const uint32_t hv = a.header ? varint_len(n) : 0u;
    if (tid < hv) dst[tid] = (uint8_t)(((n >> (7 * tid)) & 0x7f) | (tid + 1 < hv ? 0x80 : 0));
    if (wave == 0) {
      if (lane < kScRing) {
        S.rsize[lane] = 0;
        S.rseq[lane] = lane;
      }
      if (lane == 0) {
        S.ins = 0;
        S.next = 0;
        S.err = 0;
      }
    }
    const uint32_t bn = sc_next_block(a, b + gridDim.x, lane);
    __syncthreads();

    const uint32_t nsc = (n + kScS - 1) / kScS;
    if (wave == kScWorkers) {
      __builtin_amdgcn_s_setprio(SC_WPRIO);
      sc_writer(S, n, dst, hv, 0, nsc, true, &a.out_len[b], lane);
      __builtin_amdgcn_s_setprio(0);
    } else {
      for (;;) {
        const uint32_t k = uniform(__hip_atomic_fetch_add(&S.next, 1u, __ATOMIC_RELAXED, __HIP_MEMORY_SCOPE_WORKGROUP)) >> 6;
        if (k >= nsc) break;
        sc_superchunk<kDense>(S, k, n, wave, lane);
      }
    }
    SC_FETCH(bn)
    __syncthreads();
    b = bn;
  }
#undef SC_FETCH
}

template <int kDense>
__global__ __launch_bounds__(kScThreads) void k_compress_sc_span(CompressArgs a, ScSpan sp) {
  __shared__ __attribute__((aligned(16))) ScLds S;
  const uint32_t tid = threadIdx.x;
  const uint32_t wave = uniform(tid >> 6);
  const uint32_t lane = tid & 63;
  const uint32_t b = blockIdx.x / sp.parts, j = blockIdx.x % sp.parts;
  if (b >= a.nblk) return;
  uint32_t* const plen = sp.part_len + blockIdx.x;
  const uint32_t n = a.in_len[b];
  if (n > kBlockSize) {
    if (tid == 0) *plen = j == 0 ? 0xffffffffu : 0u;
    return;
  }
  const uint32_t nsc = (n + kScS - 1) / kScS;
  const uint32_t k0 = j * sp.span, k1 = min(k0 + sp.span, nsc);
  const bool todo = !a.screened || a.out_len[b] == kScreenTodoSc;
  if (!todo || k0 >= k1) {
    if (tid == 0) *plen = (!todo && j == 0) ? a.out_len[b] : 0u;
    return;
  }
  const uint8_t* const src = a.in + a.in_off[b];
  uint8_t* const dst = a.out + a.out_off[b] + (uint64_t)j * sp.pitch;
  if (((uintptr_t)src & 15) == 0) {
    const uint4* s16 = reinterpret_cast<const uint4*>(src);
    uint4* d16 = reinterpret_cast<uint4*>(S.blk);
    const uint32_t n16 = n >> 4;
    for (uint32_t k = tid; k < n16; k += kScThreads) d16[k] = s16[k];
    for (uint32_t k = (n & ~15u) + tid; k < n; k += kScThreads) S.blk[k] = src[k];
  } else {
    for (uint32_t k = tid; k < n; k += kScThreads) S.blk[k] = src[k];
  }
  if (tid < 64) S.blk[n + tid] = 0;
  {
    uint4* t16 = reinterpret_cast<uint4*>(S.T);
    for (uint32_t k = tid; k < 4 * kScTabWords / 16; k += kScThreads) t16[k] = make_uint4(0, 0, 0, 0);
  }
  const uint32_t hv = (a.header && j == 0) ? varint_len(n) : 0u;
  if (tid < hv) dst[tid] = (uint8_t)(((n >> (7 * tid)) & 0x7f) | (tid + 1 < hv ? 0x80 : 0));
  if (wave == 0) {
    if (lane < kScRing) {
      S.rsize[lane] = 0;
      S.rseq[lane] = k0 + ((lane - k0) & (kScRing - 1));
    }
    if (lane == 0) {
      S.ins = k0;
      S.next = 64 * k0;
      S.err = 0;
    }
  }
  __syncthreads();
  const uint32_t pe = kScS * k0;
  const uint32_t sub = lane & 15, gq = lane >> 4;
  for (int ph = 1; ph >= 0; --ph) {
    for (uint32_t i = wave; 128 * (4 * i) < pe; i += kScW) {
      const uint32_t G = 2 * (4 * i + gq) + (uint32_t)ph;
      const uint32_t q = 64 * G + 4 * sub;
      if (q >= pe) continue;
      const uint32_t d0 = sc_ld32(S.blk, q), d1 = sc_ld32(S.blk, q + 4);
      uint32_t* t[4];
#pragma unroll
      for (uint32_t j = 0; j < 4; ++j) {
        const uint32_t w = j ? __builtin_amdgcn_alignbyte(d1, d0, j) : d0;
        t[j] = &S.T[(w * kHashMul) >> (32 - kScTabBits)];
      }
      if (ph) {
#pragma unroll
        for (uint32_t j = 0; j < 4; ++j)
          if (q + j + 4 <= n) __hip_atomic_fetch_max(t[j], (q + j) << 16, __ATOMIC_RELAXED, __HIP_MEMORY_SCOPE_WORKGROUP);
      } else {
        uint32_t hi[4];
#pragma unroll
        for (uint32_t j = 0; j < 4; ++j) hi[j] = __hip_atomic_load(t[j], __ATOMIC_RELAXED, __HIP_MEMORY_SCOPE_WORKGROUP);
#pragma unroll
        for (uint32_t j = 0; j < 4; ++j)
          if (q + j + 4 <= n)
            __hip_atomic_fetch_max(t[j], (hi[j] & 0xffff0000u) | (q + j), __ATOMIC_RELAXED, __HIP_MEMORY_SCOPE_WORKGROUP);
      }
    }
    __syncthreads();
  }
  if (wave == kScWorkers) {
    __builtin_amdgcn_s_setprio(SC_WPRIO);
    sc_writer(S, n, dst, hv, k0, k1, false, plen, lane);
    __builtin_amdgcn_s_setprio(0);
  } else {
    for (;;) {
      const uint32_t k = uniform(__hip_atomic_fetch_add(&S.next, 1u, __ATOMIC_RELAXED, __HIP_MEMORY_SCOPE_WORKGROUP)) >> 6;
      if (k >= k1) break;
      sc_superchunk<kDense>(S, k, n, wave, lane);
    }
  }
}

hipError_t launch_compress_sc_span(const CompressArgs& a, int mode, const ScSpan& sp, hipStream_t s) {
  if (sp.parts == 0 || sp.span == 0 || sp.parts * sp.span < (kBlockSize + kScS - 1) / kScS ||
      sp.pitch < (uint64_t)sp.span * kScSlot)
    return hipErrorInvalidValue;
  const uint32_t grid = a.nblk * sp.parts;
  if (grid == 0) return hipSuccess;
  if (mode == 2)
    hipLaunchKernelGGL(k_compress_sc_span<1>, dim3(grid), dim3(kScThreads), 0, s, a, sp);
  else
    hipLaunchKernelGGL(k_compress_sc_span<0>, dim3(grid), dim3(kScThreads), 0, s, a, sp);
  return hipGetLastError();
}


hipError_t launch_compress_sc(const CompressArgs& a, int mode, hipStream_t s) {
  static uint32_t ncu_cache[64] = {};
  int dev = 0;
  if (hipGetDevice(&dev) != hipSuccess || dev < 0 || dev >= 64) dev = 0;
  uint32_t ncu = __atomic_load_n(&ncu_cache[dev], __ATOMIC_RELAXED);
  if (!ncu) {
    int v = 0;
    if (hipDeviceGetAttribute(&v, hipDeviceAttributeMultiprocessorCount, dev) != hipSuccess || v <= 0) v = 256;
    ncu = (uint32_t)v;
    __atomic_store_n(&ncu_cache[dev], ncu, __ATOMIC_RELAXED);
  }
  const uint32_t grid = min(a.nblk, ncu);
  if (mode == 2)
    hipLaunchKernelGGL(k_compress_sc<1>, dim3(grid), dim3(kScThreads), 0, s, a);
  else
    hipLaunchKernelGGL(k_compress_sc<0>, dim3(grid), dim3(kScThreads), 0, s, a);
  return hipGetLastError();
}

}
```

### snappy.jl_amd/csrc/sm_internal.h

```cpp
#pragma once
#include <hip/hip_runtime.h>
#include <stdint.h>

namespace sm {

struct CompressArgs {
  const uint8_t* in;
  const uint64_t* in_off;
  const uint32_t* in_len;
  uint8_t* out;
  const uint64_t* out_off;
  uint32_t* out_len;
  uint32_t nblk;
  uint32_t table_size;
  int header;
  int screened;
  uint64_t plan_n = 0;
  uint64_t plan_slot = 0;
  const uint8_t* in_host = nullptr;
};

struct DecompressArgs {
  const uint8_t* in;
  const uint64_t* in_off;
  const uint32_t* in_len;
  uint8_t* out;
  const uint64_t* out_off;
  const uint32_t* out_cap;
  uint32_t* out_len;
  int32_t* status;
  uint32_t nblk;
  int raw;
  uint32_t one_n = 0;
  uint32_t one_cap = 0;
};

hipError_t launch_compress(const CompressArgs& a, int mode, hipStream_t s);
hipError_t launch_compress_fast(const CompressArgs& a, int mode, hipStream_t s);
hipError_t launch_compress_sc(const CompressArgs& a, int mode, hipStream_t s);
hipError_t launch_decompress(const DecompressArgs& a, int large, hipStream_t s);

constexpr uint32_t kIdxChunk = 4096;
constexpr uint32_t kIdxEntries = 64;
constexpr uint32_t kSmallChunk = 1024;
constexpr uint32_t kSmallChunkFine = 512;
constexpr uint32_t kSmallChunkTiny = 128;
#ifndef SM_SMALL_HOPS
#define SM_SMALL_HOPS 1024
#endif
constexpr uint32_t kSmallHops = SM_SMALL_HOPS;
constexpr uint32_t kOneLaunchHops = 256u << 10;
constexpr uint32_t kDeepLevels = 4;
constexpr uint32_t kDeepChains = 4;
constexpr uint32_t kIdxPad = 288;
struct StreamFrag {
  uint32_t y;
  uint32_t O;
  uint32_t F;
  uint32_t lim;
};
hipError_t launch_validate(const uint8_t* in, const uint64_t* in_off, const uint32_t* in_len, uint32_t nblk,
                           int32_t* status, hipStream_t s);
hipError_t launch_uncompressed_length(const uint8_t* in, const uint64_t* in_off, const uint32_t* in_len,
                                      uint32_t nblk, uint32_t* out_len, int32_t* status, hipStream_t s);
hipError_t launch_stream_index(const uint8_t* in, uint32_t N, uint32_t ip0, uint32_t nchunks, uint32_t* rec,
                               hipStream_t s);
hipError_t launch_decompress_frags(const uint8_t* in, uint32_t N, uint32_t size, uint8_t* out,
                                   const StreamFrag* frags, uint32_t nfrag, int32_t* status, hipStream_t s);
struct OriginPath {
  uint32_t y, ex, O, out;
};
hipError_t launch_origin_fill(const uint8_t* in, uint32_t N, uint32_t size, const OriginPath* path, uint32_t npath,
                              uint32_t* P, int32_t* status, hipStream_t s);
hipError_t launch_path_check(const uint8_t* in, uint32_t N, uint32_t size, const OriginPath* path, uint32_t npath,
                             int32_t* status, hipStream_t s);
hipError_t launch_origin_resolve(uint32_t* P, uint32_t size, uint32_t* pending, hipStream_t s);
hipError_t launch_small_decode(const uint8_t* in, const uint8_t* in_host, uint32_t N, uint32_t ip0, uint32_t size, uint32_t chunk,
                               uint32_t nchunks, uint32_t* rec, OriginPath* path, uint32_t* ctl, uint32_t* P,
                               uint32_t rounds, uint32_t hops, uint8_t* out, uint32_t* words, hipStream_t s);
hipError_t launch_to_host(const uint8_t* src, uint32_t n, uint8_t* dst, const uint32_t* wsrc, uint32_t nw,
                          uint32_t* words, hipStream_t s);
constexpr uint32_t kLitSpans = 16;
struct LitSpans {
  uint32_t src[kLitSpans];
  uint32_t dst[kLitSpans + 1];
  uint32_t n;
};
hipError_t launch_literal_spans(const uint8_t* in, const LitSpans& sp, uint8_t* out, uint32_t* words, hipStream_t s);
hipError_t launch_origin_gather(const uint8_t* in, const uint32_t* P, uint32_t size, uint8_t* out, hipStream_t s);
hipError_t launch_frag_plan(uint64_t n, uint32_t nfrag, uint64_t slot, uint64_t* in_off, uint32_t* in_len,
                            uint64_t* out_off, hipStream_t s);
constexpr uint32_t kSpanSlot = 1088;
struct ScSpan {
  uint32_t parts, span;
  uint64_t pitch;
  uint32_t* part_len;
};
hipError_t launch_compress_span(const CompressArgs& a, int mode, const ScSpan& sp, hipStream_t s);
hipError_t launch_compress_sc_span(const CompressArgs& a, int mode, const ScSpan& sp, hipStream_t s);
hipError_t launch_parts_gather(const uint8_t* src, const uint64_t* out_off, const ScSpan& sp, const uint8_t* in,
                               const uint64_t* in_off, const uint32_t* in_len, uint32_t nblk, uint64_t* tot,
                               uint8_t* dst, hipStream_t s);
hipError_t launch_frag_gather(const uint8_t* src, const uint64_t* src_off, const uint32_t* out_len,
                              const uint32_t* in_len, uint32_t nfrag, uint64_t* tot, uint8_t* dst, hipStream_t s);
hipError_t launch_place(const uint8_t* src, const uint64_t* src_off, const uint32_t* len, const uint64_t* dst_off,
                        uint32_t nfrag, uint64_t total, int header, uint64_t cap, uint8_t* dst, uint64_t* loc_off,
                        int32_t* status, hipStream_t s);
hipError_t launch_gather(const uint8_t* src, const uint64_t* src_off, const uint32_t* len,
                         const uint64_t* dst_off, uint8_t* dst, uint32_t nblk, hipStream_t s);

}
```

Measured before the change: 390.3 GB/s.

## Split tail-wave remainder blocks into parts across idle CUs in batch compress

When the block count is not a multiple of the compress grid (CU count), the leftover blocks that would form a partial last wave are split into several superchunk-range parts. Each part is compressed by a separate workgroup into scratch, inside the same kernel launch as the whole blocks, and a gather kernel then concatenates the parts or falls back to a literal encoding. This targets tail-wave imbalance where few CUs process the last blocks alone. In exchange it adds a screening kernel, a gather pass, per-stream scratch buffers and more complex dispatch. The copy-out in the superchunk writer is also simplified to use unaligned 16-byte stores.

```diff
diff --git a/include/snappy_mi355x.h b/include/snappy_mi355x.h
--- a/include/snappy_mi355x.h
+++ b/include/snappy_mi355x.h
@@ -59,6 +59,8 @@
                                        const uint32_t* d_in_len, uint32_t nblk, uint8_t* d_out,
                                        const uint64_t* d_out_off, uint32_t* d_out_len, uint64_t total_len,
                                        int mode, void* stream);
+void sm_batch_parts_plan(uint32_t nblk, uint32_t grid, uint32_t* rem, uint32_t* parts);
+int sm_ctx_last_batch_parts(sm_ctx* ctx);
 sm_status sm_place_fragments_device(sm_ctx* ctx, const uint8_t* d_src, const uint64_t* d_src_off,
                                     const uint32_t* d_len, uint32_t nfrag, const uint64_t* d_dst_off,
                                     uint64_t total_len, int write_header, uint8_t* d_dst, uint64_t dst_capacity,
diff --git a/snappy.jl_amd/__init__.py b/snappy.jl_amd/__init__.py
--- a/snappy.jl_amd/__init__.py
+++ b/snappy.jl_amd/__init__.py
@@ -18,7 +18,8 @@
     "sm_status_message", "sm_max_compressed_length", "sm_uncompressed_length", "sm_parse32",
     "sm_encode32", "sm_ctx_create", "sm_ctx_destroy", "sm_ctx_stream", "sm_compress", "sm_uncompress",
     "sm_compress_batch_device", "sm_uncompress_batch_device", "sm_compress_batch",
-    "sm_uncompress_batch", "sm_version", "sm_compress_fragments_device", "sm_ctx_last_path", "sm_ctx_set_small_decode",
+    "sm_uncompress_batch", "sm_version", "sm_compress_fragments_device", "sm_batch_parts_plan",
+    "sm_ctx_last_batch_parts", "sm_ctx_last_path", "sm_ctx_set_small_decode",
     "sm_ctx_set_split_compress", "sm_ctx_last_compress_split",
     "sm_find_match_length", "sm_validate_batch_device", "sm_uncompressed_length_batch_device",
     "sm_validate_compressed_buffer", "sm_compress_batch_sharded", "sm_uncompress_batch_sharded",
@@ -102,6 +103,10 @@
     L.sm_version.argtypes = []
     L.sm_compress_fragments_device.restype = i32
     L.sm_compress_fragments_device.argtypes = [vp, vp, vp, vp, u32, vp, vp, vp, ctypes.c_uint64, ctypes.c_int, vp]
+    L.sm_ctx_last_batch_parts.restype = ctypes.c_int
+    L.sm_ctx_last_batch_parts.argtypes = [vp]
+    L.sm_batch_parts_plan.restype = None
+    L.sm_batch_parts_plan.argtypes = [u32, u32, ctypes.POINTER(u32), ctypes.POINTER(u32)]
     L.sm_validate_batch_device.restype = i32
     L.sm_validate_batch_device.argtypes = [vp, vp, vp, vp, u32, vp, vp]
     L.sm_uncompressed_length_batch_device.restype = i32
@@ -394,6 +399,16 @@
         raise SnappyError(st)
 
 
+def batch_parts_plan(nblk, grid):
+    rem, parts = ctypes.c_uint32(0), ctypes.c_uint32(0)
+    lib().sm_batch_parts_plan(int(nblk), int(grid), ctypes.byref(rem), ctypes.byref(parts))
+    return rem.value, parts.value
+
+
+def last_batch_parts(device=0):
+    return lib().sm_ctx_last_batch_parts(context(device))
+
+
 def uncompress_batch_device(d_in, d_in_off, d_in_len, d_out, d_out_off, d_out_cap, d_out_len, d_status,
                             stream=None, device=None):
     import torch
diff --git a/snappy.jl_amd/csrc/sm_api.hip b/snappy.jl_amd/csrc/sm_api.hip
--- a/snappy.jl_amd/csrc/sm_api.hip
+++ b/snappy.jl_amd/csrc/sm_api.hip
@@ -83,6 +83,15 @@
   bool split = true;
   bool last_split = false;
   std::mutex mu;
+  static constexpr int kPartStreams = 8;
+  struct PartScratch {
+    hipStream_t stream = nullptr;
+    DevBuf buf;
+  };
+  PartScratch part[kPartStreams];
+  int nparts = 0;
+  std::mutex part_mu;
+  std::atomic<int> last_parts{0};
 };
 
 #ifndef SM_SMALL_BODY8
@@ -700,6 +709,7 @@
     ctx->idx.release();
     ctx->gat.release();
     ctx->org.release();
+    for (int i = 0; i < ctx->nparts; ++i) ctx->part[i].buf.release();
     ctx->stage.release();
     ctx->stage_in.release();
     if (ctx->in_ev) (void)hipEventDestroy(ctx->in_ev);
@@ -714,6 +724,53 @@
 }
 
 void* sm_ctx_stream(sm_ctx* ctx) { return ctx ? (void*)ctx->stream : nullptr; }
+
+namespace {
+
+bool batch_parts_enabled() {
+  static const bool on = [] {
+    const char* e = getenv("SM_BATCH_PARTS");
+    return !(e && e[0] == '0' && e[1] == 0);
+  }();
+  return on;
+}
+
+uint8_t* batch_parts_buffer(sm_ctx* ctx, hipStream_t s) {
+  for (int i = 0; i < ctx->nparts; ++i)
+    if (ctx->part[i].stream == s) return (uint8_t*)ctx->part[i].buf.p;
+  if (ctx->nparts == sm_ctx::kPartStreams) return nullptr;
+  hipStreamCaptureStatus cap = hipStreamCaptureStatusNone;
+  if (hipStreamIsCapturing(s, &cap) != hipSuccess || cap != hipStreamCaptureStatusNone) {
+    (void)hipGetLastError();
+    return nullptr;
+  }
+  sm_ctx::PartScratch& ps = ctx->part[ctx->nparts];
+  if (ps.buf.ensure(sm::batch_parts_scratch(sm::compress_grid())) != hipSuccess) {
+    (void)hipGetLastError();
+    return nullptr;
+  }
+  ps.stream = s;
+  ++ctx->nparts;
+  return (uint8_t*)ps.buf.p;
+}
+
+hipError_t compress_device(sm_ctx* ctx, const sm::CompressArgs& a, int mode, hipStream_t s) {
+  if (mode != SM_MODE_REFERENCE && batch_parts_enabled()) {
+    const sm::BatchParts bp = sm::batch_parts_rule(a.nblk, sm::compress_grid());
+    if (bp.rem) {
+      std::lock_guard<std::mutex> lk(ctx->part_mu);
+      uint8_t* const scratch = batch_parts_buffer(ctx, s);
+      if (scratch) {
+        ctx->last_parts.store((int)bp.rem, std::memory_order_relaxed);
+        return sm::launch_compress_batch_parts(a, mode, bp, scratch, s);
+      }
+    }
+  }
+  ctx->last_parts.store(0, std::memory_order_relaxed);
+  return sm::launch_compress(a, mode, s);
+}
+
+}
 
 sm_status sm_compress_batch_device(sm_ctx* ctx, const uint8_t* d_in, const uint64_t* d_in_off,
                                    const uint32_t* d_in_len, uint32_t nblk, uint8_t* d_out,
@@ -723,7 +780,7 @@
   if (!d_in || !d_in_off || !d_in_len || !d_out || !d_out_off || !d_out_len) return SM_ERR_ARGUMENT;
   DeviceGuard g(ctx->device);
   sm::CompressArgs a{d_in, d_in_off, d_in_len, d_out, d_out_off, d_out_len, nblk, 0, 1};
-  SM_CHECK(sm::launch_compress(a, mode, (hipStream_t)stream));
+  SM_CHECK(compress_device(ctx, a, mode, (hipStream_t)stream));
   return SM_OK;
 }
 
@@ -737,8 +794,16 @@
   if (!d_in || !d_in_off || !d_in_len || !d_out || !d_out_off || !d_out_len) return SM_ERR_ARGUMENT;
   DeviceGuard g(ctx->device);
   sm::CompressArgs a{d_in, d_in_off, d_in_len, d_out, d_out_off, d_out_len, nblk, sm::hashtable_size(total_len), 0};
-  SM_CHECK(sm::launch_compress(a, mode, (hipStream_t)stream));
-  return SM_OK;
+  SM_CHECK(compress_device(ctx, a, mode, (hipStream_t)stream));
+  return SM_OK;
+}
+
+int sm_ctx_last_batch_parts(sm_ctx* ctx) { return ctx ? ctx->last_parts.load(std::memory_order_relaxed) : -1; }
+
+void sm_batch_parts_plan(uint32_t nblk, uint32_t grid, uint32_t* rem, uint32_t* parts) {
+  const sm::BatchParts bp = sm::batch_parts_rule(nblk, grid);
+  if (rem) *rem = bp.rem;
+  if (parts) *parts = bp.parts;
 }
 
 sm_status sm_place_fragments_device(sm_ctx* ctx, const uint8_t* d_src, const uint64_t* d_src_off,
diff --git a/snappy.jl_amd/csrc/sm_compress.hip b/snappy.jl_amd/csrc/sm_compress.hip
--- a/snappy.jl_amd/csrc/sm_compress.hip
+++ b/snappy.jl_amd/csrc/sm_compress.hip
@@ -431,6 +431,54 @@
   }
 }
 
+__global__ __launch_bounds__(256) void k_gather_parts(CompressArgs a, const uint8_t* __restrict__ src, ScSpan sp) {
+  const uint32_t b = blockIdx.x / sp.parts, j = blockIdx.x % sp.parts, t = threadIdx.x;
+  const uint32_t* const pl = sp.part_len + b * sp.parts;
+  if (pl[0] == kPartScreened) return;
+  const bool first = j == 0 && blockIdx.y == 0;
+  uint32_t sum = 0, before = 0, mark = 0;
+  for (uint32_t i = 0; i < sp.parts; ++i) {
+    const uint32_t L = pl[i];
+    if (L >= kOutLenError)
+      mark |= L;
+    else if (L > sp.pitch)
+      mark |= kOutLenError | 8u;
+    else {
+      sum += L;
+      before += i < j ? L : 0u;
+    }
+  }
+  if (mark) {
+    if (first && t == 0) a.out_len[b] = mark;
+    return;
+  }
+  const uint32_t n = a.in_len[b];
+  uint8_t* const dst = a.out + a.out_off[b];
+  const uint32_t hv = a.header ? varint_len(n) : 0u;
+  if (n == 0) {
+    if (first && t == 0) {
+      if (hv) dst[0] = 0;
+      a.out_len[b] = hv;
+    }
+    return;
+  }
+  const uint32_t tb = literal_tag_bytes(n), lit = hv + tb + n;
+  if (sum <= lit) {
+    gather_unit(src + b * sp.blk_pitch + j * sp.pitch, pl[j], dst + before, blockIdx.y, gridDim.y);
+    if (first && t == 0) a.out_len[b] = sum;
+    return;
+  }
+  if (j) return;
+  if (blockIdx.y == 0) {
+    const uint32_t n1 = n - 1;
+    if (t < hv) dst[t] = (uint8_t)(((n >> (7 * t)) & 0x7f) | (t + 1 < hv ? 0x80 : 0));
+    if (t < tb) dst[hv + t] = tb == 1 ? (uint8_t)(n1 << 2) : (t == 0 ? (uint8_t)((58 + tb) << 2) : (uint8_t)(n1 >> (8 * (t - 1))));
+    if (t == 0) a.out_len[b] = lit;
+  }
+  const uint8_t* const in = a.in + a.in_off[b];
+  for (uint32_t k = blockIdx.y * blockDim.x + t; k < n; k += blockDim.x * gridDim.y) dst[hv + tb + k] = in[k];
+}
+
 __global__ __launch_bounds__(256) void k_place(const uint8_t* __restrict__ src, const uint64_t* src_off,
                                                const uint32_t* len, const uint64_t* dst_off, uint32_t nfrag,
                                                uint64_t total, int header, uint64_t cap, uint8_t* __restrict__ dst,
@@ -482,6 +530,12 @@
     return hipErrorInvalidValue;
   hipLaunchKernelGGL(k_gather_parts, dim3(nunit, 4), dim3(256), 0, s, src, out_off, sp, in, in_off, in_len, nunit,
                      tot, dst);
+  return hipGetLastError();
+}
+
+hipError_t launch_batch_parts_gather(const CompressArgs& a, const uint8_t* src, const ScSpan& sp, hipStream_t s) {
+  if (a.nblk == 0 || sp.parts == 0 || sp.blk_pitch == 0) return hipErrorInvalidValue;
+  k_gather_parts<<<dim3(a.nblk * sp.parts, sp.span > 8 ? 4 : 1), dim3(256), 0, s>>>(a, src, sp);
   return hipGetLastError();
 }
 
diff --git a/snappy.jl_amd/csrc/sm_compress_fast.hip b/snappy.jl_amd/csrc/sm_compress_fast.hip
--- a/snappy.jl_amd/csrc/sm_compress_fast.hip
+++ b/snappy.jl_amd/csrc/sm_compress_fast.hip
@@ -179,6 +179,35 @@
   return launch_compress_sc(a, mode, s);
 }
 
+hipError_t launch_compress_batch_parts(const CompressArgs& a0, int mode, const BatchParts& bp, uint8_t* scratch,
+                                       hipStream_t s) {
+  if ((mode != 1 && mode != 2) || bp.rem == 0 || bp.rem > a0.nblk || bp.parts < 2 ||
+      bp.parts > kBlockScs / kPartMinScs || (bp.parts & (bp.parts - 1)) ||
+      (uint64_t)bp.rem * bp.parts > compress_grid() || !scratch)
+    return hipErrorInvalidValue;
+  CompressArgs a = a0;
+  a.screened = 1;
+  hipLaunchKernelGGL(k_literal_screen, dim3(a.nblk), dim3(kScrThreads), 0, s, a);
+  hipError_t e = hipGetLastError();
+  if (e != hipSuccess) return e;
+  const uint32_t whole = a.nblk - bp.rem;
+  a.nblk = whole;
+  CompressArgs r = a;
+  r.nblk = bp.rem;
+  r.in_off += whole;
+  r.in_len += whole;
+  r.out_off += whole;
+  r.out_len += whole;
+  const uint32_t span = kBlockScs / bp.parts;
+  uint32_t* const part_len = reinterpret_cast<uint32_t*>(scratch + batch_parts_len_offset(compress_grid()));
+  const ScSpan sp{bp.parts, span, (uint64_t)span * kSpanSlot, part_len, (uint64_t)kBlockScs * kSpanSlot};
+  CompressArgs p = r;
+  p.out = scratch;
+  e = launch_compress_sc_parts(a, p, sp, mode, s);
+  if (e != hipSuccess) return e;
+  return launch_batch_parts_gather(r, scratch, sp, s);
+}
+
 hipError_t launch_compress_span(const CompressArgs& a0, int mode, const ScSpan& sp, hipStream_t s) {
   if (mode != 1 && mode != 2) return hipErrorInvalidValue;
   CompressArgs a = a0;
diff --git a/snappy.jl_amd/csrc/sm_compress_sc.hip b/snappy.jl_amd/csrc/sm_compress_sc.hip
--- a/snappy.jl_amd/csrc/sm_compress_sc.hip
+++ b/snappy.jl_amd/csrc/sm_compress_sc.hip
@@ -252,12 +252,13 @@
   uint32_t n;
 };
 
-__device__ __attribute__((always_inline)) inline uint32_t sc_next_block(const CompressArgs& a, uint32_t from, uint32_t lane) {
-  for (uint32_t b0 = from; b0 < a.nblk; b0 += 64 * gridDim.x) {
-    const uint32_t bb = b0 + lane * gridDim.x;
+__device__ __attribute__((always_inline)) inline uint32_t sc_next_block(const CompressArgs& a, uint32_t from, uint32_t g,
+                                                                   uint32_t lane) {
+  for (uint32_t b0 = from; b0 < a.nblk; b0 += 64 * g) {
+    const uint32_t bb = b0 + lane * g;
     const bool todo = bb < a.nblk && (!a.screened || a.out_len[bb] == kScreenTodoSc);
     const uint64_t m = ballot(todo);
-    if (m) return b0 + ctz64(m) * gridDim.x;
+    if (m) return b0 + ctz64(m) * g;
   }
   return a.nblk;
 }
@@ -611,26 +612,17 @@
   __hip_atomic_store(&S.rsize[slot], total + 1, __ATOMIC_RELEASE, __HIP_MEMORY_SCOPE_WORKGROUP);
 }
 
+typedef uint32_t __attribute__((ext_vector_type(4), aligned(1))) sc_u128u;
 __device__ __attribute__((always_inline)) inline void sc_copy_out(uint8_t* const g, const uint8_t* stg, uint32_t len,
                                                                  uint32_t lane) {
-  const uint32_t ad = (uint32_t)((uintptr_t)g & 15);
-  const uint32_t u0 = ad ? 1u : 0u, u1 = (len + ad) >> 4;
-  uint4* const g16 = reinterpret_cast<uint4*>(g - ad);
-  const uint32_t* const s32 = reinterpret_cast<const uint32_t*>(stg);
-  for (uint32_t u = u0 + lane; u < u1; u += 64) {
-    const uint32_t j = 16 * u - ad;
-    const uint32_t* w = s32 + (j >> 2);
-    const uint32_t r0 = w[0], r1 = w[1], r2 = w[2], r3 = w[3], r4 = w[4];
-    g16[u] = make_uint4(__builtin_amdgcn_alignbyte(r1, r0, j), __builtin_amdgcn_alignbyte(r2, r1, j),
-                        __builtin_amdgcn_alignbyte(r3, r2, j), __builtin_amdgcn_alignbyte(r4, r3, j));
-  }
-  const uint32_t nh = min(u0 ? 16 - ad : 0u, len);
-  const uint32_t tb = max(16 * u1 > ad ? 16 * u1 - ad : 0u, nh);
-  const uint32_t nt = len - tb;
-  if (lane < nh + nt) {
-    const uint32_t jj = lane < nh ? lane : tb + (lane - nh);
-    g[jj] = stg[jj];
-  }
+  const uint32_t nu = len >> 4;
+  for (uint32_t u = lane; u < nu; u += 64) {
+    const uint4 v = reinterpret_cast<const uint4*>(stg)[u];
+    sc_u128u x;
+    x.x = v.x, x.y = v.y, x.z = v.z, x.w = v.w;
+    *reinterpret_cast<sc_u128u*>(g + 16 * u) = x;
+  }
+  if (lane < (len & 15u)) g[16 * nu + lane] = stg[16 * nu + lane];
 }
 
 __device__ __attribute__((always_inline)) inline void sc_writer(ScLds& S, uint32_t n, uint8_t* const dst, uint32_t hv,
@@ -679,14 +671,118 @@
 }
 
 template <int kDense>
-__global__ __launch_bounds__(kScThreads) void k_compress_sc(CompressArgs a) {
+__device__ __attribute__((always_inline)) inline void sc_span_item(ScLds& S, const CompressArgs& a, const ScSpan& sp,
+                                                                  const uint32_t item) {
+  const uint32_t tid = threadIdx.x;
+  const uint32_t wave = uniform(tid >> 6);
+  const uint32_t lane = tid & 63;
+  const uint32_t b = item / sp.parts, j = item % sp.parts;
+  if (b >= a.nblk) return;
+  uint32_t* const plen = sp.part_len + item;
+  const uint32_t n = a.in_len[b];
+  if (n > kBlockSize) {
+    if (tid == 0) *plen = j == 0 ? 0xffffffffu : 0u;
+    return;
+  }
+  const uint32_t nsc = (n + kScS - 1) / kScS;
+  const uint32_t k0 = j * sp.span, k1 = min(k0 + sp.span, nsc);
+  const bool todo = !a.screened || a.out_len[b] == kScreenTodoSc;
+  if (!todo || k0 >= k1) {
+    if (tid == 0) *plen = (!todo && j == 0) ? (sp.blk_pitch ? kPartScreened : a.out_len[b]) : 0u;
+    return;
+  }
+  const uint8_t* const src = a.in + a.in_off[b];
+  uint8_t* const dst = a.out + (sp.blk_pitch ? b * sp.blk_pitch : a.out_off[b]) + (uint64_t)j * sp.pitch;
+  if (((uintptr_t)src & 15) == 0) {
+    const uint4* s16 = reinterpret_cast<const uint4*>(src);
+    uint4* d16 = reinterpret_cast<uint4*>(S.blk);
+    const uint32_t n16 = n >> 4;
+    for (uint32_t k = tid; k < n16; k += kScThreads) d16[k] = s16[k];
+    for (uint32_t k = (n & ~15u) + tid; k < n; k += kScThreads) S.blk[k] = src[k];
+  } else {
+    for (uint32_t k = tid; k < n; k += kScThreads) S.blk[k] = src[k];
+  }
+  if (tid < 64) S.blk[n + tid] = 0;
+  {
+    uint4* t16 = reinterpret_cast<uint4*>(S.T);
+    for (uint32_t k = tid; k < 4 * kScTabWords / 16; k += kScThreads) t16[k] = make_uint4(0, 0, 0, 0);
+  }
+  const uint32_t hv = (a.header && j == 0) ? varint_len(n) : 0u;
+  if (tid < hv) dst[tid] = (uint8_t)(((n >> (7 * tid)) & 0x7f) | (tid + 1 < hv ? 0x80 : 0));
+  if (wave == 0) {
+    if (lane < kScRing) {
+      S.rsize[lane] = 0;
+      S.rseq[lane] = k0 + ((lane - k0) & (kScRing - 1));
+    }
+    if (lane == 0) {
+      S.ins = k0;
+      S.next = 64 * k0;
+      S.err = 0;
+    }
+  }
+  __syncthreads();
+  const uint32_t pe = kScS * k0;
+  const uint32_t sub = lane & 15, gq = lane >> 4;
+  for (int ph = 1; ph >= 0; --ph) {
+    for (uint32_t i = wave; 128 * (4 * i) < pe; i += kScW) {
+      const uint32_t G = 2 * (4 * i + gq) + (uint32_t)ph;
+      const uint32_t q = 64 * G + 4 * sub;
+      if (q >= pe) continue;
+      const uint32_t d0 = sc_ld32(S.blk, q), d1 = sc_ld32(S.blk, q + 4);
+      uint32_t* t[4];
+#pragma unroll
+      for (uint32_t j = 0; j < 4; ++j) {
+        const uint32_t w = j ? __builtin_amdgcn_alignbyte(d1, d0, j) : d0;
+        t[j] = &S.T[(w * kHashMul) >> (32 - kScTabBits)];
+      }
+      if (ph) {
+#pragma unroll
+        for (uint32_t j = 0; j < 4; ++j)
+          if (q + j + 4 <= n) __hip_atomic_fetch_max(t[j], (q + j) << 16, __ATOMIC_RELAXED, __HIP_MEMORY_SCOPE_WORKGROUP);
+      } else {
+        uint32_t hi[4];
+#pragma unroll
+        for (uint32_t j = 0; j < 4; ++j) hi[j] = __hip_atomic_load(t[j], __ATOMIC_RELAXED, __HIP_MEMORY_SCOPE_WORKGROUP);
+#pragma unroll
+        for (uint32_t j = 0; j < 4; ++j)
+          if (q + j + 4 <= n)
+            __hip_atomic_fetch_max(t[j], (hi[j] & 0xffff0000u) | (q + j), __ATOMIC_RELAXED, __HIP_MEMORY_SCOPE_WORKGROUP);
+      }
+    }
+    __syncthreads();
+  }
+  if (wave == kScWorkers) {
+    __builtin_amdgcn_s_setprio(SC_WPRIO);
+    sc_writer(S, n, dst, hv, k0, k1, false, plen, lane);
+    __builtin_amdgcn_s_setprio(0);
+  } else {
+    for (;;) {
+      const uint32_t k = uniform(__hip_atomic_fetch_add(&S.next, 1u, __ATOMIC_RELAXED, __HIP_MEMORY_SCOPE_WORKGROUP)) >> 6;
+      if (k >= k1) break;
+      sc_superchunk<kDense>(S, k, n, wave, lane);
+    }
+  }
+}
+
+template <int kDense>
+__global__ __launch_bounds__(kScThreads) void k_compress_sc_span(CompressArgs a, ScSpan sp) {
   __shared__ __attribute__((aligned(16))) ScLds S;
+  sc_span_item<kDense>(S, a, sp, blockIdx.x);
+}
+
+template <int kDense>
+__global__ __launch_bounds__(kScThreads) void k_compress_sc(CompressArgs a, uint32_t g, CompressArgs r, ScSpan sp) {
+  __shared__ __attribute__((aligned(16))) ScLds S;
+  if (blockIdx.x >= g) {
+    sc_span_item<kDense>(S, r, sp, blockIdx.x - g);
+    return;
+  }
   const uint32_t tid = threadIdx.x;
   const uint32_t wave = uniform(tid >> 6);
   const uint32_t lane = tid & 63;
   static_assert(kBlockSize / 16 / kScThreads == 4, "four 16-byte pieces per thread of a full block");
   uint4 pf0, pf1, pf2, pf3;
-  uint32_t b = sc_next_block(a, blockIdx.x, lane);
+  uint32_t b = sc_next_block(a, blockIdx.x, g, lane);
   uint32_t n = 0;
   const uint8_t* src = nullptr;
   bool inpf = false;
@@ -708,7 +804,7 @@
     uint8_t* const dst = a.out + a.out_off[b];
     if (n > kBlockSize) {
       if (tid == 0) a.out_len[b] = 0xffffffffu;
-      b = sc_next_block(a, b + gridDim.x, lane);
+      b = sc_next_block(a, b + g, g, lane);
       SC_FETCH(b)
       continue;
     }
@@ -745,7 +841,7 @@
         S.err = 0;
       }
     }
-    const uint32_t bn = sc_next_block(a, b + gridDim.x, lane);
+    const uint32_t bn = sc_next_block(a, b + g, g, lane);
     __syncthreads();
 
     const uint32_t nsc = (n + kScS - 1) / kScS;
@@ -765,100 +861,6 @@
     b = bn;
   }
 #undef SC_FETCH
-}
-
-template <int kDense>
-__global__ __launch_bounds__(kScThreads) void k_compress_sc_span(CompressArgs a, ScSpan sp) {
-  __shared__ __attribute__((aligned(16))) ScLds S;
-  const uint32_t tid = threadIdx.x;
-  const uint32_t wave = uniform(tid >> 6);
-  const uint32_t lane = tid & 63;
-  const uint32_t b = blockIdx.x / sp.parts, j = blockIdx.x % sp.parts;
-  if (b >= a.nblk) return;
-  uint32_t* const plen = sp.part_len + blockIdx.x;
-  const uint32_t n = a.in_len[b];
-  if (n > kBlockSize) {
-    if (tid == 0) *plen = j == 0 ? 0xffffffffu : 0u;
-    return;
-  }
-  const uint32_t nsc = (n + kScS - 1) / kScS;
-  const uint32_t k0 = j * sp.span, k1 = min(k0 + sp.span, nsc);
-  const bool todo = !a.screened || a.out_len[b] == kScreenTodoSc;
-  if (!todo || k0 >= k1) {
-    if (tid == 0) *plen = (!todo && j == 0) ? a.out_len[b] : 0u;
-    return;
-  }
-  const uint8_t* const src = a.in + a.in_off[b];
-  uint8_t* const dst = a.out + a.out_off[b] + (uint64_t)j * sp.pitch;
-  if (((uintptr_t)src & 15) == 0) {
-    const uint4* s16 = reinterpret_cast<const uint4*>(src);
-    uint4* d16 = reinterpret_cast<uint4*>(S.blk);
-    const uint32_t n16 = n >> 4;
-    for (uint32_t k = tid; k < n16; k += kScThreads) d16[k] = s16[k];
-    for (uint32_t k = (n & ~15u) + tid; k < n; k += kScThreads) S.blk[k] = src[k];
-  } else {
-    for (uint32_t k = tid; k < n; k += kScThreads) S.blk[k] = src[k];
-  }
-  if (tid < 64) S.blk[n + tid] = 0;
-  {
-    uint4* t16 = reinterpret_cast<uint4*>(S.T);
-    for (uint32_t k = tid; k < 4 * kScTabWords / 16; k += kScThreads) t16[k] = make_uint4(0, 0, 0, 0);
-  }
-  const uint32_t hv = (a.header && j == 0) ? varint_len(n) : 0u;
-  if (tid < hv) dst[tid] = (uint8_t)(((n >> (7 * tid)) & 0x7f) | (tid + 1 < hv ? 0x80 : 0));
-  if (wave == 0) {
-    if (lane < kScRing) {
-      S.rsize[lane] = 0;
-      S.rseq[lane] = k0 + ((lane - k0) & (kScRing - 1));
-    }
-    if (lane == 0) {
-      S.ins = k0;
-      S.next = 64 * k0;
-      S.err = 0;
-    }
-  }
-  __syncthreads();
-  const uint32_t pe = kScS * k0;
-  const uint32_t sub = lane & 15, gq = lane >> 4;
-  for (int ph = 1; ph >= 0; --ph) {
-    for (uint32_t i = wave; 128 * (4 * i) < pe; i += kScW) {
-      const uint32_t G = 2 * (4 * i + gq) + (uint32_t)ph;
-      const uint32_t q = 64 * G + 4 * sub;
-      if (q >= pe) continue;
-      const uint32_t d0 = sc_ld32(S.blk, q), d1 = sc_ld32(S.blk, q + 4);
-      uint32_t* t[4];
-#pragma unroll
-      for (uint32_t j = 0; j < 4; ++j) {
-        const uint32_t w = j ? __builtin_amdgcn_alignbyte(d1, d0, j) : d0;
-        t[j] = &S.T[(w * kHashMul) >> (32 - kScTabBits)];
-      }
-      if (ph) {
-#pragma unroll
-        for (uint32_t j = 0; j < 4; ++j)
-          if (q + j + 4 <= n) __hip_atomic_fetch_max(t[j], (q + j) << 16, __ATOMIC_RELAXED, __HIP_MEMORY_SCOPE_WORKGROUP);
-      } else {
-        uint32_t hi[4];
-#pragma unroll
-        for (uint32_t j = 0; j < 4; ++j) hi[j] = __hip_atomic_load(t[j], __ATOMIC_RELAXED, __HIP_MEMORY_SCOPE_WORKGROUP);
-#pragma unroll
-        for (uint32_t j = 0; j < 4; ++j)
-          if (q + j + 4 <= n)
-            __hip_atomic_fetch_max(t[j], (hi[j] & 0xffff0000u) | (q + j), __ATOMIC_RELAXED, __HIP_MEMORY_SCOPE_WORKGROUP);
-      }
-    }
-    __syncthreads();
-  }
-  if (wave == kScWorkers) {
-    __builtin_amdgcn_s_setprio(SC_WPRIO);
-    sc_writer(S, n, dst, hv, k0, k1, false, plen, lane);
-    __builtin_amdgcn_s_setprio(0);
-  } else {
-    for (;;) {
-      const uint32_t k = uniform(__hip_atomic_fetch_add(&S.next, 1u, __ATOMIC_RELAXED, __HIP_MEMORY_SCOPE_WORKGROUP)) >> 6;
-      if (k >= k1) break;
-      sc_superchunk<kDense>(S, k, n, wave, lane);
-    }
-  }
 }
 
 hipError_t launch_compress_sc_span(const CompressArgs& a, int mode, const ScSpan& sp, hipStream_t s) {
@@ -875,7 +877,7 @@
 }
 
 
-hipError_t launch_compress_sc(const CompressArgs& a, int mode, hipStream_t s) {
+uint32_t compress_grid() {
   static uint32_t ncu_cache[64] = {};
   int dev = 0;
   if (hipGetDevice(&dev) != hipSuccess || dev < 0 || dev >= 64) dev = 0;
@@ -886,12 +888,26 @@
     ncu = (uint32_t)v;
     __atomic_store_n(&ncu_cache[dev], ncu, __ATOMIC_RELAXED);
   }
-  const uint32_t grid = min(a.nblk, ncu);
+  return ncu;
+}
+
+hipError_t launch_compress_sc_parts(const CompressArgs& a, const CompressArgs& r, const ScSpan& sp, int mode,
+                                    hipStream_t s) {
+  const uint32_t g = min(a.nblk, compress_grid());
+  const uint32_t items = sp.parts ? r.nblk * sp.parts : 0u;
+  if (items && (sp.span == 0 || sp.parts * sp.span < (kBlockSize + kScS - 1) / kScS ||
+                sp.pitch < (uint64_t)sp.span * kScSlot || sp.blk_pitch < sp.parts * sp.pitch))
+    return hipErrorInvalidValue;
+  if (g + items == 0) return hipSuccess;
   if (mode == 2)
-    hipLaunchKernelGGL(k_compress_sc<1>, dim3(grid), dim3(kScThreads), 0, s, a);
+    hipLaunchKernelGGL(k_compress_sc<1>, dim3(g + items), dim3(kScThreads), 0, s, a, g, r, sp);
   else
-    hipLaunchKernelGGL(k_compress_sc<0>, dim3(grid), dim3(kScThreads), 0, s, a);
+    hipLaunchKernelGGL(k_compress_sc<0>, dim3(g + items), dim3(kScThreads), 0, s, a, g, r, sp);
   return hipGetLastError();
 }
 
-}
+hipError_t launch_compress_sc(const CompressArgs& a, int mode, hipStream_t s) {
+  return launch_compress_sc_parts(a, CompressArgs{}, ScSpan{}, mode, s);
+}
+
+}
diff --git a/snappy.jl_amd/csrc/sm_internal.h b/snappy.jl_amd/csrc/sm_internal.h
--- a/snappy.jl_amd/csrc/sm_internal.h
+++ b/snappy.jl_amd/csrc/sm_internal.h
@@ -95,12 +95,35 @@
   uint32_t parts, span;
   uint64_t pitch;
   uint32_t* part_len;
+  uint64_t blk_pitch = 0;
 };
+constexpr uint32_t kPartScreened = 0xffeffffdu;
 hipError_t launch_compress_span(const CompressArgs& a, int mode, const ScSpan& sp, hipStream_t s);
 hipError_t launch_compress_sc_span(const CompressArgs& a, int mode, const ScSpan& sp, hipStream_t s);
+hipError_t launch_compress_sc_parts(const CompressArgs& a, const CompressArgs& r, const ScSpan& sp, int mode,
+                                    hipStream_t s);
 hipError_t launch_parts_gather(const uint8_t* src, const uint64_t* out_off, const ScSpan& sp, const uint8_t* in,
                                const uint64_t* in_off, const uint32_t* in_len, uint32_t nblk, uint64_t* tot,
                                uint8_t* dst, hipStream_t s);
+constexpr uint32_t kBlockScs = 64;
+constexpr uint32_t kPartMinScs = 4;
+struct BatchParts {
+  uint32_t rem;
+  uint32_t parts;
+};
+inline BatchParts batch_parts_rule(uint32_t nblk, uint32_t grid) {
+  const uint32_t r = grid ? nblk % grid : 0u;
+  if (r == 0 || r > grid / 2) return {0u, 0u};
+  uint32_t p = 2;
+  while (p < kBlockScs / kPartMinScs && r * (2 * p) <= grid) p *= 2;
+  return {r, p};
+}
+inline size_t batch_parts_len_offset(uint32_t grid) { return (size_t)(grid / 2) * kBlockScs * kSpanSlot; }
+inline size_t batch_parts_scratch(uint32_t grid) { return batch_parts_len_offset(grid) + 4 * (size_t)grid; }
+uint32_t compress_grid();
+hipError_t launch_compress_batch_parts(const CompressArgs& a, int mode, const BatchParts& bp, uint8_t* scratch,
+                                       hipStream_t s);
+hipError_t launch_batch_parts_gather(const CompressArgs& a, const uint8_t* src, const ScSpan& sp, hipStream_t s);
 hipError_t launch_frag_gather(const uint8_t* src, const uint64_t* src_off, const uint32_t* out_len,
                               const uint32_t* in_len, uint32_t nfrag, uint64_t* tot, uint8_t* dst, hipStream_t s);
 hipError_t launch_place(const uint8_t* src, const uint64_t* src_off, const uint32_t* len, const uint64_t* dst_off,
```

Result: faster. 396.4 GB/s (median of 6 runs) (+1.6%).
